# rvp-group/Splat-LOAM

Measured on AMD Instinct MI355X. Metric: fwd+bwd Msplats/s, higher is better.
Workload: dtype f32; 1 GPU; 500000 surfels, 64x2048 spherical, 1 keyframe/GPU per iteration drawn from a window of 8 keyframes as Mapper.optimize does (sample_geometric, p=0.4): render fwd + mapper loss + bwd + fused Adam (one native sls_mapping_step per iteration); step=one bench step = 10 mapping iterations (1013 steps = 10130 timed iterations), N=500000, H=64, W=2048, keyframes=8, parallelism=keyframe-dp1, status_read=lagged-1, gradient_sums=float atomics

## Files before the change

include/sls_abi.h:

```cpp
#ifndef SLS_ABI_H
#define SLS_ABI_H

#include <stddef.h>
#include <stdint.h>

#ifdef __cplusplus
extern "C" {
#endif

#define SLS_OK 0
#define SLS_E_ARG (-1)
#define SLS_E_HIP (-2)
#define SLS_E_SCRATCH (-3)
#define SLS_E_UNSUPPORTED (-4)

typedef struct SlsCamera {
    int32_t H, W;
    int32_t wrap;
    int32_t tile_cull_min;
    float fx, fy, cx, cy;
    float scale_modifier;
    float near_cut, far_cut;
    uint32_t flags;
    float Rvw[9];
    float tvw[3];
    float pix_offset[2];
} SlsCamera;
#define SLS_CAM_LEAN_ALLMAP 1u

const char *sls_last_error(void);
int sls_version(void);

int sls_tile_w(void);
int sls_tile_h(void);
int sls_rec_stride(void);
int sls_grec_stride(void);

int sls_camera_from_matrices(const float *view_host, const float *proj_host, int H, int W,
                             float scale_modifier, SlsCamera *out);

int sls_ray_tables(const SlsCamera *cam, float *col_cs_host, float *row_cs_host);
int sls_ray_tables_at(const SlsCamera *cam, float col_offset, float row_offset, float *col_cs_host,
                      float *row_cs_host);

size_t sls_stage1_scratch_bytes(int N);
int sls_forward_stage1(const SlsCamera *cam, int N,
                       const float *means3D, const float *scales, const float *rotations,
                       const float *opacities, const float *col_cs, const float *row_cs,
                       float *rec, int32_t *radii, int32_t *rect, uint32_t *tiles_touched, uint64_t *tile_mask,
                       uint32_t *block_box,
                       float *depth, uint32_t *order, uint32_t *offsets, uint32_t *total_out,
                       void *scratch, size_t scratch_bytes, void *stream);

size_t sls_sort_scratch_bytes(uint64_t R);
size_t sls_block_mask_bytes(uint64_t R, int H, int W);
int sls_forward_stage2(const SlsCamera *cam, int N, uint64_t R,
                       const float *rec, const int32_t *rect, const uint32_t *tiles_touched,
                       const uint64_t *tile_mask, const uint32_t *block_box,
                       const float *depth, const uint32_t *order, const uint32_t *offsets,
                       const uint32_t *total_dev,
                       uint32_t *tile_keys, uint32_t *vals, uint32_t *tile_keys_tmp, uint32_t *vals_tmp,
                       void *sort_scratch, size_t sort_scratch_bytes, int *sorted_in_tmp,
                       uint64_t *keys64_out, int list_pairs,
                       const uint32_t **sorted_list, int *sorted_stride,
                       uint32_t *ranges, const float *col_cs, const float *row_cs,
                       float *allmap, float *pix_state, uint32_t *pix_contrib,
                       uint32_t *tile_consumed, uint64_t *block_masks, int *block_masks_shape, void *stream);

int sls_backward(const SlsCamera *cam, int N, uint64_t R,
                 const float *means3D, const float *scales, const float *rotations,
                 const int32_t *radii, const float *rec,
                 const uint32_t *ranges, const uint32_t *vals_sorted, int vals_stride,
                 const float *col_cs, const float *row_cs,
                 const float *pix_state, const uint32_t *pix_contrib,
                 const float *dL_dallmap, float *grec,
                 float *dL_dmeans3D, float *dL_dscales, float *dL_drotations,
                 float *dL_dopacities, const uint64_t *block_masks, int block_masks_shape, void *stream);

size_t sls_pose_grad_scratch_bytes(int N);
int sls_backward_pose(const SlsCamera *cam, int N, uint64_t R,
                      const float *means3D, const float *scales, const float *rotations,
                      const int32_t *radii, const float *rec,
                      const uint32_t *ranges, const uint32_t *vals_sorted, int vals_stride,
                      const float *col_cs, const float *row_cs,
                      const float *pix_state, const uint32_t *pix_contrib,
                      const float *dL_dallmap, float *grec,
                      float *dL_dmeans3D, float *dL_dscales, float *dL_drotations,
                      float *dL_dopacities, const uint64_t *block_masks, int block_masks_shape,
                      float *pose_grad, void *pose_scratch, size_t pose_scratch_bytes, void *stream);

size_t sls_backward_det_scratch_bytes(int N);
int sls_backward_det(const SlsCamera *cam, int N, uint64_t R,
                     const float *means3D, const float *scales, const float *rotations, const int32_t *radii,
                     const float *rec, const uint32_t *ranges, const uint32_t *vals_sorted, int vals_stride,
                     const float *col_cs, const float *row_cs, const float *pix_state, const uint32_t *pix_contrib,
                     const float *dL_dallmap,
                     float *dL_dmeans3D, float *dL_dscales, float *dL_drotations, float *dL_dopacities,
                     const uint64_t *block_masks, int block_masks_shape, void *det_scratch, size_t det_scratch_bytes,
                     void *stream);
int sls_backward_det_pose(const SlsCamera *cam, int N, uint64_t R,
                          const float *means3D, const float *scales, const float *rotations, const int32_t *radii,
                          const float *rec, const uint32_t *ranges, const uint32_t *vals_sorted, int vals_stride,
                          const float *col_cs, const float *row_cs, const float *pix_state, const uint32_t *pix_contrib,
                          const float *dL_dallmap,
                          float *dL_dmeans3D, float *dL_dscales, float *dL_drotations, float *dL_dopacities,
                          const uint64_t *block_masks, int block_masks_shape, void *det_scratch, size_t det_scratch_bytes,
                          float *pose_grad, void *pose_scratch, size_t pose_scratch_bytes, void *stream);

struct SlsMappingStatus;
size_t sls_forward_ws_bytes(int N, int H, int W, uint64_t R_capacity);
int sls_forward_ws(const SlsCamera *cam, int N, const float *means3D, const float *scales, const float *rotations,
                   const float *opacities, const float *col_cs, const float *row_cs, uint64_t R_capacity,
                   uint32_t *depth_order, int reuse_rounds, int list_pairs, int workspace_ready, int want_backward,
                   int32_t *radii, float *allmap, void *workspace, size_t workspace_bytes, struct SlsMappingStatus *status_dev,
                   struct SlsMappingStatus *status_mirror, const uint32_t **sorted_list, int *sorted_stride,
                   int *block_masks_shape, void *stream);
int sls_wait_status_mirror(const void *mirror_host, uint32_t sentinel, void *stream);
int sls_backward_ws(const SlsCamera *cam, int N, const float *means3D, const float *scales, const float *rotations,
                    const int32_t *radii, const float *col_cs, const float *row_cs, const float *dL_dallmap,
                    uint64_t R_capacity, void *workspace, size_t workspace_bytes, const uint32_t *sorted_list,
                    int sorted_stride, int block_masks_shape, uint32_t *block_order, float *dL_dmeans3D,
                    float *dL_dscales, float *dL_drotations, float *dL_dopacities, void *stream);
int sls_backward_ws_pose(const SlsCamera *cam, int N, const float *means3D, const float *scales, const float *rotations,
                         const int32_t *radii, const float *col_cs, const float *row_cs, const float *dL_dallmap,
                         uint64_t R_capacity, void *workspace, size_t workspace_bytes, const uint32_t *sorted_list,
                         int sorted_stride, int block_masks_shape, uint32_t *block_order, float *dL_dmeans3D,
                         float *dL_dscales, float *dL_drotations, float *dL_dopacities, float *pose_grad,
                         void *pose_scratch, size_t pose_scratch_bytes, void *stream);

size_t sls_consumer_scratch_bytes(int H, int W);
int sls_consumer_fwd_bwd(int H, int W, const float *allmap, const float *gt_depth, const uint8_t *valid,
                         const float *col_cs_half, const float *row_cs_half, float depth_ratio,
                         float lambda_normal, float lambda_alpha, int n_valid, float *loss_sums,
                         float *dL_dallmap, void *scratch, size_t scratch_bytes, void *stream);

int sls_render_maps(int H, int W, const float *allmap, const float *view_rot9, const float *col_cs_half,
                    const float *row_cs_half, float depth_ratio, float *rend_normal, float *surf_depth,
                    float *surf_normal, void *stream);

int sls_densify_weights(int H, int W, const float *image_depth, const uint8_t *valid, const float *rend_alpha,
                        float threshold_opacity, float *weights_out, uint32_t *stats_out, void *stream);

#define SLS_DENSIFY_DRAW_MAX_PIXELS 262144
size_t sls_densify_draw_scratch_bytes(int H, int W);
int sls_densify_draw(int H, int W, const float *image_depth, const uint8_t *valid, const float *rend_alpha,
                     float threshold_opacity, double percentage, uint64_t seed, uint32_t draw_index, float *weights_out,
                     int64_t *pixels_out, uint32_t *stats_out, uint32_t *stats_mirror, void *scratch, size_t scratch_bytes,
                     void *stream);

int sls_densify_rows(int n, int H, int W, const int64_t *pixels, const float *image_depth, const float *image_normal,
                     const float *col_cs_half, const float *row_cs_half, const float *cam_to_model16,
                     const float *model_T_frame16, float *xyz_out, float *quat_out, void *stream);

#define SLS_SURFACE_MAX_PIXELS 262144
size_t sls_surface_scratch_bytes(int H, int W);
int sls_surface_samples(int H, int W, const float *allmap, const float *col_cs_half, const float *row_cs_half,
                        const float *cam_to_world12, float min_opacity, float max_depth_dist, float depth_ratio,
                        int n_samples, uint64_t seed, uint32_t frame_id, float *points_out, float *normals_out,
                        int32_t *pixels_out, uint32_t *status_out, void *scratch, size_t scratch_bytes, void *stream);

struct SlsMappingStatus;
typedef struct SlsMappingConfig {
    float lambda_alpha, lambda_normal, scaling_max, scaling_max_penalty, depth_ratio;
    float lr_xyz, lr_opacity, lr_scaling, lr_rotation;
    int32_t apply_adam;
    int32_t reuse_depth_order;
    int32_t keep_grads;
    int32_t workspace_ready;
    double beta1, beta2, eps;
    uint32_t *depth_order;
    struct SlsMappingStatus *status_mirror;
    float *void_flags_out;
    uint32_t grad_chunk;
    uint32_t grad_ranks;
    int32_t deterministic;
    int32_t block_masks;
    uint64_t *grad_bitmap;
    uint8_t *det_prev;
    int32_t phase;
    int32_t reserved;
    uint32_t *block_order;
    const uint64_t *union_bitmap;
    const uint32_t *union_prefix;
    float *grad_compact;
    uint32_t *grad_compact_index;
    uint32_t grad_compact_capacity;
    uint32_t reserved2;
    float *pose_grad;
    void *pose_scratch;
    size_t pose_scratch_bytes;
} SlsMappingConfig;
typedef struct SlsMappingStatus {
    uint32_t R;
    uint32_t overflow;
    float loss_sums[4];
    float loss_reg;
    uint32_t exchange_count;
} SlsMappingStatus;
size_t sls_mapping_workspace_bytes(int N, int H, int W, uint64_t R_capacity);
size_t sls_block_order_bytes(int H, int W);
size_t sls_mapping_workspace_bytes_cfg(int N, int H, int W, uint64_t R_capacity, const struct SlsMappingConfig *cfg);
int sls_mapping_step(const SlsCamera *cam, int N,
                     float *xyz, float *scaling_raw, float *rotation_raw, float *opacity_raw,
                     float *grads, float *exp_avg, float *exp_avg_sq, int64_t adam_step,
                     const float *gt_depth, const uint8_t *valid, int n_valid,
                     const float *col_cs, const float *row_cs,
                     const float *col_cs_half, const float *row_cs_half,
                     const SlsMappingConfig *cfg, uint64_t R_capacity,
                     void *workspace, size_t workspace_bytes,
                     SlsMappingStatus *status_dev, float **allmap_out, void *stream);

#define SLS_MAX_BATCH 8
typedef struct SlsKeyframeInputs {
    SlsCamera cam;
    const float *gt_depth;
    const uint8_t *valid;
    int32_t n_valid;
    int32_t reuse_depth_order;
    const float *col_cs, *row_cs;
    const float *col_cs_half, *row_cs_half;
    uint32_t *depth_order;
    uint32_t *block_order;
    uint8_t *det_prev;
    float *pose_grad;
} SlsKeyframeInputs;
size_t sls_mapping_workspace_bytes_batch(int G, int N, int H, int W, uint64_t R_capacity, const SlsMappingConfig *cfg);
int sls_mapping_step_batch(int G, const SlsKeyframeInputs *keyframes, int N,
                           float *xyz, float *scaling_raw, float *rotation_raw, float *opacity_raw,
                           float *grads, float *exp_avg, float *exp_avg_sq, int64_t adam_step,
                           const SlsMappingConfig *cfg, uint64_t R_capacity, void *workspace, size_t workspace_bytes,
                           SlsMappingStatus *status_dev, void *stream);

typedef struct SlsAlignerParams {
    int32_t num_iterations;
    int32_t min_inliers;
    float max_distance;
    float min_cos_angle;
    float huber_delta;
    float range_weight;
    float range_huber;
    float depth_min, depth_max;
    float damping;
} SlsAlignerParams;
typedef struct SlsAlignerResult {
    float pose[12];
    float fitness;
    float chi2;
    float last_step;
    int32_t inliers, valid_query, iterations;
} SlsAlignerResult;
size_t sls_aligner_workspace_bytes(void);
int sls_aligner_normals(const SlsCamera *cam, const float *depth, const float *points, float depth_min,
                        float *normals, void *stream);
int sls_aligner_linearize(const SlsCamera *cam, const SlsAlignerParams *prm, const float *ref_depth,
                          const float *ref_points, const float *ref_normals, const float *query_depth,
                          const float *query_points, const float *T_host, void *workspace, double *sys_out,
                          void *stream);
int sls_aligner_align(const SlsCamera *cam, const SlsAlignerParams *prm, const float *ref_depth,
                      const float *ref_points, const float *ref_normals, const float *query_depth,
                      const float *query_points, const float *T_host, void *workspace,
                      SlsAlignerResult *result_dev, void *stream);

size_t sls_projector_scratch_bytes(int H, int W);
int sls_projector_prepare(int H, int W, void *scratch, size_t scratch_bytes, void *stream);
int sls_projector_intrinsics(int n, const float *cloud, int H, int W, float full_azimuth_threshold_deg,
                             float *intrinsics_out, void *scratch, size_t scratch_bytes, void *stream);
int sls_projector_project(int n, const float *cloud, const float *K_dev, int H, int W, float depth_min,
                          float depth_max, int32_t *lut, float *range_image, float *normals_image,
                          uint8_t *valid, void *scratch, size_t scratch_bytes, void *stream);

typedef struct SlsAdamGroup {
    float *param;
    const float *grad;
    float *exp_avg;
    float *exp_avg_sq;
    int64_t numel;
    float lr;
    float pad;
} SlsAdamGroup;
int sls_adam_step(const SlsAdamGroup *groups_host, int ngroups, double beta1, double beta2,
                  double eps, int64_t step, void *stream);
int sls_adam_step_guarded(const SlsAdamGroup *groups_host, int ngroups, double beta1, double beta2,
                          double eps, int64_t step, const uint32_t *skip_flag_dev, void *stream);
int sls_adam_step_reduced(const SlsAdamGroup *groups_host, int ngroups, double beta1, double beta2,
                          double eps, int64_t step, const float *void_flags_dev,
                          struct SlsMappingStatus *status_dev, struct SlsMappingStatus *status_mirror,
                          void *stream);

int sls_grad_union(int N, const uint64_t *bitmaps, int n_bitmaps, uint64_t *union_bitmap, uint32_t capacity,
                   uint32_t *word_prefix, struct SlsMappingStatus *status_dev, void *stream);
int sls_adam_step_union(int N, float *xyz, float *opacity_raw, float *scaling_raw, float *rotation_raw,
                        const uint32_t *compact_index, const float *compact_reduced, uint32_t capacity, float *exp_avg,
                        float *exp_avg_sq, float lr_xyz, float lr_opacity, float lr_scaling, float lr_rotation, double beta1,
                        double beta2, double eps, int64_t step, struct SlsMappingStatus *status_dev,
                        struct SlsMappingStatus *status_mirror, void *stream);
size_t sls_grad_bitmap_words(int N);
int sls_grad_compact(int N, const uint64_t *bitmaps, int n_bitmaps, uint64_t *union_bitmap, const float *grads_flat,
                     float *compact, uint32_t capacity, uint32_t *word_prefix, struct SlsMappingStatus *status_dev,
                     void *stream);
int sls_adam_step_sparse(int N, float *xyz, float *opacity_raw, float *scaling_raw, float *rotation_raw,
                         const uint64_t *union_bitmap, const uint32_t *word_prefix, const float *compact_reduced,
                         float *exp_avg, float *exp_avg_sq, float lr_xyz, float lr_opacity, float lr_scaling,
                         float lr_rotation, double beta1, double beta2, double eps, int64_t step, int part,
                         struct SlsMappingStatus *status_dev, struct SlsMappingStatus *status_mirror, void *stream);

size_t sls_knn_scratch_bytes(int M);
int sls_knn_dist2(int M, const float *xyz, float *out, void *scratch, size_t scratch_bytes,
                  void *stream);
int sls_knn_dist2_first(int M, int M_first, const float *xyz, float *out, void *scratch, size_t scratch_bytes,
                        void *stream);

int sls_mark_visible(const SlsCamera *cam, int N, const float *means3D, uint8_t *visible,
                     void *stream);

int sls_timing_slots(void);
const char *sls_timing_name(int slot);
int sls_timing_enable(int mode);
int sls_timing_collect(double *total_ms_host, int64_t *counts_host);

int sls_debug_wave_cycles(uint32_t *fwd_cycles, uint32_t *bwd_cycles);

int sls_debug_variant(int fwd, int bwd);

int sls_selftest(void *stream);

#ifdef __cplusplus
}
#endif
#endif
```

splat_loam_amd/_abi.py:

```python
from __future__ import annotations

import ctypes as C
import os

_HERE = os.path.dirname(os.path.abspath(__file__))
LIB_PATH = os.path.join(_HERE, "libsls_hip.so")

SLS_OK = 0


class SlsCamera(C.Structure):
    _fields_ = [
        ("H", C.c_int32), ("W", C.c_int32), ("wrap", C.c_int32), ("tile_cull_min", C.c_int32),
        ("fx", C.c_float), ("fy", C.c_float), ("cx", C.c_float), ("cy", C.c_float),
        ("scale_modifier", C.c_float), ("near_cut", C.c_float), ("far_cut", C.c_float), ("flags", C.c_uint32),
        ("Rvw", C.c_float * 9), ("tvw", C.c_float * 3),
        ("pix_offset", C.c_float * 2),
    ]


class SlsMappingConfig(C.Structure):
    _fields_ = [
        ("lambda_alpha", C.c_float), ("lambda_normal", C.c_float), ("scaling_max", C.c_float),
        ("scaling_max_penalty", C.c_float), ("depth_ratio", C.c_float),
        ("lr_xyz", C.c_float), ("lr_opacity", C.c_float), ("lr_scaling", C.c_float), ("lr_rotation", C.c_float),
        ("apply_adam", C.c_int32), ("reuse_depth_order", C.c_int32), ("keep_grads", C.c_int32), ("workspace_ready", C.c_int32),
        ("beta1", C.c_double), ("beta2", C.c_double), ("eps", C.c_double),
        ("depth_order", C.c_void_p),
        ("status_mirror", C.c_void_p),
        ("void_flags_out", C.c_void_p),
        ("grad_chunk", C.c_uint32), ("grad_ranks", C.c_uint32),
        ("deterministic", C.c_int32), ("block_masks", C.c_int32),
        ("grad_bitmap", C.c_void_p),
        ("det_prev", C.c_void_p),
        ("phase", C.c_int32), ("reserved", C.c_int32),
        ("block_order", C.c_void_p),
        ("union_bitmap", C.c_void_p), ("union_prefix", C.c_void_p), ("grad_compact", C.c_void_p),
        ("grad_compact_index", C.c_void_p), ("grad_compact_capacity", C.c_uint32), ("reserved2", C.c_uint32),
        ("pose_grad", C.c_void_p), ("pose_scratch", C.c_void_p), ("pose_scratch_bytes", C.c_size_t),
    ]


class SlsAlignerParams(C.Structure):
    _fields_ = [("num_iterations", C.c_int32), ("min_inliers", C.c_int32), ("max_distance", C.c_float),
                ("min_cos_angle", C.c_float), ("huber_delta", C.c_float), ("range_weight", C.c_float),
                ("range_huber", C.c_float), ("depth_min", C.c_float), ("depth_max", C.c_float), ("damping", C.c_float)]


class SlsAlignerResult(C.Structure):
    _fields_ = [("pose", C.c_float * 12), ("fitness", C.c_float), ("chi2", C.c_float), ("last_step", C.c_float),
                ("inliers", C.c_int32), ("valid_query", C.c_int32), ("iterations", C.c_int32)]


class SlsMappingStatus(C.Structure):
    _fields_ = [("R", C.c_uint32), ("overflow", C.c_uint32), ("loss_sums", C.c_float * 4),
                ("loss_reg", C.c_float), ("exchange_count", C.c_uint32)]


class SlsKeyframeInputs(C.Structure):
    _fields_ = [
        ("cam", SlsCamera), ("gt_depth", C.c_void_p), ("valid", C.c_void_p), ("n_valid", C.c_int32),
        ("reuse_depth_order", C.c_int32), ("col_cs", C.c_void_p), ("row_cs", C.c_void_p), ("col_cs_half", C.c_void_p),
        ("row_cs_half", C.c_void_p), ("depth_order", C.c_void_p), ("block_order", C.c_void_p), ("det_prev", C.c_void_p),
        ("pose_grad", C.c_void_p),
    ]


SLS_MAX_BATCH = 8


class SlsAdamGroup(C.Structure):
    _fields_ = [
        ("param", C.c_void_p), ("grad", C.c_void_p), ("exp_avg", C.c_void_p), ("exp_avg_sq", C.c_void_p),
        ("numel", C.c_int64), ("lr", C.c_float), ("pad", C.c_float),
    ]


_VP = C.c_void_p
_PROTOS = {
    "sls_last_error": (C.c_char_p, []),
    "sls_version": (C.c_int, []),
    "sls_tile_w": (C.c_int, []),
    "sls_tile_h": (C.c_int, []),
    "sls_rec_stride": (C.c_int, []),
    "sls_grec_stride": (C.c_int, []),
    "sls_camera_from_matrices": (C.c_int, [_VP, _VP, C.c_int, C.c_int, C.c_float, C.POINTER(SlsCamera)]),
    "sls_ray_tables": (C.c_int, [C.POINTER(SlsCamera), _VP, _VP]),
    "sls_ray_tables_at": (C.c_int, [C.POINTER(SlsCamera), C.c_float, C.c_float, _VP, _VP]),
    "sls_render_maps": (C.c_int, [C.c_int, C.c_int, _VP, _VP, _VP, _VP, C.c_float, _VP, _VP, _VP, _VP]),
    "sls_densify_rows": (C.c_int, [C.c_int, C.c_int, C.c_int] + [_VP] * 10),
    "sls_densify_weights": (C.c_int, [C.c_int, C.c_int, _VP, _VP, _VP, C.c_float, _VP, _VP, _VP]),
    "sls_densify_draw_scratch_bytes": (C.c_size_t, [C.c_int, C.c_int]),
    "sls_densify_draw": (C.c_int, [C.c_int, C.c_int, _VP, _VP, _VP, C.c_float, C.c_double, C.c_uint64, C.c_uint32] +
                         [_VP] * 5 + [C.c_size_t, _VP]),
    "sls_surface_scratch_bytes": (C.c_size_t, [C.c_int, C.c_int]),
    "sls_surface_samples": (C.c_int, [C.c_int, C.c_int, _VP, _VP, _VP, _VP, C.c_float, C.c_float, C.c_float, C.c_int, C.c_uint64,
                                      C.c_uint32, _VP, _VP, _VP, _VP, _VP, C.c_size_t, _VP]),
    "sls_consumer_scratch_bytes": (C.c_size_t, [C.c_int, C.c_int]),
    "sls_consumer_fwd_bwd": (C.c_int, [C.c_int, C.c_int] + [_VP] * 5 + [C.c_float] * 3 + [C.c_int, _VP, _VP, _VP,
                                                                                         C.c_size_t, _VP]),
    "sls_stage1_scratch_bytes": (C.c_size_t, [C.c_int]),
    "sls_forward_stage1": (C.c_int, [C.POINTER(SlsCamera), C.c_int] + [_VP] * 16 + [_VP, C.c_size_t, _VP]),
    "sls_sort_scratch_bytes": (C.c_size_t, [C.c_uint64]),
    "sls_forward_stage2": (C.c_int, [C.POINTER(SlsCamera), C.c_int, C.c_uint64] + [_VP] * 13 +
                           [_VP, C.c_size_t, C.POINTER(C.c_int), _VP, C.c_int, C.POINTER(C.c_void_p), C.POINTER(C.c_int)] +
                           [_VP] * 8 + [C.POINTER(C.c_int), _VP]),
    "sls_block_mask_bytes": (C.c_size_t, [C.c_uint64, C.c_int, C.c_int]),
    "sls_mapping_workspace_bytes": (C.c_size_t, [C.c_int, C.c_int, C.c_int, C.c_uint64]),
    "sls_block_order_bytes": (C.c_size_t, [C.c_int, C.c_int]),
    "sls_mapping_workspace_bytes_cfg": (C.c_size_t, [C.c_int, C.c_int, C.c_int, C.c_uint64, C.POINTER(SlsMappingConfig)]),
    "sls_mapping_step": (C.c_int, [C.POINTER(SlsCamera), C.c_int] + [_VP] * 7 + [C.c_int64, _VP, _VP, C.c_int] +
                         [_VP] * 4 + [C.POINTER(SlsMappingConfig), C.c_uint64, _VP, C.c_size_t, _VP,
                                      C.POINTER(C.c_void_p), _VP]),
    "sls_mapping_workspace_bytes_batch": (C.c_size_t, [C.c_int, C.c_int, C.c_int, C.c_int, C.c_uint64,
                                                       C.POINTER(SlsMappingConfig)]),
    "sls_mapping_step_batch": (C.c_int, [C.c_int, C.POINTER(SlsKeyframeInputs), C.c_int] + [_VP] * 7 +
                               [C.c_int64, C.POINTER(SlsMappingConfig), C.c_uint64, _VP, C.c_size_t, _VP, _VP]),
    "sls_backward": (C.c_int, [C.POINTER(SlsCamera), C.c_int, C.c_uint64] + [_VP] * 7 + [C.c_int] + [_VP] * 11 +
                     [C.c_int, _VP]),
    "sls_forward_ws_bytes": (C.c_size_t, [C.c_int, C.c_int, C.c_int, C.c_uint64]),
    "sls_forward_ws": (C.c_int, [C.POINTER(SlsCamera), C.c_int] + [_VP] * 6 + [C.c_uint64, _VP, C.c_int, C.c_int, C.c_int, C.c_int, _VP, _VP,
                                 _VP, C.c_size_t, _VP, _VP, C.POINTER(C.c_void_p), C.POINTER(C.c_int), C.POINTER(C.c_int), _VP]),
    "sls_backward_ws": (C.c_int, [C.POINTER(SlsCamera), C.c_int] + [_VP] * 7 + [C.c_uint64, _VP, C.c_size_t, _VP, C.c_int, C.c_int] +
                        [_VP] * 6),
    "sls_backward_det_scratch_bytes": (C.c_size_t, [C.c_int]),
    "sls_backward_det": (C.c_int, [C.POINTER(SlsCamera), C.c_int, C.c_uint64] + [_VP] * 7 + [C.c_int] + [_VP] * 10 +
                         [C.c_int, _VP, C.c_size_t, _VP]),
    "sls_pose_grad_scratch_bytes": (C.c_size_t, [C.c_int]),
    "sls_backward_pose": (C.c_int, [C.POINTER(SlsCamera), C.c_int, C.c_uint64] + [_VP] * 7 + [C.c_int] + [_VP] * 11 +
                          [C.c_int, _VP, _VP, C.c_size_t, _VP]),
    "sls_backward_ws_pose": (C.c_int, [C.POINTER(SlsCamera), C.c_int] + [_VP] * 7 + [C.c_uint64, _VP, C.c_size_t, _VP, C.c_int, C.c_int] +
                             [_VP] * 5 + [_VP, _VP, C.c_size_t, _VP]),
    "sls_backward_det_pose": (C.c_int, [C.POINTER(SlsCamera), C.c_int, C.c_uint64] + [_VP] * 7 + [C.c_int] + [_VP] * 10 +
                              [C.c_int, _VP, C.c_size_t, _VP, _VP, C.c_size_t, _VP]),
    "sls_adam_step": (C.c_int, [C.POINTER(SlsAdamGroup), C.c_int, C.c_double, C.c_double, C.c_double, C.c_int64, _VP]),
    "sls_adam_step_guarded": (C.c_int, [C.POINTER(SlsAdamGroup), C.c_int, C.c_double, C.c_double, C.c_double,
                                        C.c_int64, _VP, _VP]),
    "sls_adam_step_reduced": (C.c_int, [C.POINTER(SlsAdamGroup), C.c_int, C.c_double, C.c_double, C.c_double,
                                        C.c_int64, _VP, _VP, _VP, _VP]),
    "sls_grad_bitmap_words": (C.c_size_t, [C.c_int]),
    "sls_grad_union": (C.c_int, [C.c_int, _VP, C.c_int, _VP, C.c_uint32, _VP, _VP, _VP]),
    "sls_adam_step_union": (C.c_int, [C.c_int] + [_VP] * 6 + [C.c_uint32, _VP, _VP] + [C.c_float] * 4 + [C.c_double] * 3 + [C.c_int64, _VP, _VP, _VP]),
    "sls_grad_compact": (C.c_int, [C.c_int, _VP, C.c_int, _VP, _VP, _VP, C.c_uint32, _VP, _VP, _VP]),
    "sls_adam_step_sparse": (C.c_int, [C.c_int] + [_VP] * 9 + [C.c_float] * 4 + [C.c_double] * 3 + [C.c_int64, C.c_int, _VP, _VP, _VP]),
    "sls_projector_scratch_bytes": (C.c_size_t, [C.c_int, C.c_int]),
    "sls_projector_prepare": (C.c_int, [C.c_int, C.c_int, _VP, C.c_size_t, _VP]),
    "sls_projector_intrinsics": (C.c_int, [C.c_int, _VP, C.c_int, C.c_int, C.c_float, _VP, _VP, C.c_size_t, _VP]),
    "sls_projector_project": (C.c_int, [C.c_int, _VP, _VP, C.c_int, C.c_int, C.c_float, C.c_float, _VP, _VP, _VP, _VP,
                                        _VP, C.c_size_t, _VP]),
    "sls_knn_scratch_bytes": (C.c_size_t, [C.c_int]),
    "sls_knn_dist2": (C.c_int, [C.c_int, _VP, _VP, _VP, C.c_size_t, _VP]),
    "sls_wait_status_mirror": (C.c_int, [_VP, C.c_uint32, _VP]),
    "sls_knn_dist2_first": (C.c_int, [C.c_int, C.c_int, _VP, _VP, _VP, C.c_size_t, _VP]),
    "sls_mark_visible": (C.c_int, [C.POINTER(SlsCamera), C.c_int, _VP, _VP, _VP]),
    "sls_aligner_workspace_bytes": (C.c_size_t, []),
    "sls_aligner_normals": (C.c_int, [C.POINTER(SlsCamera), _VP, _VP, C.c_float, _VP, _VP]),
    "sls_aligner_linearize": (C.c_int, [C.POINTER(SlsCamera), C.POINTER(SlsAlignerParams)] + [_VP] * 8 + [_VP]),
    "sls_aligner_align": (C.c_int, [C.POINTER(SlsCamera), C.POINTER(SlsAlignerParams)] + [_VP] * 8 + [_VP]),
    "sls_timing_slots": (C.c_int, []),
    "sls_timing_name": (C.c_char_p, [C.c_int]),
    "sls_timing_enable": (C.c_int, [C.c_int]),
    "sls_timing_collect": (C.c_int, [C.POINTER(C.c_double), C.POINTER(C.c_int64)]),
    "sls_debug_wave_cycles": (C.c_int, [_VP, _VP]),
    "sls_debug_variant": (C.c_int, [C.c_int, C.c_int]),
    "sls_selftest": (C.c_int, [_VP]),
}

EXPORTS = tuple(_PROTOS)

_lib = None


def lib():
    global _lib
    if _lib is None:
        if not os.path.exists(LIB_PATH):
            raise RuntimeError(
                f"{LIB_PATH} is missing: build it with `python -c 'import __graft_entry__ as g; g.build()'` "
                "(hipcc --offload-arch=gfx950).  There is no CPU fallback.")
        import torch
        l = C.CDLL(LIB_PATH)
        for name, (res, args) in _PROTOS.items():
            fn = getattr(l, name)
            fn.restype = res
            fn.argtypes = args
        _lib = l
    return _lib


def check(rc: int, what: str) -> None:
    if rc != SLS_OK:
        msg = lib().sls_last_error().decode("utf-8", "replace")
        raise RuntimeError(f"{what} failed (code {rc}): {msg}")


def tile_size() -> tuple[int, int]:
    l = lib()
    return int(l.sls_tile_w()), int(l.sls_tile_h())
```

splat_loam_amd/csrc/sls_common.hpp:

```cpp
#pragma once
#include <atomic>
#include <cmath>

#include <hip/hip_runtime.h>
#include <stdint.h>
#include <stdio.h>

#include "../../include/sls_abi.h"
#include "../../include/sls_spec.h"
#include "../../include/sls_det_math.h"

#ifndef SLS_TILE_W
#define SLS_TILE_W 16
#endif
#ifndef SLS_TILE_H
#define SLS_TILE_H 16
#endif
static_assert((SLS_TILE_W * SLS_TILE_H) % 64 == 0, "a tile must be a whole number of wave64s");
static_assert(SLS_TILE_W % 8 == 0 && SLS_TILE_H % 8 == 0, "tiles are made of 8x8 wave sub-tiles");

namespace sls {

constexpr int kWave = 64;
constexpr int kTileW = SLS_TILE_W;
constexpr int kTileH = SLS_TILE_H;
constexpr int kTilePix = kTileW * kTileH;
constexpr int kRec4 = SLS_REC_STRIDE / 4;
constexpr int kGrec = SLS_GREC_STRIDE;

void set_error(const char *fmt, ...);

enum TimerSlot {
    T_PREPROCESS_FWD = 0, T_SCAN, T_EMIT_KEYS, T_SORT_HIST, T_SORT_ROWSCAN, T_SORT_SCATTER, T_TILE_RANGES,
    T_RENDER_FWD, T_GREC_MEMSET, T_RENDER_BWD, T_PREPROCESS_BWD, T_ADAM, T_KNN, T_CONSUMER, T_RESORT, T_BIN_COUNT, T_BIN_DIRECT,
    T_COUNT
};
struct DebugState {
    std::atomic<uint32_t *> dbg_fwd_cycles{nullptr}, dbg_bwd_cycles{nullptr};
};
DebugState &debug_state();
void timer_begin(int slot, hipStream_t st);
void timer_end(int slot, hipStream_t st);
struct ScopedTimer {
    int slot; hipStream_t st;
    bool open = true;
    ScopedTimer(int s, hipStream_t t) : slot(s), st(t) { timer_begin(slot, st); }
    void end_now() { if (open) { timer_end(slot, st); open = false; } }
    ~ScopedTimer() { end_now(); }
};

#define SLS_HIP_CHECK(expr)                                                         \
    do {                                                                            \
        hipError_t e_ = (expr);                                                     \
        if (e_ != hipSuccess) {                                                     \
            ::sls::set_error("%s failed: %s (%s:%d)", #expr, hipGetErrorString(e_), \
                             __FILE__, __LINE__);                                   \
            return SLS_E_HIP;                                                       \
        }                                                                           \
    } while (0)

#define SLS_LAUNCH_CHECK(name)                                                              \
    do {                                                                                    \
        hipError_t e_ = hipGetLastError();                                                  \
        if (e_ != hipSuccess) {                                                             \
            ::sls::set_error("launch of %s failed: %s", name, hipGetErrorString(e_));       \
            return SLS_E_HIP;                                                               \
        }                                                                                   \
    } while (0)

#define SLS_REQUIRE(cond, msg)                       \
    do {                                             \
        if (!(cond)) {                               \
            ::sls::set_error("%s: %s", __func__, msg); \
            return SLS_E_ARG;                        \
        }                                            \
    } while (0)

struct DevCam {
    int H, W, wrap, GX, GY;
    float fx, fy, cx, cy, mod, near_c, far_c;
    float R[9];
    float t[3];
    SlsTileCullCam tc;
    int tile_cull;
};

inline SlsTileCullCam make_tile_cull_cam(float fx, float fy, int W, int wrap)
{
    SlsTileCullCam c;
    const double hx = 0.5 * (double)(kTileW - 1), hy = 0.5 * (double)(kTileH - 1);
    const double ax = 0.5 / (double)fx, ay = 0.5 / (double)fy;
    c.chx = (float)cos(ax); c.shx = (float)sin(ax);
    c.chy = (float)cos(ay); c.shy = (float)sin(ay);
    const double kx = hx / (double)fx, ky = hy / (double)fy;
    c.kx = (float)kx; c.ky = (float)ky;
    const double span = fabs(kx) + fabs(ky);
    c.eps = (float)(0.5 * span * span * 1.01 + 4.0e-6);
    c.hx = (float)hx; c.hy = (float)hy;
    c.wrapW = wrap ? (float)W : 0.0f;
    c.invW = wrap ? 1.0f / (float)W : 0.0f;
    return c;
}

inline DevCam make_devcam(const SlsCamera &c)
{
    DevCam d;
    d.H = c.H; d.W = c.W; d.wrap = c.wrap;
    d.GX = (c.W + kTileW - 1) / kTileW;
    d.GY = (c.H + kTileH - 1) / kTileH;
    d.fx = c.fx; d.fy = c.fy;
    d.cx = c.cx - c.pix_offset[0]; d.cy = c.cy - c.pix_offset[1];
    d.mod = c.scale_modifier; d.near_c = c.near_cut; d.far_c = c.far_cut;
    for (int i = 0; i < 9; ++i) d.R[i] = c.Rvw[i];
    for (int i = 0; i < 3; ++i) d.t[i] = c.tvw[i];
    d.tc = make_tile_cull_cam(d.fx, d.fy, d.W, d.wrap);
    d.tile_cull = c.tile_cull_min == 0 ? SLS_TILE_CULL_MIN_DEFAULT : (c.tile_cull_min == 1 ? 0 : c.tile_cull_min);
    return d;
}

__host__ __device__ inline bool block_box_fits(int W, int H) { return W <= 4096 && H <= 128; }
__device__ __forceinline__ uint32_t make_block_box(float cx, float cy, float ex, float ey, int NC)
{
    if (!(ex >= 0.0f && ey >= 0.0f)) return 0u;
    const float lo = ceilf((cx - ex - 7.01f) * 0.125f), hi = floorf((cx + ex + 0.01f) * 0.125f);
    const int n = (int)fminf(hi - lo, (float)(NC - 1));
    int c0 = (int)fmaxf(fminf(lo, 1.0e6f), -1.0e6f) % NC;
    c0 += c0 < 0 ? NC : 0;
    const int r0 = (int)fminf(fmaxf(ceilf((cy - ey - 1.01f) * 0.5f), 0.0f), 63.0f);
    const int r1 = (int)fminf(floorf((cy + ey + 0.01f) * 0.5f), 63.0f);
    if (n < 0 || r1 < r0) return 0u;
    return (uint32_t)c0 | ((uint32_t)(n + 1) << 9) | ((uint32_t)r0 << 19) | ((uint32_t)(r1 + 1) << 25);
}

__device__ __forceinline__ uint64_t wave_ballot(bool p) { return __builtin_amdgcn_ballot_w64(p); }
__device__ __forceinline__ bool wave_all(bool p) { return __builtin_amdgcn_ballot_w64(!p) == 0ull; }

__device__ __forceinline__ int lane_id() { return (int)__builtin_amdgcn_mbcnt_hi(~0u, __builtin_amdgcn_mbcnt_lo(~0u, 0u)); }

template <int CTRL, int ROW_MASK>
__device__ __forceinline__ float dpp_mov0(float v)
{
    return __builtin_bit_cast(float, __builtin_amdgcn_update_dpp(0, __builtin_bit_cast(int, v), CTRL, ROW_MASK, 0xF, false));
}

__device__ __forceinline__ float wave_sum_to_lane63(float v)
{
    v += dpp_mov0<0xB1, 0xF>(v);
    v += dpp_mov0<0x4E, 0xF>(v);
    v += dpp_mov0<0x124, 0xF>(v);
    v += dpp_mov0<0x128, 0xF>(v);
    v += dpp_mov0<0x142, 0xA>(v);
    v += dpp_mov0<0x143, 0xC>(v);
    return v;
}

__device__ __forceinline__ float dpp_xor4(float v)
{
    int a = __builtin_amdgcn_update_dpp(0, __builtin_bit_cast(int, v), 0x104, 0xF, 0x5, false);
    a = __builtin_amdgcn_update_dpp(a, __builtin_bit_cast(int, v), 0x114, 0xF, 0xA, false);
    return __builtin_bit_cast(float, a);
}

typedef float v2f __attribute__((ext_vector_type(2)));
typedef unsigned v2u __attribute__((ext_vector_type(2)));
__device__ __forceinline__ v2f mk2(float a, float b) { v2f r; r.x = a; r.y = b; return r; }

__device__ __forceinline__ void permlane32_swap(float &a, float &b)
{
    const v2u r = __builtin_amdgcn_permlane32_swap(__float_as_uint(a), __float_as_uint(b), false, false);
    a = __uint_as_float(r.x); b = __uint_as_float(r.y);
}
__device__ __forceinline__ void permlane16_swap(float &a, float &b)
{
    const v2u r = __builtin_amdgcn_permlane16_swap(__float_as_uint(a), __float_as_uint(b), false, false);
    a = __uint_as_float(r.x); b = __uint_as_float(r.y);
}

__device__ __forceinline__ float block_reduce16_pk(const v2f (&x)[8], int lane)
{
    float a[16];
#pragma unroll
    for (int i = 0; i < 8; ++i) { a[2 * i] = x[i].x; a[2 * i + 1] = x[i].y; }
#pragma unroll
    for (int i = 0; i < 8; ++i) permlane32_swap(a[i], a[i + 8]);
    v2f y[4];
#pragma unroll
    for (int i = 0; i < 4; ++i) y[i] = mk2(a[2 * i], a[2 * i + 1]) + mk2(a[2 * i + 8], a[2 * i + 9]);
    float b[8];
#pragma unroll
    for (int i = 0; i < 4; ++i) { b[2 * i] = y[i].x; b[2 * i + 1] = y[i].y; }
#pragma unroll
    for (int i = 0; i < 4; ++i) permlane16_swap(b[i], b[i + 4]);
    const v2f z01 = mk2(b[0], b[1]) + mk2(b[4], b[5]), z23 = mk2(b[2], b[3]) + mk2(b[6], b[7]);
    const float z[4] = { z01.x, z01.y, z23.x, z23.y };
    float w0 = z[0], w1 = z[1];
    asm("s_nop 1\n\t"
        "v_add_f32_dpp %0, %0, %0 row_ror:8 row_mask:0xf bank_mask:0x3\n\t"
        "v_add_f32_dpp %1, %1, %1 row_ror:8 row_mask:0xf bank_mask:0x3\n\t"
        "v_add_f32_dpp %0, %2, %2 row_ror:8 row_mask:0xf bank_mask:0xc\n\t"
        "v_add_f32_dpp %1, %3, %3 row_ror:8 row_mask:0xf bank_mask:0xc\n\t"
        "s_nop 1\n\t"
        "v_add_f32_dpp %0, %0, %0 row_shl:4 row_mask:0xf bank_mask:0x5\n\t"
        "v_add_f32_dpp %0, %1, %1 row_shr:4 row_mask:0xf bank_mask:0xa"
        : "+v"(w0), "+v"(w1) : "v"(z[2]), "v"(z[3]));
    const float r = w0;
    (void)lane;
    return r;
}

__device__ __forceinline__ bool mask_bbox8x8(uint64_t m, int &xmin, int &xmax, int &ymin, int &ymax)
{
    if (m == 0) return false;
    uint64_t c = m | (m >> 32);
    c |= c >> 16;
    c |= c >> 8;
    const uint32_t cols = (uint32_t)c & 0xFFu;
    uint64_t t = (m | (m >> 4)) & 0x0F0F0F0F0F0F0F0Full;
    t = (t | (t >> 2)) & 0x0303030303030303ull;
    t = (t | (t >> 1)) & 0x0101010101010101ull;
    xmin = __builtin_ctz(cols);
    xmax = 31 - __builtin_clz(cols);
    ymin = __builtin_ctzll(t) >> 3;
    ymax = (63 - __builtin_clzll(t)) >> 3;
    return true;
}

__device__ __forceinline__ float readlane63(float v)
{
    return __builtin_bit_cast(float, __builtin_amdgcn_readlane(__builtin_bit_cast(int, v), 63));
}

__host__ __device__ inline uint32_t depth_order_key(float range)
{
    constexpr uint32_t kBase = 0x3E000000u;
    constexpr uint32_t kMax = (1u << 29) - 1u;
#if defined(__HIP_DEVICE_COMPILE__)
    const uint32_t b = __float_as_uint(range) & 0x7FFFFFFFu;
#else
    uint32_t b; __builtin_memcpy(&b, &range, 4); b &= 0x7FFFFFFFu;
#endif
    const uint32_t k = b > kBase ? b - kBase : 0u;
    return k < kMax ? k : kMax;
}

__device__ __forceinline__ uint32_t det_predict(float sum)
{
    const uint32_t e = (__float_as_uint(sum) >> 23) & 0xFFu;
    return sum == 0.0f ? 0u : min(max(e + 12u, 1u), 254u);
}
constexpr uint32_t kDetMispredicted = 8u;
__device__ __forceinline__ int det_scale_exp(uint32_t own, uint32_t gex)
{
    return (int)max(own, gex > 24u ? gex - 24u : (gex ? 1u : 0u));
}

struct AdamCoef {
    float w1, b2, w2, eps, bc2_sqrt, bc1;
};
inline AdamCoef make_adam_coef(double beta1, double beta2, double eps, int64_t step)
{
    AdamCoef c;
    c.w1 = (float)(1.0 - beta1);
    c.b2 = (float)beta2;
    c.w2 = (float)(1.0 - beta2);
    c.eps = (float)eps;
    c.bc1 = (float)(1.0 - pow(beta1, (double)step));
    c.bc2_sqrt = (float)sqrt(1.0 - pow(beta2, (double)step));
    return c;
}
__device__ __forceinline__ void adam_one(float &p, float g, float &m, float &v, float step_size, const AdamCoef &a)
{
    m = m + (g - m) * a.w1;
    v = v * a.b2 + (a.w2 * g) * g;
    const float denom = __builtin_amdgcn_sqrtf(v) * __builtin_amdgcn_rcpf(a.bc2_sqrt) + a.eps;
    p = p - step_size * (m * __builtin_amdgcn_rcpf(denom));
}
struct AdamFuse {
    int enabled, write_grads;
    int clear_grec;
    AdamCoef c;
    float lr_xyz, lr_opacity, lr_scaling, lr_rotation;
    float *exp_avg, *exp_avg_sq;
    const uint32_t *skip_flag;
    uint32_t *status_src;
    uint32_t *status_mirror;
    uint8_t *touched;
    float *void_flags;
    int void_count, void_stride;
    uint32_t gchunk;
    float *gbase;
    const uint32_t *det_max;
    const long long *det_acc;
    uint8_t *det_prev;
    uint32_t *det_gex;
    int det_onepass;
    float *reg_accum;
    uint64_t *grad_bitmap;
    int grad_bitmap_words;
    const float *loss_partials;
    int n_loss_partials;
    float loss_w[3];
    int order_T;
    const uint32_t *order_cost;
    uint32_t *order_out;
    int publisher;
    const uint64_t *union_bitmap;
    const uint32_t *union_prefix;
    float *compact;
    uint32_t *compact_idx;
    uint32_t compact_cap;
};

struct BatchKeyframe {
    DevCam cam;
    const int32_t *radii;
    float4 *grec;
    uint8_t *touched;
    uint32_t *status;
    const uint32_t *det_max;
    long long *det_acc;
    uint8_t *det_prev;
    uint32_t *det_gex;
    const float *loss_partials;
    float loss_w[3];
    const uint32_t *order_cost;
    uint32_t *order_out;
};

struct BatchFuse {
    int G;
    int n_loss_partials, order_T;
    BatchKeyframe kf[SLS_MAX_BATCH];
    AdamFuse af;
};

constexpr int kPoseRow = 8;
struct PoseOut {
    float *rows;
    uint32_t *counter;
    float *out[SLS_MAX_BATCH];
};

__device__ __forceinline__ void mirror_status_block(const uint32_t *src, uint32_t *mirror, bool override1 = false,
                                                    uint32_t word1 = 0u)
{
    uint32_t w[8];
#pragma unroll
    for (int k = 0; k < 8; ++k) w[k] = src[k];
    if (override1) w[1] = word1;
#pragma unroll
    for (int k = 0; k < 7; ++k) __builtin_nontemporal_store(w[k], mirror + k);
    __threadfence_system();
    __builtin_nontemporal_store(w[7], mirror + 7);
}

__host__ __device__ inline int xcd_remap(int b, int n)
{
    constexpr int kXcd = 8;
    if (n % kXcd != 0) return b;
    const int per = n / kXcd;
    return (b % kXcd) * per + b / kXcd;
}

}
```

splat_loam_amd/csrc/sls_exchange.hip:

```cpp
#include <string.h>

#include "sls_launch.hpp"

namespace sls {

constexpr uint32_t kExchangeTooSmall = 4u;

constexpr int kPrefixLdsWords = 12288;
__global__ __launch_bounds__(1024) void exchange_prefix_kernel(int nwords, const uint64_t *__restrict__ maps, int n_maps,
                                                               uint64_t *__restrict__ bitmap,
                                                               uint32_t *__restrict__ word_prefix, uint32_t capacity,
                                                               uint32_t *__restrict__ status_block)
{
    extern __shared__ uint64_t s_dyn[];
    __shared__ uint32_t s_wave[16];
    const bool in_lds = nwords <= kPrefixLdsWords;
    const int per = (nwords + 1023) / 1024, w0 = (int)threadIdx.x * per, w1 = min(w0 + per, nwords);
    const int pad = (in_lds && (per & 1) == 0) ? 1 : 0;
    uint64_t *const words = in_lds ? s_dyn : bitmap;
    uint32_t *const pref = in_lds ? reinterpret_cast<uint32_t *>(s_dyn + nwords + 1024) : word_prefix;
    const uint32_t magic = (uint32_t)((0x100000000ull + (uint64_t)per - 1ull) / (uint64_t)per);
#define SLS_PW(w_) ((w_) + (pad ? (int)__umulhi((uint32_t)(w_), magic) : 0))
    const int lane = threadIdx.x & 63, wave = threadIdx.x >> 6;
    const size_t stride = (size_t)(nwords + 2);
    constexpr int kBatch = 12;
    for (int base = 0; base < nwords; base += 1024 * kBatch) {
        uint64_t acc[kBatch];
#pragma unroll
        for (int k = 0; k < kBatch; ++k) acc[k] = 0ull;
        for (int m = 0; m < n_maps; m += 2) {
            uint64_t v0[kBatch], v1[kBatch];
            const bool two = m + 1 < n_maps;
#pragma unroll
            for (int k = 0; k < kBatch; ++k) {
                const int w = base + k * 1024 + (int)threadIdx.x;
                v0[k] = w < nwords ? maps[(size_t)m * stride + (size_t)w] : 0ull;
                v1[k] = (two && w < nwords) ? maps[(size_t)(m + 1) * stride + (size_t)w] : 0ull;
            }
#pragma unroll
            for (int k = 0; k < kBatch; ++k) acc[k] |= v0[k] | v1[k];
        }
#pragma unroll
        for (int k = 0; k < kBatch; ++k) {
            const int w = base + k * 1024 + (int)threadIdx.x;
            if (w < nwords) words[SLS_PW(w)] = acc[k];
        }
    }
    if (!in_lds) __threadfence();
    __syncthreads();
    uint32_t c = 0u;
    const int own = w0 + (pad ? (int)threadIdx.x : 0);
    for (int w = w0; w < w1; ++w) c += (uint32_t)__popcll(words[own + (w - w0)]);
    uint32_t incl = c;
#pragma unroll
    for (int off = 1; off < 64; off <<= 1) {
        const uint32_t t = __shfl_up(incl, off, 64);
        if (lane >= off) incl += t;
    }
    if (lane == 63) s_wave[wave] = incl;
    __syncthreads();
    uint32_t pre = incl - c;
    for (int k = 0; k < wave; ++k) pre += s_wave[k];
    for (int w = w0; w < w1; ++w) {
        pref[own + (w - w0)] = pre;
        pre += (uint32_t)__popcll(words[own + (w - w0)]);
    }
    if (threadIdx.x == 1023) {
        const uint32_t K = pre;
        uint64_t v0 = 0ull, v1 = 0ull;
        for (int m = 0; m < n_maps; ++m) {
            v0 |= maps[(size_t)m * stride + (size_t)nwords];
            v1 |= maps[(size_t)m * stride + (size_t)nwords + 1];
        }
        bitmap[nwords] = v0; bitmap[nwords + 1] = v1;
        const uint32_t void_bits = (v0 ? 1u : 0u) | (v1 ? 2u : 0u);
        status_block[7] = K;
        status_block[1] = void_bits | (K > capacity ? kExchangeTooSmall : 0u);
    }
    if (in_lds) {
        __syncthreads();
        for (int w = threadIdx.x; w < nwords; w += 1024) { bitmap[w] = words[SLS_PW(w)]; word_prefix[w] = pref[SLS_PW(w)]; }
    }
#undef SLS_PW
}

__global__ __launch_bounds__(256) void exchange_compact_kernel(int N, const uint64_t *__restrict__ bitmap,
                                                               const uint32_t *__restrict__ word_prefix,
                                                               const float *__restrict__ grads, float *__restrict__ compact,
                                                               uint32_t capacity)
{
    const int i = blockIdx.x * 256 + threadIdx.x;
    if (i >= N) return;
    const uint64_t word = bitmap[i >> 6];
    const int b = i & 63;
    if (!((word >> b) & 1ull)) return;
    const uint32_t slot = word_prefix[i >> 6] + (uint32_t)__popcll(word & ((1ull << b) - 1ull));
    if (slot >= capacity) return;
    const size_t n = (size_t)N;
    float *o = compact + (size_t)slot * 10;
    o[0] = grads[3 * (size_t)i]; o[1] = grads[3 * (size_t)i + 1]; o[2] = grads[3 * (size_t)i + 2];
    o[3] = grads[3 * n + i];
    o[4] = grads[4 * n + 2 * (size_t)i]; o[5] = grads[4 * n + 2 * (size_t)i + 1];
#pragma unroll
    for (int k = 0; k < 4; ++k) o[6 + k] = grads[6 * n + 4 * (size_t)i + k];
}

__global__ __launch_bounds__(256) void touched_bitmap_kernel(int N, const uint8_t *__restrict__ touched,
                                                             const float2 *__restrict__ scaling_raw, float log_smax_margin,
                                                             int reg_on, const uint32_t *__restrict__ status_block,
                                                             uint64_t *__restrict__ bitmap, int nwords)
{
    const int i = blockIdx.x * 256 + threadIdx.x;
    bool on = false;
    if (i < N) {
        on = touched[i] != 0;
        if (reg_on) { const float2 s = scaling_raw[i]; on = on || fmaxf(s.x, s.y) >= log_smax_margin; }
    }
    const uint64_t word = __ballot(on);
    if ((threadIdx.x & 63) == 0 && i < N) bitmap[i >> 6] = word;
    if (i == 0) {
        const uint32_t bits = status_block[1];
        bitmap[nwords] = (bits & 1u) ? 1ull : 0ull;
        bitmap[nwords + 1] = (bits & ~1u) ? 1ull : 0ull;
    }
}
int launch_touched_bitmap(int N, const uint8_t *touched, const float *scaling_raw, float smax, float pen,
                          const uint32_t *status_block, uint64_t *bitmap, hipStream_t st)
{
    hipLaunchKernelGGL(touched_bitmap_kernel, dim3((N + 255) / 256), dim3(256), 0, st, N, touched, (const float2 *)scaling_raw,
                       logf(fmaxf(smax, 1e-30f)) - 1e-3f, pen != 0.0f ? 1 : 0, status_block, bitmap, (N + 63) / 64);
    SLS_LAUNCH_CHECK("touched_bitmap_kernel");
    return SLS_OK;
}

struct SparseAdamArgs {
    float *xyz, *opacity, *scaling, *rotation;
    float *exp_avg, *exp_avg_sq;
    float lr_xyz, lr_opacity, lr_scaling, lr_rotation;
    AdamCoef c;
};

__global__ __launch_bounds__(256) void exchange_adam_kernel(int N, SparseAdamArgs a, const uint64_t *__restrict__ bitmap,
                                                            const uint32_t *__restrict__ word_prefix,
                                                            const float *__restrict__ compact,
                                                            const uint32_t *__restrict__ status_block,
                                                            uint32_t *__restrict__ status_mirror, int part)
{
    const int i = blockIdx.x * 256 + threadIdx.x;
    if (i == 0 && status_mirror && part != 1) mirror_status_block(status_block, status_mirror);
    if (status_block[1] != 0u) return;
    if (i >= N) return;
    float g[10];
#pragma unroll
    for (int k = 0; k < 10; ++k) g[k] = 0.0f;
    const uint64_t word = bitmap[i >> 6];
    const int b = i & 63;
    const bool in_union = (word >> b) & 1ull;
    if ((part == 1 && in_union) || (part == 2 && !in_union)) return;
    if (in_union) {
        const uint32_t slot = word_prefix[i >> 6] + (uint32_t)__popcll(word & ((1ull << b) - 1ull));
        const float *s = compact + (size_t)slot * 10;
#pragma unroll
        for (int k = 0; k < 10; ++k) g[k] = s[k];
    }
    const size_t n = (size_t)N, ix = 3 * (size_t)i, io = 3 * n + i, is = 4 * n + 2 * (size_t)i, ir = 6 * n + 4 * (size_t)i;
    float *M = a.exp_avg, *V = a.exp_avg_sq;
    const float ibc1 = __builtin_amdgcn_rcpf(a.c.bc1);
    const float st_x = a.lr_xyz * ibc1, st_o = a.lr_opacity * ibc1, st_s = a.lr_scaling * ibc1, st_r = a.lr_rotation * ibc1;
    float p, m, v;
#pragma unroll
    for (int k = 0; k < 3; ++k) {
        p = a.xyz[ix + k]; m = M[ix + k]; v = V[ix + k];
        adam_one(p, g[k], m, v, st_x, a.c);
        a.xyz[ix + k] = p; M[ix + k] = m; V[ix + k] = v;
    }
    p = a.opacity[i]; m = M[io]; v = V[io];
    adam_one(p, g[3], m, v, st_o, a.c);
    a.opacity[i] = p; M[io] = m; V[io] = v;
#pragma unroll
    for (int k = 0; k < 2; ++k) {
        p = a.scaling[2 * (size_t)i + k]; m = M[is + k]; v = V[is + k];
        adam_one(p, g[4 + k], m, v, st_s, a.c);
        a.scaling[2 * (size_t)i + k] = p; M[is + k] = m; V[is + k] = v;
    }
#pragma unroll
    for (int k = 0; k < 4; ++k) {
        p = a.rotation[4 * (size_t)i + k]; m = M[ir + k]; v = V[ir + k];
        adam_one(p, g[6 + k], m, v, st_r, a.c);
        a.rotation[4 * (size_t)i + k] = p; M[ir + k] = m; V[ir + k] = v;
    }
}

__global__ __launch_bounds__(256) void exchange_adam_union_kernel(uint32_t capacity, size_t n, SparseAdamArgs a,
                                                                  const uint32_t *__restrict__ index,
                                                                  const float *__restrict__ compact,
                                                                  const uint32_t *__restrict__ status_block,
                                                                  uint32_t *__restrict__ status_mirror)
{
    const uint32_t slot = blockIdx.x * 256u + threadIdx.x;
    if (slot == 0 && status_mirror) mirror_status_block(status_block, status_mirror);
    if (status_block[1] != 0u) return;
    if (slot >= min(capacity, status_block[7])) return;
    const size_t i = index[slot];
    const size_t off[4] = { 3 * i, 3 * n + i, 4 * n + 2 * i, 6 * n + 4 * i };
    float *const par[4] = { a.xyz + 3 * i, a.opacity + i, a.scaling + 2 * i, a.rotation + 4 * i };
    constexpr int kW[4] = { 3, 1, 2, 4 }, kG[4] = { 0, 3, 4, 6 };
    const float *row = compact + (size_t)slot * 10;
    float g[10], p[10], m[10], v[10];
#pragma unroll
    for (int k = 0; k < 10; ++k) g[k] = row[k];
#pragma unroll
    for (int q = 0; q < 4; ++q)
#pragma unroll
        for (int k = 0; k < kW[q]; ++k) {
            p[kG[q] + k] = par[q][k]; m[kG[q] + k] = a.exp_avg[off[q] + k]; v[kG[q] + k] = a.exp_avg_sq[off[q] + k];
        }
    const float ibc1 = __builtin_amdgcn_rcpf(a.c.bc1);
    const float stp[4] = { a.lr_xyz * ibc1, a.lr_opacity * ibc1, a.lr_scaling * ibc1, a.lr_rotation * ibc1 };
#pragma unroll
    for (int q = 0; q < 4; ++q)
#pragma unroll
        for (int k = 0; k < kW[q]; ++k) adam_one(p[kG[q] + k], g[kG[q] + k], m[kG[q] + k], v[kG[q] + k], stp[q], a.c);
#pragma unroll
    for (int q = 0; q < 4; ++q)
#pragma unroll
        for (int k = 0; k < kW[q]; ++k) {
            par[q][k] = p[kG[q] + k]; a.exp_avg[off[q] + k] = m[kG[q] + k]; a.exp_avg_sq[off[q] + k] = v[kG[q] + k];
        }
}

}

using namespace sls;

extern "C" {

size_t sls_grad_bitmap_words(int N) { return N > 0 ? (size_t)((N + 63) / 64) + 2 : 2; }

int sls_grad_union(int N, const uint64_t *bitmaps, int n_bitmaps, uint64_t *union_bitmap, uint32_t capacity,
                   uint32_t *word_prefix, SlsMappingStatus *status_dev, void *stream)
{
    return sls_grad_compact(N, bitmaps, n_bitmaps, union_bitmap, nullptr, nullptr, capacity, word_prefix, status_dev, stream);
}

int sls_grad_compact(int N, const uint64_t *bitmaps, int n_bitmaps, uint64_t *union_bitmap, const float *grads_flat,
                     float *compact, uint32_t capacity, uint32_t *word_prefix, SlsMappingStatus *status_dev, void *stream)
{
    SLS_REQUIRE(N > 0 && bitmaps && n_bitmaps >= 1 && union_bitmap && word_prefix && status_dev && (!grads_flat == !compact),
                "bad argument");
    hipStream_t st = (hipStream_t)stream;
    const int nwords = (N + 63) / 64;
    const size_t lds = nwords <= kPrefixLdsWords ? (size_t)(nwords + 1024) * 12 + 16 : 0;
    static bool lds_allowed = false;
    if (lds > 0 && !lds_allowed) {
        SLS_HIP_CHECK(hipFuncSetAttribute(reinterpret_cast<const void *>(exchange_prefix_kernel),
                                          hipFuncAttributeMaxDynamicSharedMemorySize, (kPrefixLdsWords + 1024) * 12 + 16));
        lds_allowed = true;
    }
    hipLaunchKernelGGL(exchange_prefix_kernel, dim3(1), dim3(1024), lds, st, nwords, bitmaps, n_bitmaps, union_bitmap,
                       word_prefix, capacity, (uint32_t *)status_dev);
    SLS_LAUNCH_CHECK("exchange_prefix_kernel");
    if (!grads_flat) return SLS_OK;
    hipLaunchKernelGGL(exchange_compact_kernel, dim3((N + 255) / 256), dim3(256), 0, st, N, (const uint64_t *)union_bitmap,
                       (const uint32_t *)word_prefix, grads_flat, compact, capacity);
    SLS_LAUNCH_CHECK("exchange_compact_kernel");
    return SLS_OK;
}

int sls_adam_step_sparse(int N, float *xyz, float *opacity, float *scaling, float *rotation,
                         const uint64_t *union_bitmap, const uint32_t *word_prefix, const float *compact_reduced,
                         float *exp_avg, float *exp_avg_sq, float lr_xyz, float lr_opacity, float lr_scaling,
                         float lr_rotation, double beta1, double beta2, double eps, int64_t step, int part,
                         SlsMappingStatus *status_dev, SlsMappingStatus *status_mirror, void *stream)
{
    SLS_REQUIRE(part >= 0 && part <= 2, "part: 0 every surfel, 1 outside the union, 2 the union");
    SLS_REQUIRE(N > 0 && xyz && opacity && scaling && rotation && union_bitmap && word_prefix && compact_reduced &&
                    exp_avg && exp_avg_sq && status_dev,
                "bad argument");
    SLS_REQUIRE(step >= 1, "step is 1-based");
    SparseAdamArgs a;
    memset(&a, 0, sizeof(a));
    a.xyz = xyz; a.opacity = opacity; a.scaling = scaling; a.rotation = rotation;
    a.exp_avg = exp_avg; a.exp_avg_sq = exp_avg_sq;
    a.lr_xyz = lr_xyz; a.lr_opacity = lr_opacity; a.lr_scaling = lr_scaling; a.lr_rotation = lr_rotation;
    a.c = make_adam_coef(beta1, beta2, eps, step);
    ScopedTimer tm(T_ADAM, (hipStream_t)stream);
    hipLaunchKernelGGL(exchange_adam_kernel, dim3((N + 255) / 256), dim3(256), 0, (hipStream_t)stream, N, a, union_bitmap,
                       word_prefix, compact_reduced, (const uint32_t *)status_dev, (uint32_t *)status_mirror, part);
    SLS_LAUNCH_CHECK("exchange_adam_kernel");
    return SLS_OK;
}

int sls_adam_step_union(int N, float *xyz, float *opacity, float *scaling, float *rotation, const uint32_t *compact_index,
                        const float *compact_reduced, uint32_t capacity, float *exp_avg, float *exp_avg_sq, float lr_xyz,
                        float lr_opacity, float lr_scaling, float lr_rotation, double beta1, double beta2, double eps,
                        int64_t step, SlsMappingStatus *status_dev, SlsMappingStatus *status_mirror, void *stream)
{
    SLS_REQUIRE(N > 0 && xyz && opacity && scaling && rotation && compact_index && compact_reduced && capacity > 0 &&
                    exp_avg && exp_avg_sq && status_dev,
                "bad argument");
    SLS_REQUIRE(step >= 1, "step is 1-based");
    SparseAdamArgs a;
    memset(&a, 0, sizeof(a));
    a.xyz = xyz; a.opacity = opacity; a.scaling = scaling; a.rotation = rotation;
    a.exp_avg = exp_avg; a.exp_avg_sq = exp_avg_sq;
    a.lr_xyz = lr_xyz; a.lr_opacity = lr_opacity; a.lr_scaling = lr_scaling; a.lr_rotation = lr_rotation;
    a.c = make_adam_coef(beta1, beta2, eps, step);
    ScopedTimer tm(T_ADAM, (hipStream_t)stream);
    hipLaunchKernelGGL(exchange_adam_union_kernel, dim3((capacity + 255u) / 256u), dim3(256), 0, (hipStream_t)stream, capacity,
                       (size_t)N, a, compact_index, compact_reduced, (const uint32_t *)status_dev, (uint32_t *)status_mirror);
    SLS_LAUNCH_CHECK("exchange_adam_union_kernel");
    return SLS_OK;
}

}
```

splat_loam_amd/csrc/sls_pipeline.hip:

```cpp
#include <stdlib.h>
#include <string.h>

#include "sls_consumer_dev.hpp"
#include "sls_launch.hpp"

namespace sls {

struct MapWs {
    float *rec; int32_t *radii; int32_t *rect; uint32_t *tiles; uint64_t *tmask; int32_t *erec; int32_t *serec; uint32_t *sbox; float *depth; uint32_t *order; uint32_t *offsets;
    void *order_scratch; size_t order_scratch_bytes;
    uint32_t *tkeys, *vals, *tkeys_tmp, *vals_tmp; void *sort_scratch; size_t sort_scratch_bytes;
    uint32_t *ranges; float *allmap; float *pix_state; uint32_t *pix_contrib; uint32_t *tile_consumed;
    float *dL_dallmap; void *consumer_scratch; size_t consumer_scratch_bytes; float *grec; size_t zero_bytes; uint64_t *block_masks; float *reg_accum; uint8_t *touched;
    uint32_t *det_max; unsigned long long *det_acc; size_t det_bytes;
    uint32_t *det_gex;
    uint32_t *block_cost, *block_order;
    size_t total;
};

struct Taker {
    char *p; size_t off;
    void *operator()(size_t bytes) { void *r = (void *)(p + off); off += (bytes + 255) & ~(size_t)255; return r; }
};

// ... 235 lines not shown
    SLS_REQUIRE(means3D && scales && rotations && radii && grec && dL_dmeans3D && dL_dscales && dL_drotations &&
                    dL_dopacities,
                "null pointer");
    SLS_REQUIRE(vals_stride == 1 || vals_stride == 2, "vals_stride: 1 (plain list) or 2 ((surfel, block mask) pairs)");
    hipStream_t st = (hipStream_t)stream;
    const DevCam dc = make_devcam(*cam);
    {
        ScopedTimer tm(T_GREC_MEMSET, st);
        SLS_HIP_CHECK(hipMemsetAsync(grec, 0, sizeof(float) * (size_t)N * SLS_GREC_STRIDE, st));
    }
    if (R > 0) {
        SLS_REQUIRE(rec && ranges && vals_sorted && col_cs && row_cs && pix_state && pix_contrib && dL_dallmap,
                    "null pointer");
        RenderBwdLaunch rb{};
        rb.ranges = ranges; rb.vals = vals_sorted; rb.vals_stride = vals_stride; rb.rec = rec; rb.col_cs = col_cs; rb.row_cs = row_cs;
        rb.pix_state = pix_state; rb.pix_contrib = pix_contrib; rb.dL_dallmap = dL_dallmap;
        rb.block_masks = block_masks_shape ? block_masks : nullptr; rb.block_masks_shape = block_masks_shape;
        rb.lean = (cam->flags & SLS_CAM_LEAN_ALLMAP) != 0;
        rb.grec = grec; rb.order_in_handover = true;
        if (int rc = launch_render_bwd(dc, rb, st)) return rc;
    }
    PreBwdLaunch pb{};
    pb.N = N; pb.means = means3D; pb.scales = scales; pb.rots = rotations; pb.radii = radii; pb.grec = grec;
    pb.dmeans = dL_dmeans3D; pb.dscales = dL_dscales; pb.drots = dL_drotations; pb.dopac = dL_dopacities;
    pb.pose = pose_arg(po);
    return launch_preprocess_bwd(dc, pb, st);
}

size_t sls_backward_det_scratch_bytes(int N) { return N > 0 ? (size_t)N * SLS_GREC_STRIDE * 12 + 256 : 256; }

int sls_backward_det(const SlsCamera *cam, int N, uint64_t R, const float *means3D, const float *scales,
                     const float *rotations, const int32_t *radii, const float *rec, const uint32_t *ranges,
                     const uint32_t *vals_sorted, int vals_stride, const float *col_cs, const float *row_cs,
                     const float *pix_state, const uint32_t *pix_contrib, const float *dL_dallmap, float *dL_dmeans3D,
                     float *dL_dscales, float *dL_drotations, float *dL_dopacities, const uint64_t *block_masks,
                     int block_masks_shape, void *det_scratch, size_t det_scratch_bytes, void *stream)
{
    return sls_backward_det_pose(cam, N, R, means3D, scales, rotations, radii, rec, ranges, vals_sorted, vals_stride,
                                 col_cs, row_cs, pix_state, pix_contrib, dL_dallmap, dL_dmeans3D, dL_dscales,
                                 dL_drotations, dL_dopacities, block_masks, block_masks_shape, det_scratch,
                                 det_scratch_bytes, nullptr, nullptr, 0, stream);
}

int sls_backward_det_pose(const SlsCamera *cam, int N, uint64_t R, const float *means3D, const float *scales,
                          const float *rotations, const int32_t *radii, const float *rec, const uint32_t *ranges,
                          const uint32_t *vals_sorted, int vals_stride, const float *col_cs, const float *row_cs,
                          const float *pix_state, const uint32_t *pix_contrib, const float *dL_dallmap,
                          float *dL_dmeans3D, float *dL_dscales, float *dL_drotations, float *dL_dopacities,
                          const uint64_t *block_masks, int block_masks_shape, void *det_scratch, size_t det_scratch_bytes,
                          float *pose_grad, void *pose_scratch, size_t pose_scratch_bytes_, void *stream)
{
    SLS_REQUIRE(cam, "null pointer");
    SLS_REQUIRE(N >= 0, "negative N");
    if (N == 0) {
        if (pose_grad) SLS_HIP_CHECK(hipMemsetAsync(pose_grad, 0, 6 * sizeof(float), (hipStream_t)stream));
        return SLS_OK;
    }
    PoseOut po;
    if (int prc = make_pose_out(1, N, &pose_grad, pose_scratch, pose_scratch_bytes_, &po)) return prc;
    SLS_REQUIRE(means3D && scales && rotations && radii && det_scratch && dL_dmeans3D && dL_dscales && dL_drotations &&
                    dL_dopacities,
                "null pointer");
    SLS_REQUIRE(vals_stride == 1 || vals_stride == 2, "vals_stride: 1 (plain list) or 2 ((surfel, block mask) pairs)");
    if (det_scratch_bytes < sls_backward_det_scratch_bytes(N)) {
        set_error("deterministic-backward scratch too small");
        return SLS_E_SCRATCH;
    }
    hipStream_t st = (hipStream_t)stream;
    const DevCam dc = make_devcam(*cam);
    unsigned long long *acc = (unsigned long long *)(((uintptr_t)det_scratch + 255) & ~(uintptr_t)255);
    uint32_t *mx = (uint32_t *)(acc + (size_t)N * SLS_GREC_STRIDE);
    SLS_HIP_CHECK(hipMemsetAsync(acc, 0, (size_t)N * SLS_GREC_STRIDE * 12, st));
    if (R > 0) {
        SLS_REQUIRE(rec && ranges && vals_sorted && col_cs && row_cs && pix_state && pix_contrib && dL_dallmap,
                    "null pointer");
        RenderBwdLaunch rb{};
        rb.ranges = ranges; rb.vals = vals_sorted; rb.vals_stride = vals_stride; rb.rec = rec; rb.col_cs = col_cs; rb.row_cs = row_cs;
        rb.pix_state = pix_state; rb.pix_contrib = pix_contrib; rb.dL_dallmap = dL_dallmap;
        rb.block_masks = block_masks_shape ? block_masks : nullptr; rb.block_masks_shape = block_masks_shape;
        rb.lean = (cam->flags & SLS_CAM_LEAN_ALLMAP) != 0;
        rb.det_max = mx; rb.det_acc = acc; rb.order_in_handover = true;
        if (int rc = launch_render_bwd(dc, rb, st)) return rc;
    }
    AdamFuse fuse;
    memset(&fuse, 0, sizeof(fuse));
    fuse.det_max = mx;
    fuse.det_acc = (const long long *)acc;
    PreBwdLaunch pb{};
    pb.N = N; pb.means = means3D; pb.scales = scales; pb.rots = rotations; pb.radii = radii;
    pb.dmeans = dL_dmeans3D; pb.dscales = dL_dscales; pb.drots = dL_drotations; pb.dopac = dL_dopacities;
    pb.fuse = &fuse; pb.pose = pose_arg(po);
    return launch_preprocess_bwd(dc, pb, st);
}

struct FrontArgs {
    PreFwdLaunch pf;
    uint32_t *depth_order; int reuse_rounds;
    int workspace_ready;
    uint32_t *status_mirror;
    int list_pairs;
    float *allmap; bool lean;
    bool want_backward;
};

static int binning_front(const DevCam &dc, uint32_t cap, const MapWs &w, const FrontArgs &f, SlsMappingStatus *status_dev,
                         hipStream_t st, const uint32_t **sorted_list, int *sorted_stride)
{
    const int N = f.pf.N;
    if (!f.workspace_ready) {
        ScopedTimer tm(T_GREC_MEMSET, st);
        SLS_HIP_CHECK(hipMemsetAsync(w.reg_accum, 0, w.zero_bytes, st));
    }
    uint32_t *okeys, *ovals, *n_dev;
    uint32_t *order = f.depth_order ? f.depth_order : w.order;
    depth_order_key_buffers(N, w.order_scratch, order, &okeys, &ovals, &n_dev);
    const bool merged_sort = f.reuse_rounds >= 1;
    const bool direct = bin_direct_possible(dc, N, cap);
    BinDirectLaunch bd{};
    if (direct) bd.db = make_direct_bin(dc, N, w.sort_scratch, (uint2 *)w.serec, merged_sort, true);
    PreFwdLaunch pf = f.pf;
    pf.rec = w.rec; pf.order_vals = ovals; pf.n_dev = n_dev;
    pf.status_clear = (uint32_t *)status_dev; pf.tile_mask = w.tmask; pf.erec = w.erec;
    if (merged_sort) { pf.resort_prev_order = order; pf.resort_comp = resort_comp_buffer(N, w.order_scratch); }
    if (direct) {
        pf.order_keys = merged_sort ? nullptr : okeys;
        pf.erec_box = 1;
        if (bd.db.coarse) { pf.zero_words = bd.db.coarse; pf.n_zero_words = (int)direct_coarse_words(dc, N); }
    } else {
        pf.rect = w.rect; pf.tiles = w.tiles; pf.depth = w.depth; pf.order_keys = okeys; pf.sbox = w.sbox;
    }
    if (int rc = launch_preprocess_fwd(dc, pf, st)) return rc;
    ScanHandoff handoff = { nullptr, 0, nullptr, 0 };
    DepthOrderScan ds{};
    ds.N = N; ds.tiles = w.tiles; ds.order = order; ds.offsets = w.offsets; ds.total_out = &status_dev->R;
    ds.scratch = w.order_scratch; ds.scratch_bytes = w.order_scratch_bytes;
    ds.reuse_order = f.reuse_rounds; ds.fail_flag = &status_dev->overflow; ds.window_sort_done = merged_sort;
    ds.direct = direct ? &bd.db : nullptr; ds.erec_box = (const int4 *)w.erec; ds.GX = dc.GX;
    if (int rc = launch_depth_order_scan(ds, st, &handoff)) return rc;
    int in_tmp = 0, rc;
    const uint2 *bmask = nullptr;
    if (direct) {
        bd.N = N; bd.cap = cap; bd.counted = handoff.counted != 0; bd.order = order; bd.erec_box = w.erec;
        bd.scratch = w.sort_scratch; bd.vals_out = w.vals; bd.ranges = w.ranges;
        bd.total_out = &status_dev->R; bd.overflow = &status_dev->overflow;
        bd.resort_windows = handoff.resort_windows; bd.resort_edges = handoff.resort_edges;
        bd.bmask_mode = f.list_pairs; bd.status_mirror = f.status_mirror;
        rc = launch_bin_direct(dc, bd, st, &bmask);
    } else {
        BinSortLaunch bs{};
        bs.N = N; bs.count_ptr = &status_dev->R; bs.cap = cap; bs.order = order; bs.rect = w.rect; bs.tiles = w.tiles;
        bs.tile_mask = dc.tile_cull ? w.tmask : nullptr; bs.erec = (dc.GX < 65536 && dc.GY < 65536) ? w.erec : nullptr;
        bs.depth = w.depth; bs.offsets = w.offsets; bs.sbox = w.sbox; bs.bmask_mode = f.list_pairs;
        bs.tkeys = w.tkeys; bs.vals = w.vals; bs.tkeys_tmp = w.tkeys_tmp; bs.vals_tmp = w.vals_tmp;
        bs.scratch = w.sort_scratch; bs.scratch_bytes = w.sort_scratch_bytes; bs.ranges = w.ranges;
        bs.overflow = &status_dev->overflow; bs.handoff = &handoff; bs.total_out = &status_dev->R;
        rc = launch_bin_sort(dc, bs, st, &in_tmp, &bmask);
    }
    if (rc) return rc;
    *sorted_list = bmask ? (const uint32_t *)bmask : (in_tmp ? w.vals_tmp : w.vals);
    *sorted_stride = bmask ? 2 : 1;
    RenderFwdLaunch rf{};
    rf.ranges = w.ranges; rf.vals = *sorted_list; rf.rec = w.rec; rf.col_cs = pf.col_cs; rf.row_cs = pf.row_cs;
    rf.allmap = f.allmap; rf.pix_state = w.pix_state; rf.pix_contrib = w.pix_contrib; rf.lean = f.lean; rf.bmask = bmask;
    rf.consumed_zeroed = true;
    if (f.want_backward) { rf.block_masks = w.block_masks; rf.block_cost = w.block_cost; }
    return launch_render_fwd(dc, rf, st);
}

size_t sls_forward_ws_bytes(int N, int H, int W, uint64_t R_capacity)
{
    return (N < 0 || H <= 0 || W <= 0) ? 0 : carve(N, H, W, R_capacity, nullptr, false).total;
}

int sls_forward_ws(const SlsCamera *cam, int N, const float *means3D, const float *scales, const float *rotations,
                   const float *opacities, const float *col_cs, const float *row_cs, uint64_t R_capacity,
                   uint32_t *depth_order, int reuse_rounds, int list_pairs, int workspace_ready, int want_backward,
                   int32_t *radii, float *allmap, void *workspace, size_t workspace_bytes, SlsMappingStatus *status_dev,
                   SlsMappingStatus *status_mirror, const uint32_t **sorted_list, int *sorted_stride,
                   int *block_masks_shape, void *stream)
{
    SLS_REQUIRE(cam && status_dev && workspace && sorted_list && sorted_stride && block_masks_shape, "null pointer");
    SLS_REQUIRE(N > 0, "N must be positive");
    SLS_REQUIRE(means3D && scales && rotations && opacities && col_cs && row_cs && radii && allmap, "null pointer");
    SLS_REQUIRE(R_capacity > 0 && R_capacity < (1ull << 32), "bad instance capacity");
    SLS_REQUIRE(((uintptr_t)workspace & 255) == 0, "workspace must be 256-byte aligned");
    SLS_REQUIRE(reuse_rounds >= 0 && reuse_rounds <= 4, "reuse_rounds: 0 from scratch, 1..4 repair rounds");
    SLS_REQUIRE(reuse_rounds == 0 || depth_order, "a repair needs the camera's previous depth order");
    SLS_REQUIRE(list_pairs >= 0 && list_pairs <= 2, "list_pairs: 0 auto, 1 whenever possible, 2 never");
    const int H = cam->H, W = cam->W;
    const DevCam dc = make_devcam(*cam);
    const uint32_t cap = (uint32_t)R_capacity;
    if (!bin_direct_possible(dc, N, cap)) {
        set_error("sls_forward_ws serves what the direct binning serves (<= 512 tiles, D10 off): use the staged forward");
        return SLS_E_UNSUPPORTED;
    }
    const MapWs w = carve(N, H, W, R_capacity, workspace, false);
    if (workspace_bytes < w.total) {
        set_error("forward workspace too small: %zu < %zu", workspace_bytes, w.total);
        return SLS_E_SCRATCH;
    }
    FrontArgs f{};
    f.pf.N = N; f.pf.means = means3D; f.pf.scales = scales; f.pf.rots = rotations; f.pf.opac = opacities;
    f.pf.col_cs = col_cs; f.pf.row_cs = row_cs; f.pf.radii = radii;
    f.depth_order = depth_order; f.reuse_rounds = reuse_rounds; f.workspace_ready = workspace_ready;
    f.status_mirror = (uint32_t *)status_mirror;
    f.list_pairs = list_pairs; f.allmap = allmap; f.lean = (cam->flags & SLS_CAM_LEAN_ALLMAP) != 0;
    f.want_backward = want_backward != 0;
    *block_masks_shape = want_backward ? 3 : 0;
    return binning_front(dc, cap, w, f, status_dev, (hipStream_t)stream, sorted_list, sorted_stride);
}

int sls_backward_ws(const SlsCamera *cam, int N, const float *means3D, const float *scales, const float *rotations,
                    const int32_t *radii, const float *col_cs, const float *row_cs, const float *dL_dallmap,
                    uint64_t R_capacity, void *workspace, size_t workspace_bytes, const uint32_t *sorted_list,
                    int sorted_stride, int block_masks_shape, uint32_t *block_order, float *dL_dmeans3D,
                    float *dL_dscales, float *dL_drotations, float *dL_dopacities, void *stream)
{
    return sls_backward_ws_pose(cam, N, means3D, scales, rotations, radii, col_cs, row_cs, dL_dallmap, R_capacity, workspace,
                                workspace_bytes, sorted_list, sorted_stride, block_masks_shape, block_order, dL_dmeans3D,
                                dL_dscales, dL_drotations, dL_dopacities, nullptr, nullptr, 0, stream);
}

int sls_backward_ws_pose(const SlsCamera *cam, int N, const float *means3D, const float *scales, const float *rotations,
                         const int32_t *radii, const float *col_cs, const float *row_cs, const float *dL_dallmap,
                         uint64_t R_capacity, void *workspace, size_t workspace_bytes, const uint32_t *sorted_list,
                         int sorted_stride, int block_masks_shape, uint32_t *block_order, float *dL_dmeans3D,
                         float *dL_dscales, float *dL_drotations, float *dL_dopacities, float *pose_grad,
                         void *pose_scratch, size_t pose_scratch_bytes_, void *stream)
{
    SLS_REQUIRE(cam && workspace && sorted_list, "null pointer");
    SLS_REQUIRE(N > 0, "N must be positive");
    PoseOut po;
    if (int prc = make_pose_out(1, N, &pose_grad, pose_scratch, pose_scratch_bytes_, &po)) return prc;
    SLS_REQUIRE(means3D && scales && rotations && radii && col_cs && row_cs && dL_dallmap && dL_dmeans3D && dL_dscales &&
                    dL_drotations && dL_dopacities,
                "null pointer");
    SLS_REQUIRE(sorted_stride == 1 || sorted_stride == 2, "sorted_stride: 1 (plain list) or 2 ((surfel, block mask) pairs)");
    const MapWs w = carve(N, cam->H, cam->W, R_capacity, workspace, false);
    if (workspace_bytes < w.total) {
        set_error("forward workspace too small: %zu < %zu", workspace_bytes, w.total);
        return SLS_E_SCRATCH;
    }
    hipStream_t st = (hipStream_t)stream;
    const DevCam dc = make_devcam(*cam);
    const int T = dc.GX * dc.GY;
    const bool order_bwd = block_order != nullptr && block_masks_shape == 3 && launch_order_possible(T);
    RenderBwdLaunch rb{};
    rb.ranges = w.ranges; rb.vals = sorted_list; rb.vals_stride = sorted_stride; rb.rec = w.rec; rb.col_cs = col_cs; rb.row_cs = row_cs;
    rb.pix_state = w.pix_state; rb.pix_contrib = w.pix_contrib; rb.dL_dallmap = dL_dallmap;
    rb.block_masks = block_masks_shape ? w.block_masks : nullptr; rb.block_masks_shape = block_masks_shape;
    rb.lean = (cam->flags & SLS_CAM_LEAN_ALLMAP) != 0;
    rb.grec = w.grec; rb.touched = w.touched;
    if (order_bwd) { rb.block_order = block_order; rb.order_tag = block_order_tag(T); }
    if (int rc = launch_render_bwd(dc, rb, st)) return rc;
    AdamFuse fuse;
    memset(&fuse, 0, sizeof(fuse));
    fuse.clear_grec = 1;
    fuse.touched = w.touched;
    if (order_bwd) { fuse.order_T = T; fuse.order_cost = w.block_cost; fuse.order_out = block_order; }
    PreBwdLaunch pb{};
    pb.N = N; pb.means = means3D; pb.scales = scales; pb.rots = rotations; pb.radii = radii; pb.grec = w.grec;
    pb.dmeans = dL_dmeans3D; pb.dscales = dL_dscales; pb.drots = dL_drotations; pb.dopac = dL_dopacities;
    pb.fuse = &fuse; pb.pose = pose_arg(po);
    return launch_preprocess_bwd(dc, pb, st);
}

struct StepSwitches {
    bool det, det_one;
    bool fuse_c, fuse_b;
    bool order_bwd;
};
static StepSwitches step_switches(const SlsMappingConfig *cfg, int deterministic, bool have_det_prev, bool have_block_order, int T)
{
    StepSwitches s;
    s.det = deterministic != 0;
    s.det_one = deterministic == 2 && have_det_prev;
    s.fuse_c = cfg->depth_ratio == 0.0f;
    s.fuse_b = s.fuse_c && have_block_order;
    s.order_bwd = launch_order_possible(T);
    return s;
}

static void loss_weights(const SlsMappingConfig *cfg, int H, int W, int n_valid, float *lw)
{
    lw[0] = 1.0f / ((float)H * (float)W);
    lw[1] = n_valid > 0 ? cfg->lambda_normal * (1.0f / (float)n_valid) : 0.0f;
    lw[2] = n_valid > 0 ? cfg->lambda_alpha * (1.0f / (float)n_valid) : 0.0f;
}

static void fill_step_fuse(AdamFuse &af, const SlsMappingConfig *cfg, SlsMappingStatus *status_dev, float *reg_accum, int N,
                           float *exp_avg, float *exp_avg_sq, int64_t adam_step)
{
    static_assert(sizeof(SlsMappingStatus) == 32, "the mirror copy moves 8 words");
    af.status_src = (uint32_t *)status_dev; af.status_mirror = (uint32_t *)cfg->status_mirror;
    af.reg_accum = reg_accum; af.void_flags = cfg->void_flags_out;
    const bool aligned = (N % 2 == 0) && ((((uintptr_t)exp_avg | (uintptr_t)exp_avg_sq) & 15) == 0);
    if (!cfg->apply_adam || !aligned) return;
    af.enabled = 1;
    af.write_grads = cfg->keep_grads;
    af.c = make_adam_coef(cfg->beta1, cfg->beta2, cfg->eps, adam_step);
    af.lr_xyz = cfg->lr_xyz; af.lr_opacity = cfg->lr_opacity;
    af.lr_scaling = cfg->lr_scaling; af.lr_rotation = cfg->lr_rotation;
    af.exp_avg = exp_avg; af.exp_avg_sq = exp_avg_sq;
}

static int fallback_adam(const SlsMappingConfig *cfg, int N, float *xyz, float *scaling_raw, float *rotation_raw,
                         float *opacity_raw, float *grads, float *exp_avg, float *exp_avg_sq, int64_t adam_step,
                         const uint32_t *skip_flag, hipStream_t st)
{
    SlsAdamGroup grp[4];
    memset(grp, 0, sizeof(grp));
    float *params[4] = { xyz, opacity_raw, scaling_raw, rotation_raw };
    const size_t offs[4] = { 0, (size_t)3 * N, (size_t)4 * N, (size_t)6 * N };
    const int64_t numel[4] = { (int64_t)3 * N, (int64_t)N, (int64_t)2 * N, (int64_t)4 * N };
    const float lrs[4] = { cfg->lr_xyz, cfg->lr_opacity, cfg->lr_scaling, cfg->lr_rotation };
    for (int k = 0; k < 4; ++k) {
        grp[k].param = params[k];
        grp[k].grad = grads + offs[k];
        grp[k].exp_avg = exp_avg + offs[k];
        grp[k].exp_avg_sq = exp_avg_sq + offs[k];
        grp[k].numel = numel[k];
        grp[k].lr = lrs[k];
    }
    return launch_adam(grp, 4, cfg->beta1, cfg->beta2, cfg->eps, adam_step, skip_flag, st, nullptr, nullptr, nullptr);
}

static int mapping_front(const SlsCamera *cam, int N, const float *xyz, const float *scaling_raw, const float *rotation_raw,
                         const float *opacity_raw, const float *gt_depth, const uint8_t *valid, int n_valid,
                         const float *col_cs, const float *row_cs, const float *col_cs_half, const float *row_cs_half,
                         const SlsMappingConfig *cfg, const StepSwitches &sw, uint32_t cap, const MapWs &w,
                         SlsMappingStatus *status_dev, hipStream_t st)
{
    const DevCam dc = make_devcam(*cam);
    const int T = dc.GX * dc.GY;
    FrontArgs f{};
    f.pf.N = N; f.pf.raw = 1; f.pf.smax = cfg->scaling_max; f.pf.pen = cfg->scaling_max_penalty; f.pf.reg_out = w.reg_accum;
    f.pf.means = xyz; f.pf.scales = scaling_raw; f.pf.rots = rotation_raw; f.pf.opac = opacity_raw;
    f.pf.col_cs = col_cs; f.pf.row_cs = row_cs; f.pf.radii = w.radii;
    f.depth_order = cfg->depth_order; f.reuse_rounds = cfg->reuse_depth_order; f.workspace_ready = cfg->workspace_ready;
    f.list_pairs = cfg->block_masks; f.allmap = w.allmap;
    f.lean = sw.fuse_c;
    f.want_backward = true;
    const uint32_t *sorted_vals; int vals_stride;
    if (int rc = binning_front(dc, cap, w, f, status_dev, st, &sorted_vals, &vals_stride)) return rc;
    ConsumerArgs cargs, cl{};
    cl.H = cam->H; cl.W = cam->W; cl.allmap = w.allmap; cl.gt_depth = gt_depth; cl.valid = valid;
    cl.col_h = (const float2 *)col_cs_half; cl.row_h = (const float2 *)row_cs_half;
    cl.depth_ratio = cfg->depth_ratio; cl.lambda_n = cfg->lambda_normal; cl.lambda_a = cfg->lambda_alpha;
    cl.sums = status_dev->loss_sums; cl.dL_dallmap = w.dL_dallmap;
    cl.order_tiles = sw.order_bwd ? T : 0; cl.block_cost = w.block_cost; cl.block_order = w.block_order;
    if (int rc = launch_consumer(cl, n_valid, w.consumer_scratch, w.consumer_scratch_bytes, sw.fuse_b, st,
                                 sw.fuse_c ? &cargs : nullptr)) return rc;
    if (sw.det && !sw.det_one) SLS_HIP_CHECK(hipMemsetAsync(w.det_max, 0, w.det_bytes, st));
    RenderBwdLaunch rb{};
    rb.ranges = w.ranges; rb.vals = sorted_vals; rb.vals_stride = vals_stride; rb.rec = w.rec; rb.col_cs = col_cs; rb.row_cs = row_cs;
    rb.pix_state = w.pix_state; rb.pix_contrib = w.pix_contrib; rb.dL_dallmap = w.dL_dallmap; rb.grec = w.grec;
    rb.block_masks = w.block_masks; rb.block_masks_shape = 3;
    rb.lean = sw.fuse_c;
    rb.touched = w.touched;
    rb.fused_consumer = sw.fuse_c ? &cargs : nullptr; rb.consumer_b_inline = sw.fuse_b;
    rb.det_max = (sw.det && !sw.det_one) ? w.det_max : nullptr; rb.det_acc = sw.det ? w.det_acc : nullptr;
    rb.det_prev = sw.det_one ? cfg->det_prev : nullptr; rb.det_gex = w.det_gex; rb.det_flag = &status_dev->overflow;
    if (sw.order_bwd) rb.block_order = sw.fuse_b ? cfg->block_order : w.block_order;
    if (sw.fuse_b && sw.order_bwd) rb.order_tag = block_order_tag(T);
    if (int rc = launch_render_bwd(dc, rb, st)) return rc;
    if (cfg->phase == 1 && cfg->grad_bitmap)
        return launch_touched_bitmap(N, w.touched, scaling_raw, cfg->scaling_max, cfg->scaling_max_penalty,
                                     (const uint32_t *)status_dev, cfg->grad_bitmap, st);
    return SLS_OK;
}

size_t sls_mapping_workspace_bytes(int N, int H, int W, uint64_t R_capacity)
{
    return (N < 0 || H <= 0 || W <= 0) ? 0 : carve(N, H, W, R_capacity, nullptr, true).total;
}

size_t sls_block_order_bytes(int H, int W)
{
    if (H <= 0 || W <= 0) return 0;
    const size_t T = (size_t)((W + kTileW - 1) / kTileW) * (size_t)((H + kTileH - 1) / kTileH);
    return sizeof(uint32_t) * (1 + T * (size_t)(kTilePix / 16));
}

size_t sls_mapping_workspace_bytes_cfg(int N, int H, int W, uint64_t R_capacity, const SlsMappingConfig *cfg)
{
    return (N < 0 || H <= 0 || W <= 0) ? 0 : carve(N, H, W, R_capacity, nullptr, !cfg || cfg->deterministic != 0).total;
}

int sls_mapping_step(const SlsCamera *cam, int N, float *xyz, float *scaling_raw, float *rotation_raw,
                     float *opacity_raw, float *grads, float *exp_avg, float *exp_avg_sq, int64_t adam_step,
                     const float *gt_depth, const uint8_t *valid, int n_valid, const float *col_cs,
                     const float *row_cs, const float *col_cs_half, const float *row_cs_half,
                     const SlsMappingConfig *cfg, uint64_t R_capacity, void *workspace, size_t workspace_bytes,
                     SlsMappingStatus *status_dev, float **allmap_out, void *stream)
{
    SLS_REQUIRE(cam && cfg && status_dev && workspace, "null pointer");
    SLS_REQUIRE(N > 0, "N must be positive");
    SLS_REQUIRE(xyz && scaling_raw && rotation_raw && opacity_raw && grads && gt_depth && valid && col_cs && row_cs &&
                    col_cs_half && row_cs_half,
                "null pointer");
    SLS_REQUIRE(!cfg->apply_adam || (exp_avg && exp_avg_sq && adam_step >= 1), "Adam state missing");
    SLS_REQUIRE(R_capacity > 0 && R_capacity < (1ull << 32), "bad instance capacity");
    SLS_REQUIRE(((uintptr_t)workspace & 255) == 0, "workspace must be 256-byte aligned");
    SLS_REQUIRE(cfg->phase >= 0 && cfg->phase <= 2, "phase: 0 whole iteration, 1 up to the tile backward, 2 the rest");
    PoseOut po;
    {
        float *pg = cfg->pose_grad;
        if (int prc = make_pose_out(1, N, &pg, cfg->pose_scratch, cfg->pose_scratch_bytes, &po)) return prc;
    }
    SLS_REQUIRE(!cfg->grad_bitmap || ((!cfg->apply_adam || cfg->union_bitmap) && !cfg->grad_chunk),
                "the gradient bitmap belongs to apply_adam = 0 with the flat bucket");
    SLS_REQUIRE(!cfg->union_bitmap || (cfg->phase == 2 && cfg->apply_adam && cfg->union_prefix && cfg->grad_compact && cfg->grad_compact_index &&
                                       !cfg->grad_chunk && !cfg->keep_grads && (N % 2) == 0 &&
                                       ((((uintptr_t)exp_avg | (uintptr_t)exp_avg_sq) & 15) == 0)),
                "union_bitmap: phase 2 with apply_adam = 1, the union's prefix and row buffer, even N, 16-byte aligned moments");
    SLS_REQUIRE(!cfg->grad_chunk ||
                    (!cfg->apply_adam && cfg->grad_ranks >= 1 && (cfg->grad_chunk % 4u) == 0 && (N % 2) == 0 &&
                     (uint64_t)cfg->grad_chunk * cfg->grad_ranks >= (uint64_t)10 * (uint64_t)N &&
                     (uint64_t)10 * (uint64_t)N < (1ull << 32)),
                "reduce-scatter gradient layout: apply_adam = 0, even N, chunk a multiple of 4 covering 10 N");
    const int H = cam->H, W = cam->W;
    const MapWs w = carve(N, H, W, R_capacity, workspace, cfg->deterministic != 0);
    if (workspace_bytes < w.total) {
        set_error("mapping workspace too small: %zu < %zu", workspace_bytes, w.total);
        return SLS_E_SCRATCH;
    }
    hipStream_t st = (hipStream_t)stream;
    const DevCam dc = make_devcam(*cam);
    const uint32_t cap = (uint32_t)R_capacity;
    if (allmap_out) *allmap_out = w.allmap;
    SLS_REQUIRE(cfg->deterministic >= 0 && cfg->deterministic <= 2, "deterministic: 0 off, 1 two launches, 2 one launch with predicted scales");
    SLS_REQUIRE(cfg->deterministic != 2 || cfg->det_prev, "deterministic = 2 needs the keyframe's det_prev buffer");
    const int T = dc.GX * dc.GY;
    const StepSwitches sw = step_switches(cfg, cfg->deterministic, cfg->det_prev != nullptr, cfg->block_order != nullptr, T);
    int rc = SLS_OK;
    if (cfg->phase != 2)
        rc = mapping_front(cam, N, xyz, scaling_raw, rotation_raw, opacity_raw, gt_depth, valid, n_valid, col_cs, row_cs,
                           col_cs_half, row_cs_half, cfg, sw, cap, w, status_dev, st);
    if (rc || cfg->phase == 1) return rc;
    AdamFuse fuse;
    memset(&fuse, 0, sizeof(fuse));
    fill_step_fuse(fuse, cfg, status_dev, w.reg_accum, N, exp_avg, exp_avg_sq, adam_step);
    if (fuse.enabled) fuse.skip_flag = &status_dev->overflow;
    fuse.clear_grec = 1;
    fuse.touched = w.touched;
    fuse.void_count = 1; fuse.void_stride = 0;
    if (sw.det) {
        fuse.det_max = w.det_max; fuse.det_acc = (const long long *)w.det_acc;
        fuse.det_prev = cfg->det_prev; fuse.det_gex = w.det_gex; fuse.det_onepass = sw.det_one ? 1 : 0;
    }
    if (sw.fuse_b) {
        fuse.loss_partials = (const float *)w.consumer_scratch;
        fuse.n_loss_partials = T * (kTilePix / 16);
        loss_weights(cfg, H, W, n_valid, fuse.loss_w);
        if (sw.order_bwd) { fuse.order_T = T; fuse.order_cost = w.block_cost; fuse.order_out = cfg->block_order; }
    }
    if (cfg->grad_bitmap && cfg->phase != 2) { fuse.grad_bitmap = cfg->grad_bitmap; fuse.grad_bitmap_words = (N + 63) / 64; }
    if (cfg->grad_chunk) {
        fuse.gchunk = cfg->grad_chunk; fuse.gbase = grads;
        fuse.void_flags = grads + cfg->grad_chunk; fuse.void_count = (int)cfg->grad_ranks; fuse.void_stride = (int)cfg->grad_chunk + 4;
    }
    if (cfg->union_bitmap) {
        fuse.union_bitmap = cfg->union_bitmap; fuse.union_prefix = cfg->union_prefix;
        fuse.compact = cfg->grad_compact; fuse.compact_idx = cfg->grad_compact_index; fuse.compact_cap = cfg->grad_compact_capacity;
    }
    PreBwdLaunch pb{};
    pb.N = N; pb.raw = 1; pb.smax = cfg->scaling_max; pb.pen = cfg->scaling_max_penalty;
    pb.means = xyz; pb.scales = scaling_raw; pb.rots = rotation_raw; pb.opac = opacity_raw; pb.radii = w.radii; pb.grec = w.grec;
    pb.dmeans = grads; pb.dopac = grads + (size_t)3 * N; pb.dscales = grads + (size_t)4 * N; pb.drots = grads + (size_t)6 * N;
    pb.fuse = &fuse; pb.pose = pose_arg(po);
    rc = launch_preprocess_bwd(dc, pb, st);
    if (rc || !cfg->apply_adam || fuse.enabled) return rc;
    return fallback_adam(cfg, N, xyz, scaling_raw, rotation_raw, opacity_raw, grads, exp_avg, exp_avg_sq, adam_step,
                         &status_dev->overflow, st);
}

size_t sls_mapping_workspace_bytes_batch(int G, int N, int H, int W, uint64_t R_capacity, const SlsMappingConfig *cfg)
{
    if (G < 1 || G > SLS_MAX_BATCH || N < 0 || H <= 0 || W <= 0) return 0;
    return carve_batch(G, N, H, W, R_capacity, nullptr, !cfg || cfg->deterministic != 0, nullptr);
}

int sls_mapping_step_batch(int G, const SlsKeyframeInputs *kfs, int N, float *xyz, float *scaling_raw, float *rotation_raw,
                           float *opacity_raw, float *grads, float *exp_avg, float *exp_avg_sq, int64_t adam_step,
                           const SlsMappingConfig *cfg, uint64_t R_capacity, void *workspace, size_t workspace_bytes,
                           SlsMappingStatus *status_dev, void *stream)
{
    SLS_REQUIRE(G >= 1 && G <= SLS_MAX_BATCH, "G: 1 to SLS_MAX_BATCH keyframes");
    SLS_REQUIRE(kfs && cfg && status_dev && workspace, "null pointer");
    SLS_REQUIRE(N > 0, "N must be positive");
    SLS_REQUIRE(xyz && scaling_raw && rotation_raw && opacity_raw && grads, "null pointer");
    SLS_REQUIRE(!cfg->apply_adam || (exp_avg && exp_avg_sq && adam_step >= 1), "Adam state missing");
    SLS_REQUIRE(R_capacity > 0 && R_capacity < (1ull << 32), "bad instance capacity");
    SLS_REQUIRE(((uintptr_t)workspace & 255) == 0, "workspace must be 256-byte aligned");
    SLS_REQUIRE(cfg->phase == 0 && !cfg->grad_chunk && !cfg->grad_bitmap && !cfg->union_bitmap,
                "a batch is one whole step on the flat bucket: phase 0, no grad_chunk, grad_bitmap or union_bitmap");
    SLS_REQUIRE(cfg->deterministic >= 0 && cfg->deterministic <= 2, "deterministic: 0 off, 1 two launches, 2 one launch with predicted scales");
    const int H = kfs[0].cam.H, W = kfs[0].cam.W;
    SLS_REQUIRE(H > 0 && W > 0, "bad image size");
    for (int g = 0; g < G; ++g) {
        const SlsKeyframeInputs &k = kfs[g];
        SLS_REQUIRE(k.cam.H == H && k.cam.W == W, "the keyframes of a batch share one image size");
        SLS_REQUIRE(k.gt_depth && k.valid && k.col_cs && k.row_cs && k.col_cs_half && k.row_cs_half && k.depth_order,
                    "null per-keyframe pointer");
        SLS_REQUIRE((k.block_order != nullptr) == (kfs[0].block_order != nullptr), "block_order on every keyframe or on none");
        SLS_REQUIRE(k.reuse_depth_order >= 0 && k.reuse_depth_order <= 4, "reuse_depth_order: 0 from scratch, 1..4 repair rounds");
        for (int h = 0; h < g; ++h) {
            SLS_REQUIRE(kfs[h].depth_order != k.depth_order, "two keyframes share one depth_order buffer");
            SLS_REQUIRE(!k.block_order || kfs[h].block_order != k.block_order, "two keyframes share one block_order buffer");
            SLS_REQUIRE(!k.det_prev || kfs[h].det_prev != k.det_prev, "two keyframes share one det_prev buffer");
        }
    }
    SLS_REQUIRE(!cfg->pose_grad, "a batch takes its pose gradients per keyframe: SlsKeyframeInputs.pose_grad");
    PoseOut po;
    {
        float *pg[SLS_MAX_BATCH];
        for (int g = 0; g < G; ++g) pg[g] = kfs[g].pose_grad;
        if (int prc = make_pose_out(G, N, pg, cfg->pose_scratch, cfg->pose_scratch_bytes, &po)) return prc;
    }
    const bool det = cfg->deterministic != 0;
    MapWs ws[SLS_MAX_BATCH];
    const size_t need = carve_batch(G, N, H, W, R_capacity, workspace, det, ws);
    if (workspace_bytes < need) {
        set_error("batch workspace too small: %zu < %zu", workspace_bytes, need);
        return SLS_E_SCRATCH;
    }
    hipStream_t st = (hipStream_t)stream;
    const uint32_t cap = (uint32_t)R_capacity;
    const DevCam dc0 = make_devcam(kfs[0].cam);
    const int T = dc0.GX * dc0.GY;
    const StepSwitches sw = step_switches(cfg, det ? 1 : 0, false, kfs[0].block_order != nullptr, T);
    BatchFuse bf;
    memset(&bf, 0, sizeof(bf));
    bf.G = G;
    for (int g = 0; g < G; ++g) {
        const SlsKeyframeInputs &k = kfs[g];
        const MapWs &w = ws[g];
        SlsMappingConfig kc = *cfg;
        kc.reuse_depth_order = k.reuse_depth_order; kc.depth_order = k.depth_order;
        kc.block_order = k.block_order; kc.det_prev = k.det_prev; kc.deterministic = det ? 1 : 0;
        if (g > 0) kc.scaling_max_penalty = 0.0f;
        int rc = mapping_front(&k.cam, N, xyz, scaling_raw, rotation_raw, opacity_raw, k.gt_depth, k.valid, k.n_valid,
                               k.col_cs, k.row_cs, k.col_cs_half, k.row_cs_half, &kc, sw, cap, w, status_dev + 1 + g, st);
        if (rc) return rc;
        BatchKeyframe &b = bf.kf[g];
        b.cam = make_devcam(k.cam);
        b.radii = w.radii; b.grec = (float4 *)w.grec; b.touched = w.touched;
        b.status = (uint32_t *)(status_dev + 1 + g);
        if (det) {
            b.det_max = w.det_max; b.det_acc = (long long *)w.det_acc;
            b.det_prev = k.det_prev;
        }
        if (sw.fuse_b) {
            b.loss_partials = (const float *)w.consumer_scratch;
            loss_weights(cfg, H, W, k.n_valid, b.loss_w);
            if (sw.order_bwd) { b.order_cost = w.block_cost; b.order_out = k.block_order; }
        }
    }
    if (sw.fuse_b) {
        bf.n_loss_partials = T * (kTilePix / 16);
        if (sw.order_bwd) bf.order_T = T;
    }
    AdamFuse &af = bf.af;
    fill_step_fuse(af, cfg, status_dev, ws[0].reg_accum, N, exp_avg, exp_avg_sq, adam_step);
    PreBwdLaunch pb{};
    pb.N = N; pb.raw = 1; pb.smax = cfg->scaling_max; pb.pen = cfg->scaling_max_penalty;
    pb.means = xyz; pb.scales = scaling_raw; pb.rots = rotation_raw; pb.opac = opacity_raw;
    pb.dmeans = grads; pb.dopac = grads + (size_t)3 * N; pb.dscales = grads + (size_t)4 * N; pb.drots = grads + (size_t)6 * N;
    pb.pose = pose_arg(po);
    int rc = launch_preprocess_bwd_batch(pb, bf, st);
    if (rc || !cfg->apply_adam || af.enabled) return rc;
    return fallback_adam(cfg, N, xyz, scaling_raw, rotation_raw, opacity_raw, grads, exp_avg, exp_avg_sq, adam_step,
                         &status_dev->overflow, st);
}

}
```

splat_loam_amd/csrc/sls_preprocess.hip:

```cpp
#include <cstring>
#include "sls_common.hpp"
#include "sls_consumer_dev.hpp"
#include "sls_resort.hpp"
#include "sls_launch.hpp"

namespace sls {

__device__ __forceinline__ float dot3(const float *a, const float *b)
{
    return fmaf(a[0], b[0], fmaf(a[1], b[1], a[2] * b[2]));
}
__device__ __forceinline__ void cross3(const float *a, const float *b, float *o)
{
    o[0] = fmaf(a[1], b[2], -(a[2] * b[1]));
    o[1] = fmaf(a[2], b[0], -(a[0] * b[2]));
    o[2] = fmaf(a[0], b[1], -(a[1] * b[0]));
}
__device__ __forceinline__ void matvec(const float *M, const float *v, float *o)
{
#pragma unroll
    for (int i = 0; i < 3; ++i) o[i] = dot3(M + 3 * i, v);
}
__device__ __forceinline__ void matTvec(const float *M, const float *v, float *o)
{
// ... 272 lines not shown
            const uint64_t tb = __ballot(tested);
            if (tested) s_seg_w[__popcll(tb & ((1ull << lane) - 1ull))] = (uint32_t)lane;
            if (lane == 0) { s_ends_w[0] = 0u; s_ends_w[1] = 0u; }
        }
        int seg_base = 0;
        const uint32_t total = (uint32_t)__shfl((int)incl, 63, 64);
        __builtin_amdgcn_wave_barrier();
        for (uint32_t base = 0; base < total; base += 64u) {
            const uint32_t j = base + (uint32_t)lane;
            const bool valid = j < total;
            if (tested && incl > base && incl <= base + 64u) atomicOr(&s_ends_w[(incl - 1u - base) >> 5], 1u << ((incl - 1u - base) & 31u));
            __builtin_amdgcn_wave_barrier();
            const uint64_t ends = ((uint64_t)s_ends_w[1] << 32) | (uint64_t)s_ends_w[0];
            __builtin_amdgcn_wave_barrier();
            if (lane == 0) { s_ends_w[0] = 0u; s_ends_w[1] = 0u; }
            const int seg = seg_base + (int)__popcll(ends & ((1ull << lane) - 1ull));
            seg_base += (int)__popcll(ends);
            const int owner = valid ? (int)s_seg_w[min(seg, 63)] : 0;
            const uint32_t idx = valid ? j - (s_scan_w[owner] - s_rect_cnt(s_rect_w[owner])) : 0u;
            const int4 orc = s_rect_w[owner];
            const int ncols = max(orc.y, 1);
            const int ky = (int)idx / ncols, kx = (int)idx - ky * ncols;
            int tx = orc.x + kx;
            if (tx >= cam.GX) tx -= cam.GX;
            const int ty = orc.z + ky;
            const int x0 = tx * kTileW, y0 = ty * kTileH;
            const float2 cc = col_cs[min(max(x0 + kTileW / 2 - 1, 0), cam.W - 1)], rr = row_cs[min(max(y0 + kTileH / 2 - 1, 0), cam.H - 1)];
            const int out = sls_tile_outside(&cam.tc, &s_cull_w[owner], (float)x0, (float)y0, cc.x, cc.y, rr.x, rr.y);
            if (valid && out) atomicOr(&s_drop_w[2 * owner + (int)(idx >> 5)], 1u << (idx & 31u));
        }
        __builtin_amdgcn_wave_barrier();
        if (tested) {
            const uint64_t drop = ((uint64_t)s_drop_w[2 * lane + 1] << 32) | (uint64_t)s_drop_w[2 * lane];
            my_mask &= ~drop;
            my_tiles = (uint32_t)__popcll(my_mask);
        }
        __builtin_amdgcn_wave_barrier();
    }
    if (i < N) {
        if (tiles) tiles[i] = my_tiles;
        if (pa.sbox) pa.sbox[i] = my_tiles ? make_block_box(q4.x, q4.y, q4.z, q4.w, (cam.GX * kTileW) / 8) : 0u;
        if (tile_mask) tile_mask[i] = my_mask;
        if (erec && pa.erec_box)
            reinterpret_cast<uint2 *>(erec)[i] = make_uint2((uint32_t)my_rc.x | ((uint32_t)my_rc.y << 9) | ((uint32_t)my_rc.z << 19) | ((uint32_t)my_rc.w << 25),
                                                            my_tiles ? make_block_box(q4.x, q4.y, q4.z, q4.w, (cam.GX * kTileW) / 8) : 0u);
        else if (erec) erec[i] = make_int4(my_rc.x | (my_rc.z << 16), my_rc.y | (my_rc.w << 16), (int)(uint32_t)my_mask, (int)(uint32_t)(my_mask >> 32));
    }
    {
        const int lane = threadIdx.x & 63, wave = threadIdx.x >> 6;
        float4 *t = reinterpret_cast<float4 *>(s_mem + (size_t)wave * kPreSliceBytes);
        t[lane * kRec4 + 0] = q0; t[lane * kRec4 + 1] = q1; t[lane * kRec4 + 2] = q2;
        t[lane * kRec4 + 3] = q3; t[lane * kRec4 + 4] = q4;
        __builtin_amdgcn_wave_barrier();
        const size_t base = ((size_t)first + (size_t)wave * 64) * kRec4, end = (size_t)N * kRec4;
#pragma unroll
        for (int k = 0; k < kRec4; ++k) {
            const size_t idx = base + (size_t)(k * 64 + lane);
            if (idx < end) rec[idx] = t[k * 64 + lane];
        }
    }
    if (ra.pen != 0.0f && ra.reg_out) {
        float v = my_reg;
#pragma unroll
        for (int off = 32; off > 0; off >>= 1) v += __shfl_down(v, off, 64);
        if ((threadIdx.x & 63) == 0) s_part[threadIdx.x >> 6] = v;
        __syncthreads();
        if (threadIdx.x == 0) {
            float tot = 0.0f;
#pragma unroll
            for (int k = 0; k < WAVES; ++k) tot += s_part[k];
            if (tot != 0.0f) atomicAdd(ra.reg_out, tot);
        }
    }
}

__global__ __launch_bounds__(256) void preprocess_fwd_kernel(DevCam cam, RegArgs ra, int N, PreFwdArgs pa)
{
    __shared__ __attribute__((aligned(16))) unsigned char s_mem[4 * kPreSliceBytes];
    __shared__ float s_part[4];
    preprocess_fwd_body<4>(cam, ra, N, pa, (int)blockIdx.x * 256, s_mem, s_part);
}

__global__ __launch_bounds__(512) __attribute__((amdgpu_waves_per_eu(6, 6))) void preprocess_fwd_resort_kernel(DevCam cam, RegArgs ra, int N, PreFwdArgs pa, int n_windows,
                                                                    const uint32_t *__restrict__ prev_order,
                                                                    uint64_t *__restrict__ comp)
{
    __shared__ __attribute__((aligned(16))) unsigned char s_mem[8 * kPreSliceBytes];
    __shared__ float s_part[8];
    static_assert(8 * kPreSliceBytes >= (int)(kResortThreads * sizeof(ulonglong2)), "the window sort's pairs fit the slices");
    if ((int)blockIdx.x < n_windows) {
        const float *__restrict__ means = pa.means;
        resort_sort_window((int)blockIdx.x, N, prev_order, [&](uint32_t g) {
            const float m0 = means[3 * (size_t)g], m1 = means[3 * (size_t)g + 1], m2 = means[3 * (size_t)g + 2];
            float p[3];
#pragma unroll
            for (int k = 0; k < 3; ++k) p[k] = fmaf(cam.R[3 * k], m0, fmaf(cam.R[3 * k + 1], m1, fmaf(cam.R[3 * k + 2], m2, cam.t[k])));
            const float rho2 = fmaf(p[2], p[2], fmaf(p[0], p[0], p[1] * p[1]));
            return depth_order_key(sqrtf(rho2));
        }, comp, reinterpret_cast<ulonglong2 *>(s_mem));
        return;
    }
    preprocess_fwd_body<8>(cam, ra, N, pa, ((int)blockIdx.x - n_windows) * 512, s_mem, s_part);
}

__device__ __forceinline__ void pose_terms(const SurfelGeom &g, const float *dp, const float *dTu, const float *dTv,
                                           const float *dTn, float *pg)
{
    float c0[3], c1[3], c2[3], c3[3];
    cross3(g.p, dp, c0); cross3(g.Tu, dTu, c1); cross3(g.Tv, dTv, c2); cross3(g.Tn, dTn, c3);
#pragma unroll
    for (int k = 0; k < 3; ++k) {
        pg[k] = dp[k];
        pg[3 + k] = (c0[k] + c1[k]) + (c2[k] + c3[k]);
    }
}
__device__ __forceinline__ void pose_block_row(const float *pg, float *row)
{
    __shared__ float s_w[4][6];
    float v[6];
#pragma unroll
    for (int k = 0; k < 6; ++k) v[k] = pg[k];
#pragma unroll
    for (int off = 32; off > 0; off >>= 1) {
#pragma unroll
        for (int k = 0; k < 6; ++k) v[k] += __shfl_down(v[k], off, 64);
    }
    __syncthreads();
    if ((threadIdx.x & 63) == 0) {
#pragma unroll
        for (int k = 0; k < 6; ++k) s_w[threadIdx.x >> 6][k] = v[k];
    }
    __syncthreads();
    if (threadIdx.x < 6)
        __hip_atomic_store(row + threadIdx.x, (s_w[0][threadIdx.x] + s_w[1][threadIdx.x]) + (s_w[2][threadIdx.x] + s_w[3][threadIdx.x]),
                           __ATOMIC_RELAXED, __HIP_MEMORY_SCOPE_AGENT);
}
__device__ __forceinline__ void pose_finish(const PoseOut &po, int G, int nb)
{
    __shared__ double s_fin[32][kPoseRow];
    __shared__ uint32_t s_last;
    if (threadIdx.x < 64) {
        asm volatile("s_waitcnt vmcnt(0)" ::: "memory");
        if (threadIdx.x == 0)
            s_last = (__hip_atomic_fetch_add(po.counter, 1u, __ATOMIC_RELAXED, __HIP_MEMORY_SCOPE_AGENT) == (uint32_t)(nb - 1)) ? 1u : 0u;
    }
    __syncthreads();
    if (s_last == 0u) return;
    __builtin_amdgcn_fence(__ATOMIC_ACQUIRE, "agent");
    asm volatile("s_waitcnt vmcnt(0)" ::: "memory");
    __syncthreads();
    const int c = threadIdx.x & (kPoseRow - 1), j = threadIdx.x >> 3;
    for (int g = 0; g < G; ++g) {
        const float *rows = po.rows + (size_t)g * nb * kPoseRow;
        double a = 0.0;
        if (c < 6) {
            for (int b0 = j; b0 < nb; b0 += 32 * 16) {
                float v[16];
#pragma unroll
                for (int u = 0; u < 16; ++u) {
                    const int b = b0 + 32 * u;
                    v[u] = b < nb ? __hip_atomic_load(rows + (size_t)b * kPoseRow + c, __ATOMIC_RELAXED, __HIP_MEMORY_SCOPE_AGENT) : 0.0f;
                }
#pragma unroll
                for (int u = 0; u < 16; ++u) a += (double)v[u];
            }
        }
        s_fin[j][c] = a;
        __syncthreads();
        if (threadIdx.x < 6) {
            double t = 0.0;
            for (int k = 0; k < 32; ++k) t += s_fin[k][threadIdx.x];
            po.out[g][threadIdx.x] = (float)t;
        }
        __syncthreads();
    }
    if (threadIdx.x == 0) __hip_atomic_store(po.counter, 0u, __ATOMIC_RELAXED, __HIP_MEMORY_SCOPE_AGENT);
}

template <bool POSE>
__device__ __forceinline__ void chain_grad_record(const DevCam &cam, const SurfelGeom &g, const float4 q, const float4 g0,
                                                  const float4 g1, const float4 g2, const float4 g3, float *dm, float2 &ds,
                                                  float &dop, float4 &dq, float *pg)
{
    const float gHu[3] = { g0.x, g0.y, g0.z }, gHv[3] = { g1.x, g1.y, g1.z }, gn[3] = { g2.x, g2.y, g2.z };
    const float gnpv = g0.w, grhoc = g1.w, go = g2.w, Su = g3.x, Sv = g3.y, gcpx = g3.z, gcpy = g3.w;
    float dc[3];
    const float irho = frcp(g.rho), isu = frcp(g.su), isv = frcp(g.sv);
#pragma unroll
    for (int k = 0; k < 3; ++k) dc[k] = g.p[k] * irho;
    float dp[3], dA[3], dB[3], t1[3], t2[3];
    cross3(g.p, gHu, dA); cross3(gHu, g.A, t1);
    cross3(g.p, gHv, dB); cross3(gHv, g.B, t2);
    float dTu[3], dTv[3], dTn[3];
#pragma unroll
    for (int k = 0; k < 3; ++k) {
        dp[k] = t1[k] + t2[k];
        dTv[k] = g.sig * dA[k] * isu;
        dTu[k] = -g.sig * dB[k] * isv;
    }
    const float dsu = -dot3(dA, g.A) * isu, dsv = -dot3(dB, g.B) * isv;
#pragma unroll
    for (int k = 0; k < 3; ++k) {
        dTn[k] = g.sig * (gn[k] + gnpv * g.p[k]);
        dp[k] += gnpv * g.n[k];
        dp[k] += grhoc * dc[k];
    }
    float gdc[3];
#pragma unroll
    for (int k = 0; k < 3; ++k) gdc[k] = -(Su * g.Hu[k] + Sv * g.Hv[k]);
    const float gd = dot3(gdc, dc);
#pragma unroll
    for (int k = 0; k < 3; ++k) dp[k] += (gdc[k] - gd * dc[k]) * irho;
    if (g.rxy2 > 1e-30f) {
        const float gaz = gcpx * cam.fx, gel = gcpy * cam.fy;
        const float irxy2 = frcp(g.rxy2), irr = frcp(g.rxy * g.rho2), irho2 = irho * irho;
        dp[0] += gaz * (-g.p[1] * irxy2) + gel * (-g.p[2] * g.p[0] * irr);
        dp[1] += gaz * (g.p[0] * irxy2) + gel * (-g.p[2] * g.p[1] * irr);
        dp[2] += gel * (g.rxy * irho2);
    }
    if constexpr (POSE) pose_terms(g, dp, dTu, dTv, dTn, pg);
    matTvec(cam.R, dp, dm);
    ds = make_float2(cam.mod * dsu, cam.mod * dsv);
    dop = go;
    float G0[3], G1[3], G2[3];
    matTvec(cam.R, dTu, G0); matTvec(cam.R, dTv, G1); matTvec(cam.R, dTn, G2);
    const float r = q.x, x = q.y, y = q.z, z = q.w;
    dq.x = 2.0f * (-z * G1[0] + y * G2[0] + z * G0[1] - x * G2[1] - y * G0[2] + x * G1[2]);
    dq.y = 2.0f * (y * G1[0] + z * G2[0] + y * G0[1] - 2.0f * x * G1[1] - r * G2[1] + z * G0[2] + r * G1[2] - 2.0f * x * G2[2]);
    dq.z = 2.0f * (-2.0f * y * G0[0] + x * G1[0] + r * G2[0] + x * G0[1] + z * G2[1] - r * G0[2] + z * G1[2] - 2.0f * y * G2[2]);
    dq.w = 2.0f * (-2.0f * z * G0[0] - r * G1[0] + x * G2[0] + r * G0[1] - 2.0f * z * G1[1] + y * G2[1] + x * G0[2] + y * G1[2]);
}

__device__ __forceinline__ const PoseOut &pose_arg(const PoseOut &po) { return po; }
template <bool POSE, typename... P>
__global__ __launch_bounds__(256) void preprocess_bwd_kernel(
    DevCam cam, RegArgs ra, AdamFuse af, int N, float *means, float2 *scales, float4 *rots, float *opac,
    const int *__restrict__ radii, float4 *grec, float *__restrict__ dmeans,
    float2 *__restrict__ dscales, float4 *__restrict__ drots, float *__restrict__ dopac, P... pose_args)
{
    const int n_pub = af.publisher ? 1 : 0, n_ord = af.order_out ? 8 : 0;
    if ((int)blockIdx.x < n_pub) {
        if (af.loss_partials) {
            __shared__ float s_loss[3][4];
            const int n4 = af.n_loss_partials / 4;
            float t[3] = { 0.0f, 0.0f, 0.0f };
#pragma unroll
            for (int k = 0; k < 3; ++k) {
                const float4 *src = reinterpret_cast<const float4 *>(af.loss_partials + (size_t)k * af.n_loss_partials);
#pragma unroll 8
                for (int b = threadIdx.x; b < n4; b += 256) {
                    const float4 v = src[b];
                    t[k] += (v.x + v.y) + (v.z + v.w);
                }
            }
#pragma unroll
            for (int off = 32; off > 0; off >>= 1) {
                t[0] += __shfl_down(t[0], off, 64); t[1] += __shfl_down(t[1], off, 64); t[2] += __shfl_down(t[2], off, 64);
            }
            if ((threadIdx.x & 63) == 0) { s_loss[0][threadIdx.x >> 6] = t[0]; s_loss[1][threadIdx.x >> 6] = t[1]; s_loss[2][threadIdx.x >> 6] = t[2]; }
            __syncthreads();
            if (threadIdx.x == 0) {
                float r[3];
#pragma unroll
                for (int k = 0; k < 3; ++k) r[k] = (s_loss[k][0] + s_loss[k][1]) + (s_loss[k][2] + s_loss[k][3]);
                af.status_src[2] = __float_as_uint(r[0]); af.status_src[3] = __float_as_uint(r[1]); af.status_src[4] = __float_as_uint(r[2]);
                af.status_src[5] = __float_as_uint(r[0] * af.loss_w[0] + af.loss_w[1] * r[1] + af.loss_w[2] * r[2]);
            }
        }
        if (threadIdx.x == 0) {
            if (af.reg_accum) {
                af.status_src[6] = __float_as_uint(*af.reg_accum);
                *af.reg_accum = 0.0f;
            }
            if (af.void_flags) {
                const uint32_t bits = af.status_src[1];
                for (int g = 0; g < (af.void_count > 0 ? af.void_count : 1); ++g) {
                    af.void_flags[(size_t)g * af.void_stride + 0] = (bits & 1u) ? 1.0f : 0.0f;
                    af.void_flags[(size_t)g * af.void_stride + 1] = (bits & ~1u) ? 1.0f : 0.0f;
                }
            }
            if (af.status_mirror) mirror_status_block(af.status_src, af.status_mirror);
            if (af.grad_bitmap) {
                const uint32_t bits = af.status_src[1];
                af.grad_bitmap[af.grad_bitmap_words] = (bits & 1u) ? 1ull : 0ull;
                af.grad_bitmap[af.grad_bitmap_words + 1] = (bits & ~1u) ? 1ull : 0ull;
            }
        }
        return;
    }
    if ((int)blockIdx.x < n_pub + n_ord) {
        const int xcd = (int)blockIdx.x - n_pub;
        order_blocks_by_cost(af.order_T, af.order_cost, af.order_out + 1, xcd);
        if (xcd == 0 && threadIdx.x == 0) af.order_out[0] = block_order_tag(af.order_T);
        return;
    }
    const int i = ((int)blockIdx.x - n_pub - n_ord) * 256 + threadIdx.x;
    [[maybe_unused]] float pg[6] = { 0, 0, 0, 0, 0, 0 };
    if (i >= N) { if constexpr (POSE) goto pose_reduce; else return; }
    {
    float dm[3] = { 0, 0, 0 };
    float2 ds = make_float2(0, 0);
    float4 dq = make_float4(0, 0, 0, 0);
    float dop = 0.0f;
    const float2 s_in = scales[i];
    float2 s = s_in;
    const float4 q_in = rots[i];
    float4 q = q_in;
    const float o_in = ra.raw ? opac[i] : 0.0f;
    float o = o_in;
    activate<false>(ra, s, q, o);
    const float m[3] = { means[3 * i], means[3 * i + 1], means[3 * i + 2] };
    const bool marked = !af.touched || af.touched[i] != 0;
    if (marked && af.touched) af.touched[i] = 0;
    if (radii[i] > 0 && marked) {
        SurfelGeom g;
        surfel_geom<false>(cam, m, s, q, g);
        float4 g0, g1, g2, g3;
        if (af.det_acc) {
            float gv[16];
            uint32_t prev[4] = { 0u, 0u, 0u, 0u };
            if (af.det_onepass) {
                const uint4 pv = reinterpret_cast<const uint4 *>(af.det_prev)[i];
                prev[0] = pv.x; prev[1] = pv.y; prev[2] = pv.z; prev[3] = pv.w;
            }
#pragma unroll
            for (int k = 0; k < 16; ++k) {
                int ex;
                if (af.det_onepass) {
                    const uint32_t pb = (prev[k >> 2] >> (8 * (k & 3))) & 0xFFu;
                    ex = det_scale_exp(pb, af.det_gex[k]);
                } else {
                    ex = (int)((af.det_max[(size_t)i * 16 + k] >> 23) & 0xFFu);
                }
                const long long acc = af.det_acc[(size_t)i * 16 + k];
                gv[k] = (float)ldexp((double)acc, ex - 166);
                if (af.det_onepass || af.clear_grec) const_cast<long long *>(af.det_acc)[(size_t)i * 16 + k] = 0;
            }
            if (af.det_prev && (!af.status_src || af.status_src[1] == 0u)) {
                uint32_t pw[4];
#pragma unroll
                for (int w4 = 0; w4 < 4; ++w4) {
                    pw[w4] = 0u;
#pragma unroll
                    for (int b = 0; b < 4; ++b) pw[w4] |= det_predict(gv[4 * w4 + b]) << (8 * b);
                }
                reinterpret_cast<uint4 *>(af.det_prev)[i] = make_uint4(pw[0], pw[1], pw[2], pw[3]);
                if (!af.det_onepass && af.det_gex) {
#pragma unroll
                    for (int k = 0; k < 16; ++k) {
                        const uint32_t pe = (pw[k >> 2] >> (8 * (k & 3))) & 0xFFu;
                        if (pe > af.det_gex[k]) atomicMax(&af.det_gex[k], pe);
                    }
                }
            }
            g0 = make_float4(gv[0], gv[1], gv[2], gv[3]); g1 = make_float4(gv[4], gv[5], gv[6], gv[7]);
            g2 = make_float4(gv[8], gv[9], gv[10], gv[11]); g3 = make_float4(gv[12], gv[13], gv[14], gv[15]);
        } else {
            g0 = grec[(size_t)i * 4 + 0]; g1 = grec[(size_t)i * 4 + 1];
            g2 = grec[(size_t)i * 4 + 2]; g3 = grec[(size_t)i * 4 + 3];
        }
        if (af.clear_grec && !af.det_acc) {
            const float4 z = make_float4(0.0f, 0.0f, 0.0f, 0.0f);
            grec[(size_t)i * 4 + 0] = z; grec[(size_t)i * 4 + 1] = z; grec[(size_t)i * 4 + 2] = z; grec[(size_t)i * 4 + 3] = z;
        }
        const float gHu[3] = { g0.x, g0.y, g0.z }, gHv[3] = { g1.x, g1.y, g1.z }, gn[3] = { g2.x, g2.y, g2.z };
        const float gnpv = g0.w, grhoc = g1.w, go = g2.w, Su = g3.x, Sv = g3.y, gcpx = g3.z, gcpy = g3.w;
        float dc[3];
        const float irho = frcp(g.rho), isu = frcp(g.su), isv = frcp(g.sv);
#pragma unroll
        for (int k = 0; k < 3; ++k) dc[k] = g.p[k] * irho;
        float dp[3], dA[3], dB[3], t1[3], t2[3];
        cross3(g.p, gHu, dA); cross3(gHu, g.A, t1);
        cross3(g.p, gHv, dB); cross3(gHv, g.B, t2);
        float dTu[3], dTv[3], dTn[3];
#pragma unroll
        for (int k = 0; k < 3; ++k) {
            dp[k] = t1[k] + t2[k];
            dTv[k] = g.sig * dA[k] * isu;
            dTu[k] = -g.sig * dB[k] * isv;
        }
        const float dsu = -dot3(dA, g.A) * isu, dsv = -dot3(dB, g.B) * isv;
#pragma unroll
        for (int k = 0; k < 3; ++k) {
            dTn[k] = g.sig * (gn[k] + gnpv * g.p[k]);
            dp[k] += gnpv * g.n[k];
            dp[k] += grhoc * dc[k];
        }
        float gdc[3];
#pragma unroll
        for (int k = 0; k < 3; ++k) gdc[k] = -(Su * g.Hu[k] + Sv * g.Hv[k]);
        const float gd = dot3(gdc, dc);
#pragma unroll
        for (int k = 0; k < 3; ++k) dp[k] += (gdc[k] - gd * dc[k]) * irho;
        if (g.rxy2 > 1e-30f) {
            const float gaz = gcpx * cam.fx, gel = gcpy * cam.fy;
            const float irxy2 = frcp(g.rxy2), irr = frcp(g.rxy * g.rho2), irho2 = irho * irho;
            dp[0] += gaz * (-g.p[1] * irxy2) + gel * (-g.p[2] * g.p[0] * irr);
            dp[1] += gaz * (g.p[0] * irxy2) + gel * (-g.p[2] * g.p[1] * irr);
            dp[2] += gel * (g.rxy * irho2);
        }
        if constexpr (POSE) pose_terms(g, dp, dTu, dTv, dTn, pg);
        matTvec(cam.R, dp, dm);
        ds = make_float2(cam.mod * dsu, cam.mod * dsv);
        dop = go;
        float G0[3], G1[3], G2[3];
        matTvec(cam.R, dTu, G0); matTvec(cam.R, dTv, G1); matTvec(cam.R, dTn, G2);
        const float r = q.x, x = q.y, y = q.z, z = q.w;
        dq.x = 2.0f * (-z * G1[0] + y * G2[0] + z * G0[1] - x * G2[1] - y * G0[2] + x * G1[2]);
        dq.y = 2.0f * (y * G1[0] + z * G2[0] + y * G0[1] - 2.0f * x * G1[1] - r * G2[1] + z * G0[2] + r * G1[2] - 2.0f * x * G2[2]);
        dq.z = 2.0f * (-2.0f * y * G0[0] + x * G1[0] + r * G2[0] + x * G0[1] + z * G2[1] - r * G0[2] + z * G1[2] - 2.0f * y * G2[2]);
        dq.w = 2.0f * (-2.0f * z * G0[0] - r * G1[0] + x * G2[0] + r * G0[1] - 2.0f * z * G1[1] + y * G2[1] + x * G0[2] + y * G1[2]);
    }
    if (ra.pen != 0.0f) {
        const bool first = s.x >= s.y;
        if ((first ? s.x : s.y) >= ra.smax) { if (first) ds.x += ra.pen; else ds.y += ra.pen; }
    }
    if (ra.raw) {
        ds.x *= s.x; ds.y *= s.y;
        dop *= o * (1.0f - o);
        const float nrm = fsqrt(q_in.x * q_in.x + q_in.y * q_in.y + q_in.z * q_in.z + q_in.w * q_in.w);
        const float inv = frcp(fmaxf(nrm, 1e-12f));
        const float dd = dq.x * q.x + dq.y * q.y + dq.z * q.z + dq.w * q.w;
        dq.x = (dq.x - dd * q.x) * inv; dq.y = (dq.y - dd * q.y) * inv;
        dq.z = (dq.z - dd * q.z) * inv; dq.w = (dq.w - dd * q.w) * inv;
    }
    if (af.grad_bitmap) {
        const bool nz = dm[0] != 0.0f || dm[1] != 0.0f || dm[2] != 0.0f || dop != 0.0f || ds.x != 0.0f || ds.y != 0.0f ||
                        dq.x != 0.0f || dq.y != 0.0f || dq.z != 0.0f || dq.w != 0.0f;
        const uint64_t bal = __ballot(nz);
        if ((threadIdx.x & 63) == 0) af.grad_bitmap[i >> 6] = bal;
    }
    if (af.gchunk) {
        const uint32_t C = af.gchunk, n = (uint32_t)N, ui = (uint32_t)i;
        uint32_t e = 3u * ui, qd = e / C, lim = (qd + 1u) * C;
#pragma unroll
        for (int k = 0; k < 3; ++k) {
            if (e + (uint32_t)k >= lim) { ++qd; lim += C; }
            af.gbase[(size_t)(e + (uint32_t)k) + 4u * (size_t)qd] = dm[k];
        }
        e = 3u * n + ui;      af.gbase[(size_t)e + 4u * (size_t)(e / C)] = dop;
        e = 4u * n + 2u * ui; *reinterpret_cast<float2 *>(af.gbase + (size_t)e + 4u * (size_t)(e / C)) = ds;
        e = 6u * n + 4u * ui; *reinterpret_cast<float4 *>(af.gbase + (size_t)e + 4u * (size_t)(e / C)) = dq;
    } else if (!af.enabled || af.write_grads) {
        dmeans[3 * i] = dm[0]; dmeans[3 * i + 1] = dm[1]; dmeans[3 * i + 2] = dm[2];
        dscales[i] = ds;
        drots[i] = dq;
        dopac[i] = dop;
    }
    if (af.union_bitmap) {
        const uint64_t word = af.union_bitmap[i >> 6];
        const int b = i & 63;
        if ((word >> b) & 1ull) {
            const uint32_t slot = af.union_prefix[i >> 6] + (uint32_t)__popcll(word & ((1ull << b) - 1ull));
            if (slot < af.compact_cap) {
                float *o = af.compact + (size_t)slot * 10;
                o[0] = dm[0]; o[1] = dm[1]; o[2] = dm[2]; o[3] = dop; o[4] = ds.x; o[5] = ds.y;
                o[6] = dq.x; o[7] = dq.y; o[8] = dq.z; o[9] = dq.w;
                af.compact_idx[slot] = (uint32_t)i;
            }
            if constexpr (POSE) goto pose_reduce; else return;
        }
        if (dm[0] != 0.0f || dm[1] != 0.0f || dm[2] != 0.0f || dop != 0.0f || ds.x != 0.0f || ds.y != 0.0f ||
            dq.x != 0.0f || dq.y != 0.0f || dq.z != 0.0f || dq.w != 0.0f)
            if (af.status_src) atomicOr(af.status_src + 1, 32u);
    }
    if (af.enabled && *af.skip_flag == 0u) {
        const size_t n = (size_t)N, ix = 3 * (size_t)i, io = 3 * n + i, is = 4 * n + 2 * (size_t)i, ir = 6 * n + 4 * (size_t)i;
        float *M = af.exp_avg, *V = af.exp_avg_sq;
        float p, mm, vv;
        const float ibc1 = frcp(af.c.bc1);
        const float st_x = af.lr_xyz * ibc1, st_o = af.lr_opacity * ibc1;
        const float st_s = af.lr_scaling * ibc1, st_r = af.lr_rotation * ibc1;
#pragma unroll
        for (int k = 0; k < 3; ++k) {
            p = m[k]; mm = M[ix + k]; vv = V[ix + k];
            adam_one(p, dm[k], mm, vv, st_x, af.c);
            means[3 * i + k] = p; M[ix + k] = mm; V[ix + k] = vv;
        }
        p = o_in; mm = M[io]; vv = V[io];
        adam_one(p, dop, mm, vv, st_o, af.c);
        opac[i] = p; M[io] = mm; V[io] = vv;
        float2 ps = s_in, ms = *reinterpret_cast<float2 *>(M + is), vs = *reinterpret_cast<float2 *>(V + is);
        adam_one(ps.x, ds.x, ms.x, vs.x, st_s, af.c);
        adam_one(ps.y, ds.y, ms.y, vs.y, st_s, af.c);
        scales[i] = ps; *reinterpret_cast<float2 *>(M + is) = ms; *reinterpret_cast<float2 *>(V + is) = vs;
        float4 pq = q_in, mq = *reinterpret_cast<float4 *>(M + ir), vq = *reinterpret_cast<float4 *>(V + ir);
        adam_one(pq.x, dq.x, mq.x, vq.x, st_r, af.c);
        adam_one(pq.y, dq.y, mq.y, vq.y, st_r, af.c);
        adam_one(pq.z, dq.z, mq.z, vq.z, st_r, af.c);
        adam_one(pq.w, dq.w, mq.w, vq.w, st_r, af.c);
        rots[i] = pq; *reinterpret_cast<float4 *>(M + ir) = mq; *reinterpret_cast<float4 *>(V + ir) = vq;
    }
    }
pose_reduce:
    if constexpr (POSE) {
        const PoseOut &po = pose_arg(pose_args...);
        const int row = (int)blockIdx.x - n_pub - n_ord;
        pose_block_row(pg, po.rows + (size_t)row * kPoseRow);
        pose_finish(po, 1, (int)gridDim.x - n_pub - n_ord);
    }
}

template <bool POSE, typename... P>
__global__ __launch_bounds__(256) void preprocess_bwd_batch_kernel(RegArgs ra, BatchFuse bf, int N, float *means, float2 *scales,
                                                                   float4 *rots, float *opac, float *__restrict__ dmeans,
                                                                   float2 *__restrict__ dscales, float4 *__restrict__ drots,
                                                                   float *__restrict__ dopac, P... pose_args)
{
    const AdamFuse &af = bf.af;
    const int n_ord = bf.order_T > 0 ? 8 * bf.G : 0;
    if (blockIdx.x == 0) {
        __shared__ float s_loss[SLS_MAX_BATCH][3][4];
        if (bf.n_loss_partials > 0) {
            const int n4 = bf.n_loss_partials / 4;
#pragma unroll
            for (int g = 0; g < SLS_MAX_BATCH; ++g) {
                if (g >= bf.G) break;
                float t[3] = { 0.0f, 0.0f, 0.0f };
#pragma unroll
                for (int k = 0; k < 3; ++k) {
                    const float4 *src = reinterpret_cast<const float4 *>(bf.kf[g].loss_partials + (size_t)k * bf.n_loss_partials);
#pragma unroll 8
                    for (int b = threadIdx.x; b < n4; b += 256) {
                        const float4 v = src[b];
                        t[k] += (v.x + v.y) + (v.z + v.w);
                    }
                }
#pragma unroll
                for (int off = 32; off > 0; off >>= 1) {
                    t[0] += __shfl_down(t[0], off, 64); t[1] += __shfl_down(t[1], off, 64); t[2] += __shfl_down(t[2], off, 64);
                }
                if ((threadIdx.x & 63) == 0) {
                    s_loss[g][0][threadIdx.x >> 6] = t[0]; s_loss[g][1][threadIdx.x >> 6] = t[1]; s_loss[g][2][threadIdx.x >> 6] = t[2];
                }
            }
            __syncthreads();
        }
        if (threadIdx.x == 0) {
            uint32_t R = 0u, bits = 0u;
            float sums[4] = { 0.0f, 0.0f, 0.0f, 0.0f };
#pragma unroll
            for (int g = 0; g < SLS_MAX_BATCH; ++g) {
                if (g >= bf.G) break;
                uint32_t *st = bf.kf[g].status;
                if (bf.n_loss_partials > 0) {
                    float r[3];
#pragma unroll
                    for (int k = 0; k < 3; ++k) r[k] = (s_loss[g][k][0] + s_loss[g][k][1]) + (s_loss[g][k][2] + s_loss[g][k][3]);
                    const float* w = bf.kf[g].loss_w;
                    st[2] = __float_as_uint(r[0]); st[3] = __float_as_uint(r[1]); st[4] = __float_as_uint(r[2]);
                    st[5] = __float_as_uint(r[0] * w[0] + w[1] * r[1] + w[2] * r[2]);
                }
                R = max(R, st[0]);
                bits |= st[1];
#pragma unroll
                for (int k = 0; k < 4; ++k) sums[k] = g == 0 ? __uint_as_float(st[2 + k]) : sums[k] + __uint_as_float(st[2 + k]);
            }
            uint32_t *out = af.status_src;
            out[0] = R; out[1] = bits;
#pragma unroll
            for (int k = 0; k < 4; ++k) out[2 + k] = __float_as_uint(sums[k]);
            out[6] = 0u;
            if (af.reg_accum) {
                out[6] = __float_as_uint(*af.reg_accum);
                *af.reg_accum = 0.0f;
            }
            out[7] = 0u;
            if (af.void_flags) {
                af.void_flags[0] = (bits & 1u) ? 1.0f : 0.0f;
                af.void_flags[1] = (bits & ~1u) ? 1.0f : 0.0f;
            }
            if (af.status_mirror) mirror_status_block(out, af.status_mirror);
        }
        return;
    }
    if ((int)blockIdx.x < 1 + n_ord) {
        const int b = (int)blockIdx.x - 1, g = b >> 3, xcd = b & 7;
        const BatchKeyframe *kf = bf.kf;
        order_blocks_by_cost(bf.order_T, kf[g].order_cost, kf[g].order_out + 1, xcd);
        if (xcd == 0 && threadIdx.x == 0) kf[g].order_out[0] = block_order_tag(bf.order_T);
        return;
    }
    const int i = ((int)blockIdx.x - 1 - n_ord) * 256 + threadIdx.x;
    [[maybe_unused]] float pg[POSE ? SLS_MAX_BATCH : 1][6];
    if constexpr (POSE) {
#pragma unroll
        for (int g = 0; g < SLS_MAX_BATCH; ++g) {
#pragma unroll
            for (int k = 0; k < 6; ++k) pg[g][k] = 0.0f;
        }
    }
    if (i >= N) { if constexpr (POSE) goto pose_reduce; else return; }
    {
    uint32_t skip = 0u;
#pragma unroll
    for (int g = 0; g < SLS_MAX_BATCH; ++g) {
        if (g >= bf.G) break;
        skip |= bf.kf[g].status[1];
    }
    float dm[3] = { 0, 0, 0 };
    float2 ds = make_float2(0, 0);
    float4 dq = make_float4(0, 0, 0, 0);
    float dop = 0.0f;
    const float2 s_in = scales[i];
    float2 s = s_in;
    const float4 q_in = rots[i];
    float4 q = q_in;
    const float o_in = opac[i];
    float o = o_in;
    activate<false>(ra, s, q, o);
    const float m[3] = { means[3 * i], means[3 * i + 1], means[3 * i + 2] };
#pragma unroll
    for (int kg = 0; kg < SLS_MAX_BATCH; ++kg) {
        if (kg >= bf.G) break;
        const BatchKeyframe &kf = bf.kf[kg];
        if (kf.touched[i] == 0) continue;
        kf.touched[i] = 0;
        if (kf.radii[i] <= 0) continue;
        SurfelGeom g;
        surfel_geom<false>(kf.cam, m, s, q, g);
        float4 g0, g1, g2, g3;
        if (kf.det_acc) {
            float gv[16];
#pragma unroll
            for (int k = 0; k < 16; ++k) {
                const int ex = (int)((kf.det_max[(size_t)i * 16 + k] >> 23) & 0xFFu);
                gv[k] = (float)ldexp((double)kf.det_acc[(size_t)i * 16 + k], ex - 166);
                kf.det_acc[(size_t)i * 16 + k] = 0;
            }
            if (kf.det_prev && skip == 0u) {
                uint32_t pw[4];
#pragma unroll
                for (int w4 = 0; w4 < 4; ++w4) {
                    pw[w4] = 0u;
#pragma unroll
                    for (int b = 0; b < 4; ++b) pw[w4] |= det_predict(gv[4 * w4 + b]) << (8 * b);
                }
                reinterpret_cast<uint4 *>(kf.det_prev)[i] = make_uint4(pw[0], pw[1], pw[2], pw[3]);
                if (kf.det_gex) {
#pragma unroll
                    for (int k = 0; k < 16; ++k) {
                        const uint32_t pe = (pw[k >> 2] >> (8 * (k & 3))) & 0xFFu;
                        if (pe > kf.det_gex[k]) atomicMax(&kf.det_gex[k], pe);
                    }
                }
            }
            g0 = make_float4(gv[0], gv[1], gv[2], gv[3]); g1 = make_float4(gv[4], gv[5], gv[6], gv[7]);
            g2 = make_float4(gv[8], gv[9], gv[10], gv[11]); g3 = make_float4(gv[12], gv[13], gv[14], gv[15]);
        } else {
            float4 *rec = kf.grec + (size_t)i * 4;
            g0 = rec[0]; g1 = rec[1]; g2 = rec[2]; g3 = rec[3];
            const float4 z = make_float4(0.0f, 0.0f, 0.0f, 0.0f);
            rec[0] = z; rec[1] = z; rec[2] = z; rec[3] = z;
        }
        float dmk[3], dopk;
        float2 dsk;
        float4 dqk;
        chain_grad_record<POSE>(kf.cam, g, q, g0, g1, g2, g3, dmk, dsk, dopk, dqk, pg[POSE ? kg : 0]);
        dm[0] += dmk[0]; dm[1] += dmk[1]; dm[2] += dmk[2];
        ds.x += dsk.x; ds.y += dsk.y;
        dop += dopk;
        dq.x += dqk.x; dq.y += dqk.y; dq.z += dqk.z; dq.w += dqk.w;
    }
    if (ra.pen != 0.0f) {
        const bool first = s.x >= s.y;
        if ((first ? s.x : s.y) >= ra.smax) { if (first) ds.x += ra.pen; else ds.y += ra.pen; }
    }
    ds.x *= s.x; ds.y *= s.y;
    dop *= o * (1.0f - o);
    {
        const float nrm = fsqrt(q_in.x * q_in.x + q_in.y * q_in.y + q_in.z * q_in.z + q_in.w * q_in.w);
        const float inv = frcp(fmaxf(nrm, 1e-12f));
        const float dd = dq.x * q.x + dq.y * q.y + dq.z * q.z + dq.w * q.w;
        dq.x = (dq.x - dd * q.x) * inv; dq.y = (dq.y - dd * q.y) * inv;
        dq.z = (dq.z - dd * q.z) * inv; dq.w = (dq.w - dd * q.w) * inv;
    }
    if (!af.enabled || af.write_grads) {
        dmeans[3 * i] = dm[0]; dmeans[3 * i + 1] = dm[1]; dmeans[3 * i + 2] = dm[2];
        dscales[i] = ds;
        drots[i] = dq;
        dopac[i] = dop;
    }
    if (af.enabled && skip == 0u) {
        const size_t n = (size_t)N, ix = 3 * (size_t)i, io = 3 * n + i, is = 4 * n + 2 * (size_t)i, ir = 6 * n + 4 * (size_t)i;
        float *M = af.exp_avg, *V = af.exp_avg_sq;
        float p, mm, vv;
        const float ibc1 = frcp(af.c.bc1);
        const float st_x = af.lr_xyz * ibc1, st_o = af.lr_opacity * ibc1;
        const float st_s = af.lr_scaling * ibc1, st_r = af.lr_rotation * ibc1;
#pragma unroll
        for (int k = 0; k < 3; ++k) {
            p = m[k]; mm = M[ix + k]; vv = V[ix + k];
            adam_one(p, dm[k], mm, vv, st_x, af.c);
            means[3 * i + k] = p; M[ix + k] = mm; V[ix + k] = vv;
        }
        p = o_in; mm = M[io]; vv = V[io];
        adam_one(p, dop, mm, vv, st_o, af.c);
        opac[i] = p; M[io] = mm; V[io] = vv;
        float2 ps = s_in, ms = *reinterpret_cast<float2 *>(M + is), vs = *reinterpret_cast<float2 *>(V + is);
        adam_one(ps.x, ds.x, ms.x, vs.x, st_s, af.c);
        adam_one(ps.y, ds.y, ms.y, vs.y, st_s, af.c);
        scales[i] = ps; *reinterpret_cast<float2 *>(M + is) = ms; *reinterpret_cast<float2 *>(V + is) = vs;
        float4 pq = q_in, mq = *reinterpret_cast<float4 *>(M + ir), vq = *reinterpret_cast<float4 *>(V + ir);
        adam_one(pq.x, dq.x, mq.x, vq.x, st_r, af.c);
        adam_one(pq.y, dq.y, mq.y, vq.y, st_r, af.c);
        adam_one(pq.z, dq.z, mq.z, vq.z, st_r, af.c);
        adam_one(pq.w, dq.w, mq.w, vq.w, st_r, af.c);
        rots[i] = pq; *reinterpret_cast<float4 *>(M + ir) = mq; *reinterpret_cast<float4 *>(V + ir) = vq;
    }
    }
pose_reduce:
    if constexpr (POSE) {
        const PoseOut &po = pose_arg(pose_args...);
        const int row = (int)blockIdx.x - 1 - n_ord, nb = (int)gridDim.x - 1 - n_ord;
#pragma unroll
        for (int g = 0; g < SLS_MAX_BATCH; ++g) {
            if (g >= bf.G) break;
            pose_block_row(pg[g], po.rows + ((size_t)g * nb + row) * kPoseRow);
        }
        pose_finish(po, bf.G, nb);
    }
}

__global__ __launch_bounds__(256) void mark_visible_kernel(DevCam cam, int N, const float *__restrict__ means,
                                                           uint8_t *__restrict__ visible)
{
    const int i = blockIdx.x * 256 + threadIdx.x;
    if (i >= N) return;
    float p[3];
#pragma unroll
    for (int k = 0; k < 3; ++k)
        p[k] = fmaf(cam.R[3 * k], means[3 * i], fmaf(cam.R[3 * k + 1], means[3 * i + 1], fmaf(cam.R[3 * k + 2], means[3 * i + 2], cam.t[k])));
    const float rho = sqrtf(fmaf(p[2], p[2], fmaf(p[0], p[0], p[1] * p[1])));
    visible[i] = (rho >= cam.near_c && rho < 1.0e18f) ? 1 : 0;
}

int launch_preprocess_fwd(const DevCam &cam, const PreFwdLaunch &a, hipStream_t st)
{
    const int N = a.N;
    RegArgs ra;
    ra.raw = a.raw; ra.smax = a.smax; ra.pen = a.pen; ra.reg_out = a.reg_out; ra.status_clear = a.status_clear;
    ra.zero_words = a.zero_words; ra.n_zero_words = a.n_zero_words;
    PreFwdArgs pa;
    pa.means = a.means; pa.scales = (const float2 *)a.scales; pa.rots = (const float4 *)a.rots; pa.opac = a.opac;
    pa.rec = (float4 *)a.rec; pa.radii = a.radii; pa.rect = (int4 *)a.rect; pa.tiles = a.tiles; pa.depth = a.depth;
    pa.order_keys = a.order_keys; pa.order_vals = a.order_vals; pa.n_dev = a.n_dev;
    pa.col_cs = (const float2 *)a.col_cs; pa.row_cs = (const float2 *)a.row_cs;
    pa.tile_mask = (a.col_cs && a.row_cs) ? a.tile_mask : nullptr;
    pa.erec = (cam.GX < 65536 && cam.GY < 65536) ? (int4 *)a.erec : nullptr;
    pa.sbox = block_box_fits(cam.GX * kTileW, cam.H) ? a.sbox : nullptr;
    pa.erec_box = (a.erec_box && pa.erec && block_box_fits(cam.GX * kTileW, cam.H)) ? 1 : 0;
    ScopedTimer tm(T_PREPROCESS_FWD, st);
    if (a.resort_prev_order && a.resort_comp) {
        pa.order_vals = nullptr;
        const int nw = (N + kResortWindow - 1) / kResortWindow, nb = (N + 511) / 512;
        hipLaunchKernelGGL(preprocess_fwd_resort_kernel, dim3(nw + nb), dim3(512), 0, st, cam, ra, N, pa, nw, a.resort_prev_order,
                           a.resort_comp);
        SLS_LAUNCH_CHECK("preprocess_fwd_resort_kernel");
        return SLS_OK;
    }
    hipLaunchKernelGGL(preprocess_fwd_kernel, dim3((N + 255) / 256), dim3(256), 0, st, cam, ra, N, pa);
    SLS_LAUNCH_CHECK("preprocess_fwd_kernel");
    return SLS_OK;
}

int launch_preprocess_bwd(const DevCam &cam, const PreBwdLaunch &a, hipStream_t st)
{
    const int N = a.N, nb = (N + 255) / 256;
    RegArgs ra{};
    ra.raw = a.raw; ra.smax = a.smax; ra.pen = a.pen;
    AdamFuse af;
    memset(&af, 0, sizeof(af));
    if (a.fuse) af = *a.fuse;
    af.publisher = (af.loss_partials || af.reg_accum || af.void_flags || af.status_mirror || af.grad_bitmap) ? 1 : 0;
    ScopedTimer tm(T_PREPROCESS_BWD, st);
    if (a.pose)
        hipLaunchKernelGGL((preprocess_bwd_kernel<true, PoseOut>), dim3(nb + af.publisher + (af.order_out ? 8 : 0)), dim3(256), 0, st, cam, ra, af, N,
                           const_cast<float *>(a.means), (float2 *)const_cast<float *>(a.scales), (float4 *)const_cast<float *>(a.rots),
                           const_cast<float *>(a.opac), a.radii, (float4 *)const_cast<float *>(a.grec), a.dmeans, (float2 *)a.dscales,
                           (float4 *)a.drots, a.dopac, *a.pose);
    else
        hipLaunchKernelGGL(preprocess_bwd_kernel<false>, dim3(nb + af.publisher + (af.order_out ? 8 : 0)), dim3(256), 0, st, cam, ra, af, N,
                           const_cast<float *>(a.means), (float2 *)const_cast<float *>(a.scales), (float4 *)const_cast<float *>(a.rots),
                           const_cast<float *>(a.opac), a.radii, (float4 *)const_cast<float *>(a.grec), a.dmeans, (float2 *)a.dscales,
                           (float4 *)a.drots, a.dopac);
    SLS_LAUNCH_CHECK("preprocess_bwd_kernel");
    return SLS_OK;
}

int launch_preprocess_bwd_batch(const PreBwdLaunch &a, const BatchFuse &bf, hipStream_t st)
{
    const int N = a.N, nb = (N + 255) / 256;
    float *means = const_cast<float *>(a.means), *scales = const_cast<float *>(a.scales), *rots = const_cast<float *>(a.rots),
          *opac = const_cast<float *>(a.opac);
    RegArgs ra{};
    ra.raw = 1; ra.smax = a.smax; ra.pen = a.pen;
    ScopedTimer tm(T_PREPROCESS_BWD, st);
    if (a.pose)
        hipLaunchKernelGGL((preprocess_bwd_batch_kernel<true, PoseOut>), dim3(nb + 1 + (bf.order_T > 0 ? 8 * bf.G : 0)), dim3(256), 0, st, ra, bf, N,
                           means, (float2 *)scales, (float4 *)rots, opac, a.dmeans, (float2 *)a.dscales, (float4 *)a.drots, a.dopac, *a.pose);
    else
        hipLaunchKernelGGL(preprocess_bwd_batch_kernel<false>, dim3(nb + 1 + (bf.order_T > 0 ? 8 * bf.G : 0)), dim3(256), 0, st, ra, bf, N,
                           means, (float2 *)scales, (float4 *)rots, opac, a.dmeans, (float2 *)a.dscales, (float4 *)a.drots, a.dopac);
    SLS_LAUNCH_CHECK("preprocess_bwd_batch_kernel");
    return SLS_OK;
}

int launch_mark_visible(const DevCam &cam, int N, const float *means, uint8_t *visible, hipStream_t st)
{
    const int nb = (N + 255) / 256;
    hipLaunchKernelGGL(mark_visible_kernel, dim3(nb), dim3(256), 0, st, cam, N, means, visible);
    SLS_LAUNCH_CHECK("mark_visible_kernel");
    return SLS_OK;
}

}
```

splat_loam_amd/engine.py:

```python
from __future__ import annotations

import ctypes as C
import os
import weakref

import torch
import torch.distributed as dist

from . import _abi
from .fused import camera_aux
from .rasterizer import GaussianRasterizationSettings, get_camera


def carry_bucket(buf: torch.Tensor, keep: torch.Tensor, n_new: int) -> torch.Tensor:
    n_old = int(keep.numel())
    n_keep = int(keep.sum().item())
    if buf.numel() != 10 * n_old or n_new < n_keep:
        raise ValueError("bucket / mask / new size do not fit together")
    out = torch.zeros((10 * n_new,), dtype=buf.dtype, device=buf.device)
    src_off = dst_off = 0
    for width in (3, 1, 2, 4):
        src = buf[src_off:src_off + width * n_old].view(n_old, width)
        out[dst_off:dst_off + width * n_keep].view(n_keep, width).copy_(src[keep])
        src_off += width * n_old
        dst_off += width * n_new
    return out


def dp_chunk(N: int, G: int) -> int:
    return -(-(10 * N) // (4 * G)) * 4


def dp_pieces(N: int, lo: int, hi: int, lrs):
    out = []
    for g0, g1, lr in ((0, 3 * N, lrs[0]), (3 * N, 4 * N, lrs[1]), (4 * N, 6 * N, lrs[2]), (6 * N, 10 * N, lrs[3])):
        a, b = max(lo, g0), min(hi, g1)
        if b > a:
            out.append((a, b, lr))
    return out


def dp_chunked(flat: torch.Tensor, C: int, G: int) -> torch.Tensor:
    out = torch.zeros((G, C + 4), dtype=flat.dtype, device=flat.device)
    pad = torch.zeros((G * C,), dtype=flat.dtype, device=flat.device)
    pad[:flat.numel()] = flat
    out[:, :C] = pad.view(G, C)
    return out.reshape(-1)


class MappingEngine:
    def __init__(self, model, cfg, lrs=(5e-4, 5e-2, 5e-3, 1e-3), betas=(0.9, 0.999), eps=1e-15,
                 capacity_factor: float = 1.3):
        self.model, self.cfg = model, cfg
        self.lrs, self.betas, self.eps = tuple(lrs), tuple(betas), float(eps)
        self.capacity_factor = float(capacity_factor)
        p = model._xyz
        if not p.is_cuda:
            raise RuntimeError("MappingEngine needs ROCm device parameters; there is no CPU fallback")
        self.dev = p.device
        self.N = int(p.shape[0])
        n10 = 10 * self.N
        self.grads = torch.zeros((n10 + 2,), dtype=torch.float32, device=self.dev)
        self.exp_avg = torch.zeros((n10,), dtype=torch.float32, device=self.dev)
        self.exp_avg_sq = torch.zeros((n10,), dtype=torch.float32, device=self.dev)
        self.status = torch.zeros((8,), dtype=torch.int32, device=self.dev)
        self.t = 0
        self.capacity = 0
        self.workspace = None
        self.allmap_ptr = C.c_void_p(0)
        self.last = None
        self._lag_dev = torch.zeros((2, 8), dtype=torch.int32, device=self.dev)
        self._lag_host = torch.zeros((2, 8), dtype=torch.int32).pin_memory()
        self._lag_ev = [torch.cuda.Event(), torch.cuda.Event()]
        self._lag_np = self._lag_host.numpy()
        self.status_poll = True
        self._lag_polled = [False, False]
        self._group = None
        self._lag_ready = []
        self.flushed = []
        self._lag_pending = None
        self.reuse_depth_order = True
        self.inline_loss_stage = True
        self.repair_span = 256
        self._repair_rounds, self._repair_until = 1, 0
        self.keep_grads = False
        self._ws_ready = False
        self._ws_hw = None
        self._ws_det = None
        self.status_mirror = True
        self._orders = {}
        self._set_order_ages()
        self.max_cached_orders = 64
        self.stats = {"repeated_too_small": 0, "repeated_resort": 0, "repeated_exchange": 0, "repeated_det": 0}
        self._enq = 0
        self.dp_mode = os.environ.get("SLS_DP_MODE", "rs_ag")
        self._dp = None
        self._dp_agreed, self._dp_use_rs, self._dp_scheme = None, False, 0
        from .rasterizer import deterministic_mode
        self.deterministic = 2 if os.environ.get("SLS_DETERMINISTIC", "0") == "2" else deterministic_mode()
        self._det_prev = {}
        self._det_two_pass_next = True
        self.block_masks = int(os.environ.get("SLS_BLOCK_MASKS", "0"))
        self._sx = None
        self.exchanged_bytes = 0
        self.exchange_at_world_1 = False
        self.comm_events = None
        self._last_call = None
        self.pose_grad = None
        self._pose_buf = torch.zeros((_abi.SLS_MAX_BATCH, 6), dtype=torch.float32, device=self.dev)
        self._pose_scratch = None

    def grad_views(self):
        N = self.N
        g = self.grads
        if self._dp is not None:
            C, G = self._dp["C"], self._dp["G"]
            g = g.view(G, C + 4)[:, :C].reshape(-1)[:10 * N].clone()
        return {"xyz": g[0:3 * N].view(N, 3), "opacity": g[3 * N:4 * N].view(N, 1),
                "scaling": g[4 * N:6 * N].view(N, 2), "rotation": g[6 * N:10 * N].view(N, 4)}

    def _ensure_workspace(self, H, W, capacity):
        lib = _abi.lib()
        if (self.workspace is None or capacity > self.capacity or (H, W) != self._ws_hw
                or self._ws_det != bool(self.deterministic) or self.N > getattr(self, "_ws_n", 0)):
            self._ws_det = bool(self.deterministic)
            self.capacity, self._ws_hw = int(max(capacity, self.capacity)), (H, W)
            wcfg = _abi.SlsMappingConfig()
            wcfg.deterministic = 1 if self.deterministic else 0
            self._ws_n = self.N + (self.N // 4 if getattr(self, "_bucket_store", None) is not None else 0)
            nbytes = int(lib.sls_mapping_workspace_bytes_cfg(self._ws_n, H, W, self.capacity, C.byref(wcfg)))
            self.workspace = None
            self.workspace = torch.empty((nbytes + 256,), dtype=torch.uint8, device=self.dev)
            self._ws_ready = False
        base = self.workspace.data_ptr()
        return (base + 255) & ~255, self.workspace.numel() - 256

    def _config(self, apply_adam, with_regulariser, reuse_order=False):
        c, cfg = _abi.SlsMappingConfig(), self.cfg
        c.reuse_depth_order = int(reuse_order)
        c.keep_grads = 1 if self.keep_grads else 0
        c.workspace_ready = 1 if self._ws_ready else 0
        self._ws_ready = True
        c.lambda_alpha, c.lambda_normal = cfg.opt_lambda_alpha, cfg.opt_lambda_normal
        c.scaling_max = cfg.opt_scaling_max
        c.scaling_max_penalty = cfg.opt_scaling_max_penalty if with_regulariser else 0.0
        c.depth_ratio = cfg.depth_ratio
        c.lr_xyz, c.lr_opacity, c.lr_scaling, c.lr_rotation = self.lrs
        c.apply_adam = 1 if apply_adam else 0
        c.beta1, c.beta2, c.eps = self.betas[0], self.betas[1], self.eps
        if self._dp is not None and not apply_adam:
            c.grad_chunk, c.grad_ranks = self._dp["C"], self._dp["G"]
        c.deterministic = 1 if self.deterministic else 0
        c.block_masks = int(self.block_masks)
        if self._sx is not None and not apply_adam:
            c.grad_bitmap = self._sx["mine"].data_ptr()
        return c

    def _order_entry(self, camera):
        ent = self._orders.get(id(camera))
        return ent if ent is not None and ent[2]() is camera else None

    def _forget_order(self, camera, failed_repair=False):
        ent = self._order_entry(camera)
        if ent is not None:
            ent[1] = None
        if failed_repair:
            self._repair_rounds = min(self._repair_rounds + 1, 3)
            self._repair_until = self._enq + self.repair_span

    def _set_order_ages(self):
        scale = min(max(500000.0 / max(self.N, 1), 1.0), 3.0)
        self.max_order_age = int(4 * scale)
        self.order_age_round3 = int(12 * scale)
        self.max_order_age_extra = int(48 * scale)
        self.order_age_round4 = 1000000

    def _order_for(self, camera, allow_reuse, H, W, advance=True):
        lib = _abi.lib()
        ent = self._order_entry(camera)
        if ent is None:
            stale = [k for k, e in self._orders.items() if e[2]() is None]
            for k in stale:
                del self._orders[k]
            if len(self._orders) >= self.max_cached_orders:
                self._orders.pop(next(iter(self._orders)))
            ent = [torch.empty((self.N,), dtype=torch.int32, device=self.dev), None, weakref.ref(camera),
                   torch.zeros((int(lib.sls_block_order_bytes(H, W)) // 4,), dtype=torch.int32, device=self.dev)]
            self._orders[id(camera)] = ent
        age = self._enq - ent[1] if ent[1] is not None else None
        reuse = allow_reuse and self.reuse_depth_order and age is not None and age <= self.max_order_age_extra
        if self._repair_rounds > 1 and self._enq >= self._repair_until:
            self._repair_rounds -= 1
            self._repair_until = self._enq + self.repair_span
        reuse = min(self._repair_rounds + (1 if age is not None and age > self.max_order_age else 0)
                    + (1 if age is not None and age > self.order_age_round3 else 0)
                    + (1 if age is not None and age > self.order_age_round4 else 0), 4) if reuse else 0
        if advance:
            self._enq += 1
            ent[1] = self._enq
        return ent, reuse

    def _det_prev_for(self, camera):
        dent = self._det_prev.get(id(camera))
        first_visit = dent is None or dent[1]() is not camera
        if first_visit:
            for k in [k for k, e in self._det_prev.items() if e[1]() is None]:
                del self._det_prev[k]
            while len(self._det_prev) >= self.max_cached_orders:
                self._det_prev.pop(next(iter(self._det_prev)))
            dent = [torch.zeros((self.N, 16), dtype=torch.uint8, device=self.dev), weakref.ref(camera)]
            self._det_prev[id(camera)] = dent
        return dent, first_visit

    def _pose_args(self, cfg, slots):
        need = int(_abi.lib().sls_pose_grad_scratch_bytes(self.N)) * int(slots)
        if self._pose_scratch is None or self._pose_scratch.numel() < need:
            self._pose_scratch = torch.zeros((need,), dtype=torch.uint8, device=self.dev)
        cfg.pose_scratch, cfg.pose_scratch_bytes = self._pose_scratch.data_ptr(), int(self._pose_scratch.numel())

    def _params(self):
        m = self.model
        ps = (m._xyz, m._scaling, m._rotation, m._opacity)
        for p in ps:
            if p.dtype != torch.float32 or not p.is_contiguous() or p.shape[0] != self.N:
                raise RuntimeError("model parameters must stay contiguous float32 of the engine's size")
        return ps

    def _enqueue(self, camera, apply_adam, with_regulariser, status=None, mirror=None, allow_reuse=True, phase=0,
                 pose_grad=False):
        lib = _abi.lib()
        H, W = int(camera.image_height), int(camera.image_width)
        settings = GaussianRasterizationSettings(H, W, 1.0, camera.world_view_transform, camera.projection_matrix)
        ce = get_camera(settings, self.dev)
        aux = camera_aux(camera)
        if self.capacity == 0:
            self.capacity = max(4 * self.N, 1 << 16)
        ws_ptr, ws_bytes = self._ensure_workspace(H, W, self.capacity)
        xyz, scaling, rotation, opacity = self._params()
        ent, reuse = self._order_for(camera, allow_reuse, H, W)
        cfg = self._config(apply_adam, with_regulariser, reuse)
        if self.deterministic == 2:
            dent, first_visit = self._det_prev_for(camera)
            cfg.det_prev = dent[0].data_ptr()
            cfg.deterministic = 1 if (self._det_two_pass_next or first_visit or not cfg.workspace_ready) else 2
            self._det_two_pass_next = False
        cfg.depth_order = ent[0].data_ptr()
        cfg.block_order = ent[3].data_ptr() if self.inline_loss_stage else None
        cfg.status_mirror = mirror
        cfg.void_flags_out = None if (apply_adam or self._dp is not None) else self.grads.data_ptr() + 4 * 10 * self.N
        cfg.phase = int(phase)
        if pose_grad:
            cfg.pose_grad = self._pose_buf.data_ptr()
            self._pose_args(cfg, 1)
        args = (C.byref(ce.cam), self.N, xyz.data_ptr(), scaling.data_ptr(), rotation.data_ptr(), opacity.data_ptr(),
                self.grads.data_ptr(), self.exp_avg.data_ptr(), self.exp_avg_sq.data_ptr(), self.t + 1,
                aux.gt.data_ptr(), aux.valid.data_ptr(), aux.n_valid, ce.col_cs.data_ptr(), ce.row_cs.data_ptr(),
                aux.col_h.data_ptr(), aux.row_h.data_ptr(), C.byref(cfg), self.capacity, ws_ptr, ws_bytes,
                (self.status if status is None else status).data_ptr(), C.byref(self.allmap_ptr),
                torch.cuda.current_stream(self.dev).cuda_stream)
        self._last_call = (args, cfg) if phase == 1 else None
        _abi.check(lib.sls_mapping_step(*args), "sls_mapping_step")

    @staticmethod
    def _void_reason(st):
        if st["too_small"]:
            return "repeated_too_small"
        if st["resort_failed"]:
            return "repeated_resort"
        return "repeated_det" if st.get("det_mispredicted") else "repeated_exchange"

    def _sharded(self, group):
        if not dist.is_initialized():
            return False
        return dist.get_world_size(group) > 1 or self.exchange_at_world_1

    def _read_status(self):
        return self._note(self._parse_status(self.status.cpu()))

    def _note(self, st):
        if st["overflow"] and self.deterministic == 2:
            self._det_two_pass_next = True
        if st.get("outside_union"):
            raise RuntimeError("a surfel outside the agreed union of the touched sets had a non-zero gradient: the early "
                               "gradient bitmap was no superset (sparse exchange) — the iteration's update is void")
        if st.get("handover_mismatch"):
            raise RuntimeError("the tile backward found a forward -> backward hand-over buffer that is not this forward's "
                               "(its tag word does not match): the iteration's gradients are void")
        if self._sx is not None and (not st["overflow"] or st["exchange_too_small"]):
            want = int(st["exchange_count"] * 1.5) + 4096
            self._sx["send"] = int(min(self.N, max(want, int(self._sx["send"] * 0.97))))
        return st

    @staticmethod
    def _parse_status(h):
        R, flags = int(h[0].item()) & 0xFFFFFFFF, int(h[1].item())
        f = h.view(torch.float32)
        return {"R": R, "overflow": bool(flags), "too_small": bool(flags & 1), "resort_failed": bool(flags & 2),
                "exchange_too_small": bool(flags & 4), "det_mispredicted": bool(flags & 8),
                "handover_mismatch": bool(flags & 16), "outside_union": bool(flags & 32),
                "exchange_count": int(h[7].item()) & 0xFFFFFFFF,
                "loss_pixel": float(f[5]), "loss_reg": float(f[6]),
                "loss": float(f[5]) + float(f[6]), "sums": [float(f[2]), float(f[3]), float(f[4])]}

    @staticmethod
    def _parse_status_np(h):
        import numpy as np
        f = h.view(np.float32)
        R, flags = int(h[0]) & 0xFFFFFFFF, int(h[1])
        return {"R": R, "overflow": bool(flags), "too_small": bool(flags & 1), "resort_failed": bool(flags & 2),
                "exchange_too_small": bool(flags & 4), "det_mispredicted": bool(flags & 8),
                "handover_mismatch": bool(flags & 16), "outside_union": bool(flags & 32),
                "exchange_count": int(h[7]) & 0xFFFFFFFF,
                "loss_pixel": float(f[5]), "loss_reg": float(f[6]),
                "loss": float(f[5]) + float(f[6]), "sums": [float(f[2]), float(f[3]), float(f[4])]}

    @torch.no_grad()
    def step(self, camera, group=None, sync: bool = True, pose_grad: bool = False):
        sharded = self._sharded(group)
        if pose_grad:
            if sync is not True:
                raise ValueError("pose_grad needs sync=True: the gradient belongs to the iteration whose status is returned")
            if sharded:
                raise NotImplementedError("pose_grad is served on the single-process path only")
        if self._dp is not None and not sharded:
            raise RuntimeError("this engine's optimiser state is sharded over a process group (dp_mode rs_ag): "
                               "it cannot take a single-process step")
        self._group = group
        if sync == "lagged":
            return self._step_lagged(camera)
        if self._lag_pending is not None:
            self.flush()
        reuse_ok = sync is not False
        while True:
            if not sharded:
                self._enqueue(camera, apply_adam=True, with_regulariser=True, allow_reuse=reuse_ok, pose_grad=pose_grad)
            else:
                rank = dist.get_rank(group)
                self._ensure_dp(group)
                self._enqueue(camera, apply_adam=False, with_regulariser=(rank == 0), allow_reuse=reuse_ok,
                              phase=self._phase_for_exchange())
                self._exchange_and_adam(group, self.status, None)
            if not sync:
                self.t += 1
                return None
            st = self._read_status()
            if not st["overflow"]:
                self.t += 1
                self.last = st
                self.pose_grad = self._pose_buf[0] if pose_grad else None
                return st
            if st["too_small"] or st["resort_failed"]:
                self._forget_order(camera, failed_repair=st["resort_failed"])
            self.stats[self._void_reason(st)] += 1
            if st["too_small"]:
                need = st["R"]
                if sharded:
                    t = torch.tensor([need], dtype=torch.int64, device=self.dev)
                    dist.all_reduce(t, op=dist.ReduceOp.MAX, group=group)
                    need = int(t.item())
                self.capacity = int(max(need, self.capacity) * self.capacity_factor) + 1024
                self.workspace = None

    @torch.no_grad()
    def pose_step(self, camera):
        if self._dp is not None or self._sx is not None:
            raise RuntimeError("this engine's gradient bucket is laid out for a keyframe-parallel exchange: pose_step "
                               "needs the single-process engine")
        if self._lag_pending is not None:
            self.flush()
        while True:
            self._enqueue(camera, apply_adam=False, with_regulariser=False, pose_grad=True)
            st = self._read_status()
            if not st["overflow"]:
                self.pose_grad = self._pose_buf[0]
                return st
            if st["too_small"] or st["resort_failed"]:
                self._forget_order(camera, failed_repair=st["resort_failed"])
            self.stats[self._void_reason(st)] += 1
            if st["too_small"]:
                self.capacity = int(max(st["R"], self.capacity) * self.capacity_factor) + 1024
                self.workspace = None

    def _ensure_batch_workspace(self, G, H, W, capacity):
        lib = _abi.lib()
        b = getattr(self, "_bws", None)
        det = bool(self.deterministic)
        if b is None or G > b["G"] or capacity != b["cap"] or (H, W) != b["hw"] or det != b["det"] or self.N != b["n"]:
            wcfg = _abi.SlsMappingConfig()
            wcfg.deterministic = 1 if det else 0
            Gw = max(G, b["G"] if b is not None and (H, W) == b["hw"] else 1)
            nbytes = int(lib.sls_mapping_workspace_bytes_batch(Gw, self.N, H, W, capacity, C.byref(wcfg)))
            self._bws = None
            b = self._bws = {"G": Gw, "cap": int(capacity), "hw": (H, W), "det": det, "n": self.N, "ready": 0,
                             "buf": torch.empty((nbytes + 256,), dtype=torch.uint8, device=self.dev),
                             "status": torch.zeros((_abi.SLS_MAX_BATCH + 1, 8), dtype=torch.int32, device=self.dev)}
        base = b["buf"].data_ptr()
        return b, (base + 255) & ~255, b["buf"].numel() - 256

    def _enqueue_batch(self, cameras, apply_adam, with_regulariser, allow_reuse=True, pose_grad=False):
        lib = _abi.lib()
        G = len(cameras)
        H, W = int(cameras[0].image_height), int(cameras[0].image_width)
        if self.capacity == 0:
            self.capacity = max(4 * self.N, 1 << 16)
        b, ws_ptr, ws_bytes = self._ensure_batch_workspace(G, H, W, self.capacity)
        xyz, scaling, rotation, opacity = self._params()
        kfs = (_abi.SlsKeyframeInputs * G)()
        keep = []
        reuse_used, ents = [], []
        for g, camera in enumerate(cameras):
            settings = GaussianRasterizationSettings(H, W, 1.0, camera.world_view_transform, camera.projection_matrix)
            ce = get_camera(settings, self.dev)
            aux = camera_aux(camera)
            ent, reuse = self._order_for(camera, allow_reuse, H, W, advance=False)
            ents.append(ent)
            k = kfs[g]
            k.cam = ce.cam
            k.gt_depth, k.valid, k.n_valid = aux.gt.data_ptr(), aux.valid.data_ptr(), aux.n_valid
            k.reuse_depth_order = int(reuse)
            k.col_cs, k.row_cs = ce.col_cs.data_ptr(), ce.row_cs.data_ptr()
            k.col_cs_half, k.row_cs_half = aux.col_h.data_ptr(), aux.row_h.data_ptr()
            k.depth_order = ent[0].data_ptr()
            k.block_order = ent[3].data_ptr() if self.inline_loss_stage else None
            k.det_prev = self._det_prev_for(camera)[0][0].data_ptr() if self.deterministic == 2 else None
            k.pose_grad = self._pose_buf[g].data_ptr() if pose_grad else None
            keep.append((ce, aux))
            reuse_used.append(int(reuse))
        self._enq += 1
        for ent in ents:
            ent[1] = self._enq
        ready = self._ws_ready
        cfg = self._config(apply_adam, with_regulariser)
        self._ws_ready = ready
        cfg.workspace_ready = 1 if G <= b["ready"] else 0
        b["ready"] = max(b["ready"], G)
        cfg.void_flags_out = None if apply_adam else self.grads.data_ptr() + 4 * 10 * self.N
        if pose_grad:
            self._pose_args(cfg, G)
        self.last_batch_reuse = reuse_used
        _abi.check(lib.sls_mapping_step_batch(G, kfs, self.N, xyz.data_ptr(), scaling.data_ptr(), rotation.data_ptr(),
                                              opacity.data_ptr(), self.grads.data_ptr(), self.exp_avg.data_ptr(),
                                              self.exp_avg_sq.data_ptr(), self.t + 1, C.byref(cfg), b["cap"],
                                              ws_ptr, ws_bytes, b["status"].data_ptr(),
                                              torch.cuda.current_stream(self.dev).cuda_stream),
                   "sls_mapping_step_batch")
        return b["status"]

    @torch.no_grad()
    def step_batch(self, cameras, group=None, sync: bool = True, pose_grad: bool = False):
        cams = list(cameras)
        if pose_grad and sync is not True:
            raise ValueError("pose_grad needs sync=True: the gradients belong to the iteration whose status is returned")
        if pose_grad and self._sharded(group):
            raise NotImplementedError("pose_grad is served on the single-process path only")
        if sync == "lagged":
            raise ValueError("step_batch has no lagged mode")
        if not 1 <= len(cams) <= _abi.SLS_MAX_BATCH:
            raise ValueError(f"a batch holds 1 to {_abi.SLS_MAX_BATCH} keyframes, not {len(cams)}")
        if len({id(c) for c in cams}) != len(cams):
            raise ValueError("a keyframe appears twice in the batch")
        if len({(int(c.image_height), int(c.image_width)) for c in cams}) != 1:
            raise ValueError("the keyframes of a batch must share one image size")
        sharded = self._sharded(group)
        if sharded and self.dp_mode != "allreduce":
            raise NotImplementedError(f"step_batch over a process group needs dp_mode 'allreduce', not {self.dp_mode!r}")
        if self._dp is not None or self._sx is not None:
            raise RuntimeError("this engine's optimiser state is laid out for another exchange: step_batch cannot use it")
        self._group = group
        if self._lag_pending is not None:
            self.flush()
        reuse_ok = sync is not False
        while True:
            if not sharded:
                status = self._enqueue_batch(cams, apply_adam=True, with_regulariser=True, allow_reuse=reuse_ok,
                                             pose_grad=pose_grad)
            else:
                self._ensure_dp(group)
                status = self._enqueue_batch(cams, apply_adam=False, with_regulariser=(dist.get_rank(group) == 0),
                                             allow_reuse=reuse_ok)
                self._exchange_and_adam(group, status[0], None)
            if not sync:
                self.t += 1
                return None
            h = status[:len(cams) + 1].cpu()
            st = self._note(self._parse_status(h[0]))
            st["keyframes"] = [self._parse_status(h[1 + g]) for g in range(len(cams))]
            if not st["overflow"]:
                self.t += 1
                self.last = st
                self.pose_grad = self._pose_buf[:len(cams)] if pose_grad else None
                return st
            for cam, kst in zip(cams, st["keyframes"]):
                if kst["too_small"] or kst["resort_failed"]:
                    self._forget_order(cam, failed_repair=kst["resort_failed"])
            self.stats[self._void_reason(st)] += 1
            if st["too_small"]:
                need = st["R"]
                if sharded:
                    t = torch.tensor([need], dtype=torch.int64, device=self.dev)
                    dist.all_reduce(t, op=dist.ReduceOp.MAX, group=group)
                    need = int(t.item())
                self.capacity = int(max(need, self.capacity) * self.capacity_factor) + 1024
                self.workspace = None
                self._bws = None

    def _step_lagged(self, camera):
        slot = 0 if self._lag_pending is None else self._lag_pending[0] ^ 1
        group = self._group
        polled = False
        if self._sharded(group):
            self._ensure_dp(group)
            self._enqueue(camera, apply_adam=False, with_regulariser=(dist.get_rank(group) == 0),
                          status=self._lag_dev[slot], phase=self._phase_for_exchange())
            self._exchange_and_adam(group, self._lag_dev[slot],
                                    self._lag_host[slot].data_ptr() if self.status_mirror else None)
            if not self.status_mirror:
                self._lag_host[slot].copy_(self._lag_dev[slot], non_blocking=True)
        elif self.status_mirror:
            polled = self.status_poll
            if polled:
                self._lag_np[slot, 0] = -1
                self._lag_np[slot, 7] = -1
            self._enqueue(camera, apply_adam=True, with_regulariser=True, status=self._lag_dev[slot],
                          mirror=self._lag_host[slot].data_ptr())
        else:
            self._enqueue(camera, apply_adam=True, with_regulariser=True, status=self._lag_dev[slot])
            self._lag_host[slot].copy_(self._lag_dev[slot], non_blocking=True)
        self.t += 1
        self._lag_polled[slot] = polled
        if not polled:
            self._lag_ev[slot].record(torch.cuda.current_stream(self.dev))
        prev, self._lag_pending = self._lag_pending, (slot, camera)
        if prev is not None:
            self._lag_collect(prev, redo_current=True)
        return self._lag_ready.pop(0) if self._lag_ready else None

    def _lag_collect(self, prev, redo_current):
        pslot, pcam = prev
        if self._lag_polled[pslot]:
            row, spins = self._lag_np[pslot], 0
            while row[7] == -1 or row[0] == -1:
                spins += 1
                if spins > 2_000_000:
                    torch.cuda.current_stream(self.dev).synchronize()
                    if row[7] == -1 or row[0] == -1:
                        raise RuntimeError("the mapping iteration's status never reached its host mirror")
            st = self._note(self._parse_status_np(row.copy()))
        else:
            self._lag_ev[pslot].synchronize()
            st = self._note(self._parse_status(self._lag_host[pslot].clone()))
        if not st["overflow"]:
            self.last = st
            self._lag_ready.append(st)
            return st
        cur, self._lag_pending = self._lag_pending, None
        torch.cuda.current_stream(self.dev).synchronize()
        cur_st = self._note(self._parse_status(self._lag_dev[cur[0]].cpu())) if cur is not None else None
        cur_void = cur_st is not None and cur_st["overflow"]
        self.t -= 2 if cur is not None else 1
        if st["too_small"] or st["resort_failed"]:
            self._forget_order(pcam, failed_repair=st["resort_failed"])
        if cur_void and (cur_st["too_small"] or cur_st["resort_failed"]):
            self._forget_order(cur[1], failed_repair=cur_st["resort_failed"])
        self.stats[self._void_reason(st)] += 1
        if st["too_small"] or (cur_void and cur_st["too_small"]):
            need = max(st["R"], cur_st["R"] if cur_void else 0, self.capacity)
            self.capacity = int(need * self.capacity_factor) + 1024
            self.workspace = None
        if cur_st is not None and not cur_void:
            self._lag_ready.append(cur_st)
        st = self.step(pcam, group=self._group, sync=True)
        self._lag_ready.append(st)
        if cur is not None and not cur_void:
            self.t += 1
        if cur_void:
            if redo_current:
                self._redo_pending(cur[1])
            else:
                self._lag_ready.append(self.step(cur[1], group=self._group, sync=True))
        return st

    def _redo_pending(self, camera):
        ready, self._lag_ready = self._lag_ready, []
        self._step_lagged(camera)
        self._lag_ready = ready + self._lag_ready

    def flush(self):
        if self._lag_pending is not None:
            prev, self._lag_pending = self._lag_pending, None
            self._lag_collect(prev, redo_current=False)
        self.flushed, self._lag_ready = self._lag_ready, []
        return self.flushed[-1] if self.flushed else None

    def _ensure_dp(self, group):
        if self.dp_mode not in ("rs_ag", "allreduce", "sparse"):
            raise ValueError(f"dp_mode must be 'rs_ag', 'allreduce' or 'sparse', not {self.dp_mode!r}")
        G, rank, N = dist.get_world_size(group), dist.get_rank(group), self.N
        if self._dp is not None:
            if self._dp["G"] != G or self._dp["rank"] != rank:
                raise RuntimeError("the process group changed under an engine whose optimiser state is sharded "
                                   f"({self._dp['G']} ranks -> {G}): build a new engine (or remap(reset_state=True))")
            return
        if self._dp_agreed != (G, rank):
            want = (2 if N % 2 == 0 else 0) if self.dp_mode == "sparse" else (1 if (self.dp_mode == "rs_ag" and N % 2 == 0 and 10 * N < 2 ** 32) else 0)
            t = torch.tensor([want, -want], dtype=torch.int32, device=self.dev)
            dist.all_reduce(t, op=dist.ReduceOp.MIN, group=group)
            lo, hi = int(t[0].item()), -int(t[1].item())
            if hi == 2 and lo != 2:
                raise RuntimeError("keyframe-parallel ranks disagree on the gradient exchange: some ask for dp_mode "
                                   "'sparse', others for a dense scheme (check SLS_DP_MODE on every rank)")
            self._dp_use_rs = lo == 1
            self._dp_agreed = (G, rank)
            self._dp_scheme = lo
        if self._dp_scheme == 2:
            if self._sx is not None and (self._sx["G"], self._sx["rank"]) != (G, rank):
                raise RuntimeError("the process group changed under an engine set up for the sparse exchange "
                                   f"({self._sx['G']} ranks -> {G}): build a new engine (or remap())")
            if self._sx is None:
                lib = _abi.lib()
                nw = int(lib.sls_grad_bitmap_words(N))
                self._sx = {"bitmap": torch.zeros((nw,), dtype=torch.int64, device=self.dev),
                            "mine": torch.zeros((nw,), dtype=torch.int64, device=self.dev),
                            "all": torch.zeros((G * nw,), dtype=torch.int64, device=self.dev),
                            "prefix": torch.zeros((nw,), dtype=torch.int32, device=self.dev),
                            "compact": torch.zeros((10 * N,), dtype=torch.float32, device=self.dev),
                            "index": torch.zeros((N,), dtype=torch.int32, device=self.dev),
                            "send": N,
                            "G": G, "rank": rank}
            return
        if not self._dp_use_rs:
            return
        C = dp_chunk(N, G)
        flat = torch.zeros((G * C,), dtype=torch.float32, device=self.dev)
        m = self.model
        for p, off, w in ((m._xyz, 0, 3), (m._opacity, 3 * N, 1), (m._scaling, 4 * N, 2), (m._rotation, 6 * N, 4)):
            view = flat[off:off + w * N].view(N, w)
            view.copy_(p.data)
            p.data = view
        lo, hi = min(rank * C, 10 * N), min((rank + 1) * C, 10 * N)
        ea, es = torch.zeros((C,), dtype=torch.float32, device=self.dev), torch.zeros((C,), dtype=torch.float32, device=self.dev)
        ea[:hi - lo].copy_(self.exp_avg[lo:hi])
        es[:hi - lo].copy_(self.exp_avg_sq[lo:hi])
        self.exp_avg, self.exp_avg_sq = ea, es
        self.grads = torch.zeros((G * (C + 4),), dtype=torch.float32, device=self.dev)
        self._dp = {"G": G, "rank": rank, "C": C, "flat": flat, "lo": lo, "hi": hi,
                    "gshard": torch.zeros((C + 4,), dtype=torch.float32, device=self.dev)}

    def _phase_for_exchange(self):
        return 1 if self._sx is not None else 0

    def _exchange_and_adam(self, group, status, mirror):
        ev = None
        if self.comm_events is not None:
            ev = [torch.cuda.Event(enable_timing=True) for _ in range(4)]
            ev[0].record()
        if self._sx is not None:
            lib, sx, N = _abi.lib(), self._sx, self.N
            st = torch.cuda.current_stream(self.dev).cuda_stream
            dist.all_gather_into_tensor(sx["all"], sx["mine"], group=group)
            G = int(sx["all"].numel() // sx["mine"].numel())
            send = int(sx["send"])
            _abi.check(lib.sls_grad_union(N, sx["all"].data_ptr(), G, sx["bitmap"].data_ptr(), send, sx["prefix"].data_ptr(),
                                          status.data_ptr(), st), "sls_grad_union")
            args, cfg = self._last_call
            cfg.phase, cfg.workspace_ready, cfg.apply_adam, cfg.keep_grads = 2, 1, 1, 0
            cfg.union_bitmap, cfg.union_prefix = sx["bitmap"].data_ptr(), sx["prefix"].data_ptr()
            cfg.grad_compact, cfg.grad_compact_index, cfg.grad_compact_capacity = sx["compact"].data_ptr(), sx["index"].data_ptr(), send
            _abi.check(lib.sls_mapping_step(*args), "sls_mapping_step (phase 2)")
            dist.all_reduce(sx["compact"][:10 * send], op=dist.ReduceOp.SUM, group=group)
            if ev:
                ev[1].record()
            xyz, scaling, rotation, opacity = self._params()
            _abi.check(lib.sls_adam_step_union(N, xyz.data_ptr(), opacity.data_ptr(), scaling.data_ptr(), rotation.data_ptr(),
                                               sx["index"].data_ptr(), sx["compact"].data_ptr(), send, self.exp_avg.data_ptr(),
                                               self.exp_avg_sq.data_ptr(), self.lrs[0], self.lrs[1], self.lrs[2], self.lrs[3],
                                               self.betas[0], self.betas[1], self.eps, self.t + 1, status.data_ptr(), mirror,
                                               st), "sls_adam_step_union")
            if ev:
                ev[2].record(); ev[3].record()
            self.exchanged_bytes = 8 * int(sx["mine"].numel()) + 40 * send
        elif self._dp is None:
            dist.all_reduce(self.grads, op=dist.ReduceOp.SUM, group=group)
            if ev:
                ev[1].record()
            self._adam_reduced(status, mirror)
            if ev:
                ev[2].record(); ev[3].record()
            self.exchanged_bytes = 4 * int(self.grads.numel())
        else:
            d = self._dp
            dist.reduce_scatter_tensor(d["gshard"], self.grads, op=dist.ReduceOp.SUM, group=group)
            if ev:
                ev[1].record()
            self._adam_shard(status, mirror)
            if ev:
                ev[2].record()
            C, r = d["C"], d["rank"]
            mine = d["flat"][r * C:(r + 1) * C]
            if d.get("ag_in_place", True):
                try:
                    dist.all_gather_into_tensor(d["flat"], mine, group=group)
                except (RuntimeError, ValueError):
                    d["ag_in_place"] = False
            if not d.get("ag_in_place", True):
                dist.all_gather_into_tensor(d["flat"], mine.clone(), group=group)
            if ev:
                ev[3].record()
            self.exchanged_bytes = 4 * int(self.grads.numel()) + 4 * C
        if ev:
            self.comm_events.append(ev)

    def _adam_shard(self, status, mirror):
        lib, d, N = _abi.lib(), self._dp, self.N
        lo, hi, C = d["lo"], d["hi"], d["C"]
        arr = (_abi.SlsAdamGroup * 4)()
        k = 0
        for a, b, lr in dp_pieces(N, lo, hi, self.lrs):
            arr[k].param = d["flat"].data_ptr() + 4 * a
            arr[k].grad = d["gshard"].data_ptr() + 4 * (a - lo)
            arr[k].exp_avg = self.exp_avg.data_ptr() + 4 * (a - lo)
            arr[k].exp_avg_sq = self.exp_avg_sq.data_ptr() + 4 * (a - lo)
            arr[k].numel = b - a
            arr[k].lr = lr
            k += 1
        if k == 0:
            arr[0].param = arr[0].grad = arr[0].exp_avg = arr[0].exp_avg_sq = d["gshard"].data_ptr()
            arr[0].numel, arr[0].lr, k = 0, 0.0, 1
        _abi.check(lib.sls_adam_step_reduced(arr, k, self.betas[0], self.betas[1], self.eps, self.t + 1,
                                             d["gshard"].data_ptr() + 4 * C, status.data_ptr(), mirror,
                                             torch.cuda.current_stream(self.dev).cuda_stream),
                   "sls_adam_step_reduced")

    def _adam_reduced(self, status, mirror):
        lib = _abi.lib()
        N = self.N
        xyz, scaling, rotation, opacity = self._params()
        arr = (_abi.SlsAdamGroup * 4)()
        spec = ((xyz, 0, 3 * N, self.lrs[0]), (opacity, 3 * N, N, self.lrs[1]),
                (scaling, 4 * N, 2 * N, self.lrs[2]), (rotation, 6 * N, 4 * N, self.lrs[3]))
        for k, (p, off, n, lr) in enumerate(spec):
            arr[k].param = p.data_ptr()
            arr[k].grad = self.grads.data_ptr() + 4 * off
            arr[k].exp_avg = self.exp_avg.data_ptr() + 4 * off
            arr[k].exp_avg_sq = self.exp_avg_sq.data_ptr() + 4 * off
            arr[k].numel = n
            arr[k].lr = lr
        _abi.check(lib.sls_adam_step_reduced(arr, 4, self.betas[0], self.betas[1], self.eps, self.t + 1,
                                             self.grads.data_ptr() + 4 * 10 * N, status.data_ptr(), mirror,
                                             torch.cuda.current_stream(self.dev).cuda_stream),
                   "sls_adam_step_reduced")

    @torch.no_grad()
    def remap(self, keep=None, appended: int = 0, reset_state: bool = True):
        if self._lag_pending is not None or self._lag_ready:
            self.flush()
        n_old = self.N
        if keep is None:
            keep = torch.ones((n_old,), dtype=torch.bool, device=self.dev)
        keep = keep.to(self.dev).reshape(-1)
        if keep.dtype != torch.bool or keep.numel() != n_old or appended < 0:
            raise ValueError("keep must be a bool mask over the engine's current surfels, appended >= 0")
        n_keep = int(keep.sum().item())
        n_new = n_keep + int(appended)
        if int(self.model._xyz.shape[0]) != n_new:
            raise RuntimeError(f"the model holds {int(self.model._xyz.shape[0])} surfels, keep/appended describe {n_new}")
        if self._dp is not None and not reset_state:
            raise RuntimeError("remap(reset_state=False) is not available once the optimiser state is sharded "
                               "(keyframe-parallel mode rs_ag): use reset_state=True or dp_mode='allreduce'")

        if reset_state:
            self.exp_avg = torch.zeros((10 * n_new,), dtype=torch.float32, device=self.dev)
            self.exp_avg_sq = torch.zeros((10 * n_new,), dtype=torch.float32, device=self.dev)
            self.t = 0
        else:
            self.exp_avg = carry_bucket(self.exp_avg, keep, n_new)
            self.exp_avg_sq = carry_bucket(self.exp_avg_sq, keep, n_new)
        self._dp_agreed = None
        self._sx = None
        self._dp = None
        self.N = n_new
        self._set_order_ages()
        self.grads = torch.zeros((10 * n_new + 2,), dtype=torch.float32, device=self.dev)
        self.workspace = None
        self._orders.clear()
        self._det_prev.clear()
        self._det_two_pass_next = True
        self._pose_scratch = None
        self._params()

    @torch.no_grad()
    def resize(self, n_new: int) -> None:
        if self._lag_pending is not None or self._lag_ready:
            self.flush()
        if self._dp is not None or self._sx is not None:
            raise RuntimeError("resize() is for the single-GPU engine; keyframe-parallel state is laid out by N: use remap()")
        n_new = int(n_new)
        if int(self.model._xyz.shape[0]) != n_new:
            raise RuntimeError(f"the model holds {int(self.model._xyz.shape[0])} surfels, not {n_new}")
        n10 = 10 * n_new
        store = getattr(self, "_bucket_store", None)
        if store is None or store[0].numel() < n10 + 2:
            room = n10 + n10 // 4 + 2
            store = [torch.zeros((room,), dtype=torch.float32, device=self.dev) for _ in range(3)]
            self._bucket_store = store
        self.grads, self.exp_avg, self.exp_avg_sq = store[0][:n10 + 2], store[1][:n10], store[2][:n10]
        self.grads.zero_()
        self.N, self.t = n_new, 0
        self._set_order_ages()
        for ent in self._orders.values():
            ent[1] = None
            if ent[0].numel() < n_new:
                ent[0] = torch.empty((n_new + n_new // 4,), dtype=torch.int32, device=self.dev)
        self._det_prev.clear()
        self._det_two_pass_next = True
        self._ws_ready = False
        self._params()

    def allmap(self, H, W) -> torch.Tensor:
        off = int(self.allmap_ptr.value) - self.workspace.data_ptr()
        return self.workspace[off:off + 7 * H * W * 4].view(torch.float32).view(7, H, W).clone()
```

Before: 1867 Msplats/s.

## Skip Adam updates for surfels with all-zero moments and zero gradient

Adds a per-surfel liveness bitmap, seeded by a scan of the Adam moment buffers and then maintained inside the fused preprocess-backward Adam epilogue. Surfels that have zero moments and receive zero gradient return early, so their parameter and moment reads and writes are skipped. Parameter loads are also deferred for surfels that no keyframe reached. This targets the memory traffic of the full-N fused Adam when only a fraction of the 500k surfels are visible per keyframe. The cost is extra ballot and bitmap work plus a Python property layer that invalidates the bitmap whenever the moments are accessed from outside.

```diff
diff --git a/include/sls_abi.h b/include/sls_abi.h
--- a/include/sls_abi.h
+++ b/include/sls_abi.h
@@ -189,6 +189,7 @@
     float *pose_grad;
     void *pose_scratch;
     size_t pose_scratch_bytes;
+    uint64_t *adam_live;
 } SlsMappingConfig;
 typedef struct SlsMappingStatus {
     uint32_t R;
@@ -295,6 +296,7 @@
                         double beta2, double eps, int64_t step, struct SlsMappingStatus *status_dev,
                         struct SlsMappingStatus *status_mirror, void *stream);
 size_t sls_grad_bitmap_words(int N);
+int sls_adam_live_scan(const float *exp_avg, const float *exp_avg_sq, int N, uint64_t *live_out, void *stream);
 int sls_grad_compact(int N, const uint64_t *bitmaps, int n_bitmaps, uint64_t *union_bitmap, const float *grads_flat,
                      float *compact, uint32_t capacity, uint32_t *word_prefix, struct SlsMappingStatus *status_dev,
                      void *stream);
diff --git a/splat_loam_amd/_abi.py b/splat_loam_amd/_abi.py
--- a/splat_loam_amd/_abi.py
+++ b/splat_loam_amd/_abi.py
@@ -38,6 +38,7 @@
         ("union_bitmap", C.c_void_p), ("union_prefix", C.c_void_p), ("grad_compact", C.c_void_p),
         ("grad_compact_index", C.c_void_p), ("grad_compact_capacity", C.c_uint32), ("reserved2", C.c_uint32),
         ("pose_grad", C.c_void_p), ("pose_scratch", C.c_void_p), ("pose_scratch_bytes", C.c_size_t),
+        ("adam_live", C.c_void_p),
     ]
 
 
@@ -139,6 +140,7 @@
     "sls_adam_step_reduced": (C.c_int, [C.POINTER(SlsAdamGroup), C.c_int, C.c_double, C.c_double, C.c_double,
                                         C.c_int64, _VP, _VP, _VP, _VP]),
     "sls_grad_bitmap_words": (C.c_size_t, [C.c_int]),
+    "sls_adam_live_scan": (C.c_int, [_VP, _VP, C.c_int, _VP, _VP]),
     "sls_grad_union": (C.c_int, [C.c_int, _VP, C.c_int, _VP, C.c_uint32, _VP, _VP, _VP]),
     "sls_adam_step_union": (C.c_int, [C.c_int] + [_VP] * 6 + [C.c_uint32, _VP, _VP] + [C.c_float] * 4 + [C.c_double] * 3 + [C.c_int64, _VP, _VP, _VP]),
     "sls_grad_compact": (C.c_int, [C.c_int, _VP, C.c_int, _VP, _VP, _VP, C.c_uint32, _VP, _VP, _VP]),
diff --git a/splat_loam_amd/csrc/sls_common.hpp b/splat_loam_amd/csrc/sls_common.hpp
--- a/splat_loam_amd/csrc/sls_common.hpp
+++ b/splat_loam_amd/csrc/sls_common.hpp
@@ -309,6 +309,7 @@
     float *compact;
     uint32_t *compact_idx;
     uint32_t compact_cap;
+    uint64_t *adam_live;
 };
 
 struct BatchKeyframe {
diff --git a/splat_loam_amd/csrc/sls_exchange.hip b/splat_loam_amd/csrc/sls_exchange.hip
--- a/splat_loam_amd/csrc/sls_exchange.hip
+++ b/splat_loam_amd/csrc/sls_exchange.hip
@@ -229,6 +229,21 @@
         }
 }
 
+__global__ __launch_bounds__(256) void adam_live_scan_kernel(int N, const uint32_t *__restrict__ M, const uint32_t *__restrict__ V,
+                                                             uint64_t *__restrict__ live)
+{
+    const int i = blockIdx.x * 256 + threadIdx.x;
+    uint32_t any = 0u;
+    if (i < N) {
+        const size_t n = (size_t)N, ix = 3 * (size_t)i, io = 3 * n + i, is = 4 * n + 2 * (size_t)i, ir = 6 * n + 4 * (size_t)i;
+        any = M[ix] | M[ix + 1] | M[ix + 2] | V[ix] | V[ix + 1] | V[ix + 2] | M[io] | V[io] | M[is] | M[is + 1] | V[is] | V[is + 1];
+#pragma unroll
+        for (int k = 0; k < 4; ++k) any |= M[ir + k] | V[ir + k];
+    }
+    const uint64_t bal = __ballot(any != 0u);
+    if ((threadIdx.x & 63) == 0 && (i >> 6) < (N + 63) / 64) live[i >> 6] = bal;
+}
+
 }
 
 using namespace sls;
@@ -236,6 +251,15 @@
 extern "C" {
 
 size_t sls_grad_bitmap_words(int N) { return N > 0 ? (size_t)((N + 63) / 64) + 2 : 2; }
+
+int sls_adam_live_scan(const float *exp_avg, const float *exp_avg_sq, int N, uint64_t *live_out, void *stream)
+{
+    SLS_REQUIRE(N > 0 && exp_avg && exp_avg_sq && live_out, "bad argument");
+    hipLaunchKernelGGL(adam_live_scan_kernel, dim3((N + 255) / 256), dim3(256), 0, (hipStream_t)stream, N, (const uint32_t *)exp_avg,
+                       (const uint32_t *)exp_avg_sq, live_out);
+    SLS_LAUNCH_CHECK("adam_live_scan_kernel");
+    return SLS_OK;
+}
 
 int sls_grad_union(int N, const uint64_t *bitmaps, int n_bitmaps, uint64_t *union_bitmap, uint32_t capacity,
                    uint32_t *word_prefix, SlsMappingStatus *status_dev, void *stream)
diff --git a/splat_loam_amd/csrc/sls_pipeline.hip b/splat_loam_amd/csrc/sls_pipeline.hip
--- a/splat_loam_amd/csrc/sls_pipeline.hip
+++ b/splat_loam_amd/csrc/sls_pipeline.hip
@@ -561,6 +561,7 @@
     af.lr_xyz = cfg->lr_xyz; af.lr_opacity = cfg->lr_opacity;
     af.lr_scaling = cfg->lr_scaling; af.lr_rotation = cfg->lr_rotation;
     af.exp_avg = exp_avg; af.exp_avg_sq = exp_avg_sq;
+    if (cfg->eps >= 1.17549435e-38 && !cfg->union_bitmap) af.adam_live = cfg->adam_live;
 }
 
 static int fallback_adam(const SlsMappingConfig *cfg, int N, float *xyz, float *scaling_raw, float *rotation_raw,
diff --git a/splat_loam_amd/csrc/sls_preprocess.hip b/splat_loam_amd/csrc/sls_preprocess.hip
--- a/splat_loam_amd/csrc/sls_preprocess.hip
+++ b/splat_loam_amd/csrc/sls_preprocess.hip
@@ -598,17 +598,21 @@
     float2 ds = make_float2(0, 0);
     float4 dq = make_float4(0, 0, 0, 0);
     float dop = 0.0f;
-    const float2 s_in = scales[i];
+    const bool marked = !af.touched || af.touched[i] != 0;
+    if (marked && af.touched) af.touched[i] = 0;
+    const bool reached = marked && radii[i] > 0;
+    const bool lazy = af.enabled && af.adam_live != nullptr;
+    const bool have_all = !lazy || reached, have_s = have_all || ra.pen != 0.0f;
+    const float2 s_in = have_s ? scales[i] : make_float2(0.0f, 0.0f);
     float2 s = s_in;
-    const float4 q_in = rots[i];
+    const float4 q_in = have_all ? rots[i] : make_float4(1.0f, 0.0f, 0.0f, 0.0f);
     float4 q = q_in;
-    const float o_in = ra.raw ? opac[i] : 0.0f;
+    const float o_in = (ra.raw && have_all) ? opac[i] : 0.0f;
     float o = o_in;
     activate<false>(ra, s, q, o);
-    const float m[3] = { means[3 * i], means[3 * i + 1], means[3 * i + 2] };
-    const bool marked = !af.touched || af.touched[i] != 0;
-    if (marked && af.touched) af.touched[i] = 0;
-    if (radii[i] > 0 && marked) {
+    float m[3] = { 0.0f, 0.0f, 0.0f };
+    if (have_all) { m[0] = means[3 * i]; m[1] = means[3 * i + 1]; m[2] = means[3 * i + 2]; }
+    if (reached) {
         SurfelGeom g;
         surfel_geom<false>(cam, m, s, q, g);
         float4 g0, g1, g2, g3;
@@ -720,9 +724,9 @@
         dq.x = (dq.x - dd * q.x) * inv; dq.y = (dq.y - dd * q.y) * inv;
         dq.z = (dq.z - dd * q.z) * inv; dq.w = (dq.w - dd * q.w) * inv;
     }
+    const bool nz = dm[0] != 0.0f || dm[1] != 0.0f || dm[2] != 0.0f || dop != 0.0f || ds.x != 0.0f || ds.y != 0.0f ||
+                    dq.x != 0.0f || dq.y != 0.0f || dq.z != 0.0f || dq.w != 0.0f;
     if (af.grad_bitmap) {
-        const bool nz = dm[0] != 0.0f || dm[1] != 0.0f || dm[2] != 0.0f || dop != 0.0f || ds.x != 0.0f || ds.y != 0.0f ||
-                        dq.x != 0.0f || dq.y != 0.0f || dq.z != 0.0f || dq.w != 0.0f;
         const uint64_t bal = __ballot(nz);
         if ((threadIdx.x & 63) == 0) af.grad_bitmap[i >> 6] = bal;
     }
@@ -761,6 +765,21 @@
             if (af.status_src) atomicOr(af.status_src + 1, 32u);
     }
     if (af.enabled && *af.skip_flag == 0u) {
+        float2 ps = s_in;
+        float4 pq = q_in;
+        float p_o = o_in;
+        if (lazy) {
+            const uint64_t was = af.adam_live[i >> 6];
+            const bool update = ((was >> (i & 63)) & 1ull) != 0ull || nz;
+            const uint64_t now = __ballot(update);
+            if ((threadIdx.x & 63) == 0 && now != was) af.adam_live[i >> 6] = now;
+            if (!update) { if constexpr (POSE) goto pose_reduce; else return; }
+            if (!have_s) ps = scales[i];
+            if (!have_all) {
+                pq = rots[i]; p_o = opac[i];
+                m[0] = means[3 * i]; m[1] = means[3 * i + 1]; m[2] = means[3 * i + 2];
+            }
+        }
         const size_t n = (size_t)N, ix = 3 * (size_t)i, io = 3 * n + i, is = 4 * n + 2 * (size_t)i, ir = 6 * n + 4 * (size_t)i;
         float *M = af.exp_avg, *V = af.exp_avg_sq;
         float p, mm, vv;
@@ -773,14 +792,14 @@
             adam_one(p, dm[k], mm, vv, st_x, af.c);
             means[3 * i + k] = p; M[ix + k] = mm; V[ix + k] = vv;
         }
-        p = o_in; mm = M[io]; vv = V[io];
+        p = p_o; mm = M[io]; vv = V[io];
         adam_one(p, dop, mm, vv, st_o, af.c);
         opac[i] = p; M[io] = mm; V[io] = vv;
-        float2 ps = s_in, ms = *reinterpret_cast<float2 *>(M + is), vs = *reinterpret_cast<float2 *>(V + is);
+        float2 ms = *reinterpret_cast<float2 *>(M + is), vs = *reinterpret_cast<float2 *>(V + is);
         adam_one(ps.x, ds.x, ms.x, vs.x, st_s, af.c);
         adam_one(ps.y, ds.y, ms.y, vs.y, st_s, af.c);
         scales[i] = ps; *reinterpret_cast<float2 *>(M + is) = ms; *reinterpret_cast<float2 *>(V + is) = vs;
-        float4 pq = q_in, mq = *reinterpret_cast<float4 *>(M + ir), vq = *reinterpret_cast<float4 *>(V + ir);
+        float4 mq = *reinterpret_cast<float4 *>(M + ir), vq = *reinterpret_cast<float4 *>(V + ir);
         adam_one(pq.x, dq.x, mq.x, vq.x, st_r, af.c);
         adam_one(pq.y, dq.y, mq.y, vq.y, st_r, af.c);
         adam_one(pq.z, dq.z, mq.z, vq.z, st_r, af.c);
@@ -898,21 +917,31 @@
     float2 ds = make_float2(0, 0);
     float4 dq = make_float4(0, 0, 0, 0);
     float dop = 0.0f;
-    const float2 s_in = scales[i];
-    float2 s = s_in;
-    const float4 q_in = rots[i];
-    float4 q = q_in;
-    const float o_in = opac[i];
-    float o = o_in;
-    activate<false>(ra, s, q, o);
-    const float m[3] = { means[3 * i], means[3 * i + 1], means[3 * i + 2] };
+    uint32_t reached = 0u;
 #pragma unroll
     for (int kg = 0; kg < SLS_MAX_BATCH; ++kg) {
         if (kg >= bf.G) break;
         const BatchKeyframe &kf = bf.kf[kg];
         if (kf.touched[i] == 0) continue;
         kf.touched[i] = 0;
-        if (kf.radii[i] <= 0) continue;
+        if (kf.radii[i] > 0) reached |= 1u << kg;
+    }
+    const bool lazy = af.enabled && af.adam_live != nullptr;
+    const bool have_all = !lazy || reached != 0u, have_s = have_all || ra.pen != 0.0f;
+    const float2 s_in = have_s ? scales[i] : make_float2(0.0f, 0.0f);
+    float2 s = s_in;
+    const float4 q_in = have_all ? rots[i] : make_float4(1.0f, 0.0f, 0.0f, 0.0f);
+    float4 q = q_in;
+    const float o_in = have_all ? opac[i] : 0.0f;
+    float o = o_in;
+    activate<false>(ra, s, q, o);
+    float m[3] = { 0.0f, 0.0f, 0.0f };
+    if (have_all) { m[0] = means[3 * i]; m[1] = means[3 * i + 1]; m[2] = means[3 * i + 2]; }
+#pragma unroll
+    for (int kg = 0; kg < SLS_MAX_BATCH; ++kg) {
+        if (kg >= bf.G) break;
+        const BatchKeyframe &kf = bf.kf[kg];
+        if (((reached >> kg) & 1u) == 0u) continue;
         SurfelGeom g;
         surfel_geom<false>(kf.cam, m, s, q, g);
         float4 g0, g1, g2, g3;
@@ -978,6 +1007,23 @@
         dopac[i] = dop;
     }
     if (af.enabled && skip == 0u) {
+        float2 ps = s_in;
+        float4 pq = q_in;
+        float p_o = o_in;
+        if (lazy) {
+            const bool nz = dm[0] != 0.0f || dm[1] != 0.0f || dm[2] != 0.0f || dop != 0.0f || ds.x != 0.0f || ds.y != 0.0f ||
+                            dq.x != 0.0f || dq.y != 0.0f || dq.z != 0.0f || dq.w != 0.0f;
+            const uint64_t was = af.adam_live[i >> 6];
+            const bool update = ((was >> (i & 63)) & 1ull) != 0ull || nz;
+            const uint64_t now = __ballot(update);
+            if ((threadIdx.x & 63) == 0 && now != was) af.adam_live[i >> 6] = now;
+            if (!update) { if constexpr (POSE) goto pose_reduce; else return; }
+            if (!have_s) ps = scales[i];
+            if (!have_all) {
+                pq = rots[i]; p_o = opac[i];
+                m[0] = means[3 * i]; m[1] = means[3 * i + 1]; m[2] = means[3 * i + 2];
+            }
+        }
         const size_t n = (size_t)N, ix = 3 * (size_t)i, io = 3 * n + i, is = 4 * n + 2 * (size_t)i, ir = 6 * n + 4 * (size_t)i;
         float *M = af.exp_avg, *V = af.exp_avg_sq;
         float p, mm, vv;
@@ -990,14 +1036,14 @@
             adam_one(p, dm[k], mm, vv, st_x, af.c);
             means[3 * i + k] = p; M[ix + k] = mm; V[ix + k] = vv;
         }
-        p = o_in; mm = M[io]; vv = V[io];
+        p = p_o; mm = M[io]; vv = V[io];
         adam_one(p, dop, mm, vv, st_o, af.c);
         opac[i] = p; M[io] = mm; V[io] = vv;
-        float2 ps = s_in, ms = *reinterpret_cast<float2 *>(M + is), vs = *reinterpret_cast<float2 *>(V + is);
+        float2 ms = *reinterpret_cast<float2 *>(M + is), vs = *reinterpret_cast<float2 *>(V + is);
         adam_one(ps.x, ds.x, ms.x, vs.x, st_s, af.c);
         adam_one(ps.y, ds.y, ms.y, vs.y, st_s, af.c);
         scales[i] = ps; *reinterpret_cast<float2 *>(M + is) = ms; *reinterpret_cast<float2 *>(V + is) = vs;
-        float4 pq = q_in, mq = *reinterpret_cast<float4 *>(M + ir), vq = *reinterpret_cast<float4 *>(V + ir);
+        float4 mq = *reinterpret_cast<float4 *>(M + ir), vq = *reinterpret_cast<float4 *>(V + ir);
         adam_one(pq.x, dq.x, mq.x, vq.x, st_r, af.c);
         adam_one(pq.y, dq.y, mq.y, vq.y, st_r, af.c);
         adam_one(pq.z, dq.z, mq.z, vq.z, st_r, af.c);
@@ -1069,6 +1115,7 @@
     memset(&af, 0, sizeof(af));
     if (a.fuse) af = *a.fuse;
     af.publisher = (af.loss_partials || af.reg_accum || af.void_flags || af.status_mirror || af.grad_bitmap) ? 1 : 0;
+    if (!af.enabled || af.union_bitmap) af.adam_live = nullptr;
     ScopedTimer tm(T_PREPROCESS_BWD, st);
     if (a.pose)
         hipLaunchKernelGGL((preprocess_bwd_kernel<true, PoseOut>), dim3(nb + af.publisher + (af.order_out ? 8 : 0)), dim3(256), 0, st, cam, ra, af, N,
diff --git a/splat_loam_amd/engine.py b/splat_loam_amd/engine.py
--- a/splat_loam_amd/engine.py
+++ b/splat_loam_amd/engine.py
@@ -61,8 +61,8 @@
         self.N = int(p.shape[0])
         n10 = 10 * self.N
         self.grads = torch.zeros((n10 + 2,), dtype=torch.float32, device=self.dev)
-        self.exp_avg = torch.zeros((n10,), dtype=torch.float32, device=self.dev)
-        self.exp_avg_sq = torch.zeros((n10,), dtype=torch.float32, device=self.dev)
+        self._exp_avg = torch.zeros((n10,), dtype=torch.float32, device=self.dev)
+        self._exp_avg_sq = torch.zeros((n10,), dtype=torch.float32, device=self.dev)
         self.status = torch.zeros((8,), dtype=torch.int32, device=self.dev)
         self.t = 0
         self.capacity = 0
@@ -109,6 +109,56 @@
         self.pose_grad = None
         self._pose_buf = torch.zeros((_abi.SLS_MAX_BATCH, 6), dtype=torch.float32, device=self.dev)
         self._pose_scratch = None
+        self.skip_dormant = True
+        self.skip_dormant_min_surfels = 100_000
+        self._live = None
+        self._live_valid = False
+
+    @property
+    def exp_avg(self):
+        self._live_valid = False
+        return self._exp_avg
+
+    @exp_avg.setter
+    def exp_avg(self, t):
+        self._live_valid = False
+        self._exp_avg = t
+
+    @property
+    def exp_avg_sq(self):
+        self._live_valid = False
+        return self._exp_avg_sq
+
+    @exp_avg_sq.setter
+    def exp_avg_sq(self, t):
+        self._live_valid = False
+        self._exp_avg_sq = t
+
+    def invalidate_live(self):
+        self._live_valid = False
+
+    def _live_ptr(self):
+        if (not self.skip_dormant or self.N < self.skip_dormant_min_surfels or self.N % 2 or
+                ((self._exp_avg.data_ptr() | self._exp_avg_sq.data_ptr()) & 15)):
+            self._live_valid = False
+            return None
+        lib = _abi.lib()
+        nw = int(lib.sls_grad_bitmap_words(self.N))
+        if self._live is None or self._live.numel() < nw:
+            self._live = torch.zeros((nw + nw // 4,), dtype=torch.int64, device=self.dev)
+            self._live_valid = False
+        if not self._live_valid:
+            _abi.check(lib.sls_adam_live_scan(self._exp_avg.data_ptr(), self._exp_avg_sq.data_ptr(), self.N,
+                                              self._live.data_ptr(), torch.cuda.current_stream(self.dev).cuda_stream),
+                       "sls_adam_live_scan")
+            self._live_valid = True
+        return self._live.data_ptr()
+
+    def live_count(self) -> int:
+        if not self._live_valid or self._live is None:
+            return None
+        words = self._live[:(self.N + 63) // 64].cpu().numpy().view("uint64")
+        return int(sum(bin(int(w)).count("1") for w in words))
 
     def grad_views(self):
         N = self.N
@@ -249,11 +299,13 @@
         cfg.status_mirror = mirror
         cfg.void_flags_out = None if (apply_adam or self._dp is not None) else self.grads.data_ptr() + 4 * 10 * self.N
         cfg.phase = int(phase)
+        if apply_adam:
+            cfg.adam_live = self._live_ptr()
         if pose_grad:
             cfg.pose_grad = self._pose_buf.data_ptr()
             self._pose_args(cfg, 1)
         args = (C.byref(ce.cam), self.N, xyz.data_ptr(), scaling.data_ptr(), rotation.data_ptr(), opacity.data_ptr(),
-                self.grads.data_ptr(), self.exp_avg.data_ptr(), self.exp_avg_sq.data_ptr(), self.t + 1,
+                self.grads.data_ptr(), self._exp_avg.data_ptr(), self._exp_avg_sq.data_ptr(), self.t + 1,
                 aux.gt.data_ptr(), aux.valid.data_ptr(), aux.n_valid, ce.col_cs.data_ptr(), ce.row_cs.data_ptr(),
                 aux.col_h.data_ptr(), aux.row_h.data_ptr(), C.byref(cfg), self.capacity, ws_ptr, ws_bytes,
                 (self.status if status is None else status).data_ptr(), C.byref(self.allmap_ptr),
@@ -435,12 +487,14 @@
         cfg.workspace_ready = 1 if G <= b["ready"] else 0
         b["ready"] = max(b["ready"], G)
         cfg.void_flags_out = None if apply_adam else self.grads.data_ptr() + 4 * 10 * self.N
+        if apply_adam:
+            cfg.adam_live = self._live_ptr()
         if pose_grad:
             self._pose_args(cfg, G)
         self.last_batch_reuse = reuse_used
         _abi.check(lib.sls_mapping_step_batch(G, kfs, self.N, xyz.data_ptr(), scaling.data_ptr(), rotation.data_ptr(),
-                                              opacity.data_ptr(), self.grads.data_ptr(), self.exp_avg.data_ptr(),
-                                              self.exp_avg_sq.data_ptr(), self.t + 1, C.byref(cfg), b["cap"],
+                                              opacity.data_ptr(), self.grads.data_ptr(), self._exp_avg.data_ptr(),
+                                              self._exp_avg_sq.data_ptr(), self.t + 1, C.byref(cfg), b["cap"],
                                               ws_ptr, ws_bytes, b["status"].data_ptr(),
                                               torch.cuda.current_stream(self.dev).cuda_stream),
                    "sls_mapping_step_batch")
@@ -639,9 +693,9 @@
             p.data = view
         lo, hi = min(rank * C, 10 * N), min((rank + 1) * C, 10 * N)
         ea, es = torch.zeros((C,), dtype=torch.float32, device=self.dev), torch.zeros((C,), dtype=torch.float32, device=self.dev)
-        ea[:hi - lo].copy_(self.exp_avg[lo:hi])
-        es[:hi - lo].copy_(self.exp_avg_sq[lo:hi])
-        self.exp_avg, self.exp_avg_sq = ea, es
+        ea[:hi - lo].copy_(self._exp_avg[lo:hi])
+        es[:hi - lo].copy_(self._exp_avg_sq[lo:hi])
+        self._exp_avg, self._exp_avg_sq = ea, es
         self.grads = torch.zeros((G * (C + 4),), dtype=torch.float32, device=self.dev)
         self._dp = {"G": G, "rank": rank, "C": C, "flat": flat, "lo": lo, "hi": hi,
                     "gshard": torch.zeros((C + 4,), dtype=torch.float32, device=self.dev)}
@@ -650,6 +704,7 @@
         return 1 if self._sx is not None else 0
 
     def _exchange_and_adam(self, group, status, mirror):
+        self._live_valid = False
         ev = None
         if self.comm_events is not None:
             ev = [torch.cuda.Event(enable_timing=True) for _ in range(4)]
@@ -672,8 +727,8 @@
                 ev[1].record()
             xyz, scaling, rotation, opacity = self._params()
             _abi.check(lib.sls_adam_step_union(N, xyz.data_ptr(), opacity.data_ptr(), scaling.data_ptr(), rotation.data_ptr(),
-                                               sx["index"].data_ptr(), sx["compact"].data_ptr(), send, self.exp_avg.data_ptr(),
-                                               self.exp_avg_sq.data_ptr(), self.lrs[0], self.lrs[1], self.lrs[2], self.lrs[3],
+                                               sx["index"].data_ptr(), sx["compact"].data_ptr(), send, self._exp_avg.data_ptr(),
+                                               self._exp_avg_sq.data_ptr(), self.lrs[0], self.lrs[1], self.lrs[2], self.lrs[3],
                                                self.betas[0], self.betas[1], self.eps, self.t + 1, status.data_ptr(), mirror,
                                                st), "sls_adam_step_union")
             if ev:
@@ -718,8 +773,8 @@
         for a, b, lr in dp_pieces(N, lo, hi, self.lrs):
             arr[k].param = d["flat"].data_ptr() + 4 * a
             arr[k].grad = d["gshard"].data_ptr() + 4 * (a - lo)
-            arr[k].exp_avg = self.exp_avg.data_ptr() + 4 * (a - lo)
-            arr[k].exp_avg_sq = self.exp_avg_sq.data_ptr() + 4 * (a - lo)
+            arr[k].exp_avg = self._exp_avg.data_ptr() + 4 * (a - lo)
+            arr[k].exp_avg_sq = self._exp_avg_sq.data_ptr() + 4 * (a - lo)
             arr[k].numel = b - a
             arr[k].lr = lr
             k += 1
@@ -741,8 +796,8 @@
         for k, (p, off, n, lr) in enumerate(spec):
             arr[k].param = p.data_ptr()
             arr[k].grad = self.grads.data_ptr() + 4 * off
-            arr[k].exp_avg = self.exp_avg.data_ptr() + 4 * off
-            arr[k].exp_avg_sq = self.exp_avg_sq.data_ptr() + 4 * off
+            arr[k].exp_avg = self._exp_avg.data_ptr() + 4 * off
+            arr[k].exp_avg_sq = self._exp_avg_sq.data_ptr() + 4 * off
             arr[k].numel = n
             arr[k].lr = lr
         _abi.check(lib.sls_adam_step_reduced(arr, 4, self.betas[0], self.betas[1], self.eps, self.t + 1,
@@ -769,12 +824,12 @@
                                "(keyframe-parallel mode rs_ag): use reset_state=True or dp_mode='allreduce'")
 
         if reset_state:
-            self.exp_avg = torch.zeros((10 * n_new,), dtype=torch.float32, device=self.dev)
-            self.exp_avg_sq = torch.zeros((10 * n_new,), dtype=torch.float32, device=self.dev)
+            self._exp_avg = torch.zeros((10 * n_new,), dtype=torch.float32, device=self.dev)
+            self._exp_avg_sq = torch.zeros((10 * n_new,), dtype=torch.float32, device=self.dev)
             self.t = 0
         else:
-            self.exp_avg = carry_bucket(self.exp_avg, keep, n_new)
-            self.exp_avg_sq = carry_bucket(self.exp_avg_sq, keep, n_new)
+            self._exp_avg = carry_bucket(self._exp_avg, keep, n_new)
+            self._exp_avg_sq = carry_bucket(self._exp_avg_sq, keep, n_new)
         self._dp_agreed = None
         self._sx = None
         self._dp = None
@@ -786,6 +841,7 @@
         self._det_prev.clear()
         self._det_two_pass_next = True
         self._pose_scratch = None
+        self._live_valid = False
         self._params()
 
     @torch.no_grad()
@@ -803,7 +859,7 @@
             room = n10 + n10 // 4 + 2
             store = [torch.zeros((room,), dtype=torch.float32, device=self.dev) for _ in range(3)]
             self._bucket_store = store
-        self.grads, self.exp_avg, self.exp_avg_sq = store[0][:n10 + 2], store[1][:n10], store[2][:n10]
+        self.grads, self._exp_avg, self._exp_avg_sq = store[0][:n10 + 2], store[1][:n10], store[2][:n10]
         self.grads.zero_()
         self.N, self.t = n_new, 0
         self._set_order_ages()
@@ -814,6 +870,7 @@
         self._det_prev.clear()
         self._det_two_pass_next = True
         self._ws_ready = False
+        self._live_valid = False
         self._params()
 
     def allmap(self, H, W) -> torch.Tensor:
```

Result: no change. 1862 Msplats/s (-0.3%).
